# renjie-liang/HUAL

Hardware: AMD Instinct MI355X
Metric: train clips/sec (higher is better)
Workload: dtype f32 (fp16x3 / bf16x3 split-operand MFMA, fp32 accumulate); 1 GPU; Charades-STA SeqPAN train step (fwd+bwd+clip+AdamWD, dropout 0.2), batch 64/GPU, T=128, vdim=1024, L=20, C=8, dim=128, 8 heads, 2 attention layers, random init; ONE batch resident in HBM, batch assembly (hual_assemble_batch) outside the timed region; global_batch=64, T=128, vdim=1024, L=20, parallelism=dp1, launch=hipGraph, video_dtype=f32

## Files before the change

hual_amd/csrc/convblock.h:

```cpp
#pragma once
#include "common.h"
#include "rowops.h"

namespace hual {

struct CbLayerFwd {
  const float* ln_g; const float* ln_b;
  const float* dw;
  const float* wimg;
  const float* bias;
  float* c; float* xout;
  float* y;
  uint8_t* relu_bits; uint8_t* keep_bits;
  float* mean; float* rstd;
  int drop_site;
};
struct CbFwdArgs {
  const float* x0;
  const float* pos; float* x0_out;
  CbLayerFwd l[4];
  int MT;
  uint32_t drop_row0;
};
#define HUAL_CB_MAXMT 46
int conv_block_fused_rows(int R, int Nv = 0);
struct LnProjArgs;
int launch_conv_block_fwd(const CbFwdArgs& a, const RowSpace& rs, const DropCfg& drop, hipStream_t s, const LnProjArgs* tail = nullptr);

struct CbLayerBwd {
  const float* ln_g; const float* ln_b; const float* dw;
  const float* wimg_t;
  const float* x;
  const float* mean; const float* rstd;
  const uint8_t* relu_prev; const uint8_t* keep_prev;
  float* dz;
  float* dz_prev;
  float* part;
};
struct CbBwdArgs {
  const float* dx_in;
  const uint8_t* relu_bits3; const uint8_t* keep_bits3;
  float* dx_out;
  CbLayerBwd l[4];
  int MT;
  uint32_t drop_row0;
};
#define HUAL_CB_BWD_MAXMT 40
int conv_block_fused_rows_bwd(int R, int Nv = 0);
int conv_block_bwd_blocks(int R, int Nv = 0);
int launch_conv_block_bwd(const CbBwdArgs& a, const RowSpace& rs, const DropCfg& drop, hipStream_t s);

}
```

hual_amd/csrc/convblock.hip:

```cpp
#include "convblock.h"
#include "tilecore.h"
#include "prof.h"

using namespace hual;

#include "lnproj_body.h"

#define CB_XS 33
#define CB_NPAR 10
#define CB_TP_F4 (10 * 32)

template <bool TAIL>
__device__ __forceinline__ void conv_block_fwd_body(const CbFwdArgs& a, const RowSpace& rs, const DropCfg& drop, const LnProjArgs* lp, char* cb_lds) {
  const int MT = a.MT;
  const int XR = MT + 24;
  float4* X = reinterpret_cast<float4*>(cb_lds);
  float4* TP = X + XR * CB_XS;
  char* Ahi = reinterpret_cast<char*>(TP + (TAIL ? CB_TP_F4 : 0));
  char* Alo = Ahi + 64 * 256;
  float* ainv = reinterpret_cast<float*>(Alo + 64 * 256);
  float* smean = ainv + 64;
  float* srstd = smean + 72;
  float4* par = reinterpret_cast<float4*>(srstd + 72);
  const int lane = threadIdx.x & 63, wave = threadIdx.x >> 6;
  const int l32 = threadIdx.x & 31, grp = threadIdx.x >> 5;
  const int col = 4 * l32;
  const int R = rs.R;
  const int tile_ = xcd_tile_clip(blockIdx.x, rs.R, rs.Nq > 0 ? rs.Nv : 0, MT);
  if (tile_ < 0) return;
  const int r0 = tile_ * MT;
  if (r0 >= rs.R) return;
  const int xbase = r0 - 12;

  const DropRegs dr = drop_load(drop);
  HUAL_STAMP_K(2, 0);
  TfW wc, wn;
  tf_load_w(wc, a.l[0].wimg, wave, lane);
  {
    float4 xv[5], pv[5], qv[4];
    const float* posp = a.pos ? a.pos : a.x0;
#pragma unroll
    for (int u = 0; u < 5; ++u) {
      const int i = grp + 16 * u, row = min(max(xbase + i, 0), R - 1);
      int lo, hi;
      cb_segment(row, rs, lo, hi);
      xv[u] = ld4(a.x0 + (size_t)row * HUAL_D + col);
      pv[u] = ld4(posp + (size_t)(a.pos ? row - lo : row) * HUAL_D + col);
    }
#pragma unroll
    for (int l = 0; l < 4; ++l) {
      const CbLayerFwd& L = a.l[l];
      const float* src = grp < 7 ? L.dw + grp * HUAL_D : (grp == 7 ? L.ln_g : (grp == 8 ? L.ln_b : L.bias));
      qv[l] = ld4(src + col);
    }
    float4 tq = f4zero();
    if (TAIL) {
      const float* src = lp->g1;
      if (grp == 1) src = lp->b1;
      if (grp == 2 && lp->g2) src = lp->g2;
      if (grp == 3 && lp->g2) src = lp->b2;
#pragma unroll
      for (int k = 0; k < HUAL_LNPROJ_MAX; ++k)
        if (grp == 4 + k && k < lp->nproj && lp->bias[k]) src = lp->bias[k];
      tq = ld4(src + col);
    }
#pragma unroll
    for (int u = 0; u < 5; ++u) {
      const int i = grp + 16 * u, row = xbase + i;
      if (i >= XR) continue;
      const bool ok = row >= 0 && row < R;
      float4 v = ok ? xv[u] : f4zero();
      if (a.pos) {
        v = ok ? cb_add(v, pv[u]) : v;
        if (row >= r0 && row < r0 + MT && row < R) st4(a.x0_out + (size_t)row * HUAL_D + col, v);
      }
      X[__mul24(i, CB_XS) + l32] = v;
    }
#pragma unroll
    for (int l = 0; l < 4; ++l)
      if (grp < CB_NPAR) par[(l * CB_NPAR + grp) * 32 + l32] = qv[l];
    if (TAIL && grp < LNP_TP_VECS) TP[grp * 32 + l32] = tq;
  }
  cb_barrier();
  HUAL_STAMP_K(2, 1);

#pragma unroll 1
  for (int l = 0; l < 4; ++l) {
    const CbLayerFwd& L = a.l[l];
    const int H = 9 - 3 * l;
    const int nout = MT + 2 * H;
    const int ntile = (nout + 15) >> 4;
    const int obase = r0 - H;
    const int j = lane & 15, g = lane >> 4, ecol = 16 * wave + 4 * g;
    const float4* lp = par + l * CB_NPAR * 32;
    {
      const int ri = threadIdx.x >> 2, q = threadIdx.x & 3;
      const int xi = ri + 9 - H;
      const int t = xbase + xi;
      const bool ok = ri < nout + 6 && t >= 0 && t < R;
      float4 v[8];
#pragma unroll
      for (int k = 0; k < 8; ++k) v[k] = ok ? X[__mul24(xi, CB_XS) + 8 * q + k] : f4zero();
      float p[8];
#pragma unroll
      for (int k = 0; k < 8; ++k) p[k] = cb_hsum(v[k]);
      float s = ((p[0] + p[1]) + (p[2] + p[3])) + ((p[4] + p[5]) + (p[6] + p[7]));
      s += dpp_xor_partner(s, 1);
      s += dpp_xor_partner(s, 2);
      const float mean = s * (1.0f / HUAL_D);
#pragma unroll
      for (int k = 0; k < 8; ++k) {
        const float4 d = make_float4(v[k].x - mean, v[k].y - mean, v[k].z - mean, v[k].w - mean);
        p[k] = cb_hsum(cb_mul(d, d));
      }
      s = ((p[0] + p[1]) + (p[2] + p[3])) + ((p[4] + p[5]) + (p[6] + p[7]));
      s += dpp_xor_partner(s, 1);
      s += dpp_xor_partner(s, 2);
      const float rstd = rsqrtf(s * (1.0f / HUAL_D) + LN_EPS);
      if (ok && q == 0) {
        smean[xi] = mean;
        srstd[xi] = rstd;
        if (t >= r0 && t < r0 + MT) { L.mean[t] = mean; L.rstd[t] = rstd; }
      }
    }
    cb_barrier();
    HUAL_STAMP_K(2, 2 + 6 * l);
    if (l + 1 < 4) tf_load_w(wn, a.l[l + 1].wimg, wave, lane);
    {
      const float4 gam = lp[7 * 32 + l32], bet = lp[8 * 32 + l32];
      float4 w[7];
#pragma unroll
      for (int k = 0; k < 7; ++k) w[k] = lp[k * 32 + l32];
      const int la = grp * ntile, lb = la + ntile;
      float4 hv[10];
      {
        float4 xr[10];
        float mr[10], sr[10];
#pragma unroll
        for (int s = 0; s < 10; ++s) {
          const int t = obase + la - 3 + s;
          const int xi = min(max(t - xbase, 0), XR - 1);
          xr[s] = X[__mul24(xi, CB_XS) + l32];
          mr[s] = smean[xi];
          sr[s] = srstd[xi];
        }
#pragma unroll
        for (int s = 0; s < 10; ++s) {
          const int li = la - 3 + s, t = obase + li;
          const bool in = s < ntile + 6 && li < nout + 3 && t >= 0 && t < R;
          const float4 v = xr[s];
          const float mean = mr[s], rstd = sr[s];
          const float4 hn = cb_fma(make_float4((v.x - mean) * rstd, (v.y - mean) * rstd, (v.z - mean) * rstd, (v.w - mean) * rstd), gam, bet);
          hv[s] = in ? hn : f4zero();
        }
      }
      int slo, shi;
      cb_segment(min(max(obase + la, 0), R - 1), rs, slo, shi);
#pragma unroll
      for (int u = 0; u < 4; ++u) {
        const int lo_ = la + u;
        if (lo_ >= lb) continue;
        const int o = obase + lo_;
        float4 c = f4zero();
        const bool live = lo_ < nout && o >= 0 && o < R;
        if (live) {
          if (o >= shi) { slo = shi; shi = slo + (slo < rs.Nv ? rs.T : rs.L); }
          c = cb_fma((o - 3 >= slo) ? hv[u] : f4zero(), w[0], c);
          c = cb_fma((o - 2 >= slo) ? hv[u + 1] : f4zero(), w[1], c);
          c = cb_fma((o - 1 >= slo) ? hv[u + 2] : f4zero(), w[2], c);
          c = cb_fma(hv[u + 3], w[3], c);
          c = cb_fma((o + 1 < shi) ? hv[u + 4] : f4zero(), w[4], c);
          c = cb_fma((o + 2 < shi) ? hv[u + 5] : f4zero(), w[5], c);
          c = cb_fma((o + 3 < shi) ? hv[u + 6] : f4zero(), w[6], c);
          if (o >= r0 && o < r0 + MT) st4_nt(L.c + (size_t)o * HUAL_D + col, c);
        }
        const float inv = cb_store_operand_fx(Ahi, Alo, lo_, l32, c);
        if (l32 == 0) ainv[lo_] = live ? inv : 0.f;
      }
    }
    HUAL_STAMP_K(2, 3 + 6 * l);
    cb_barrier();
    HUAL_STAMP_K(2, 4 + 6 * l);
    f32x4 acc[4];
    if (ntile > 3) tf_mma_lean<4, 64 * 256>(Ahi, wc, lane, acc);
    else tf_mma_lean<3, 64 * 256>(Ahi, wc, lane, reinterpret_cast<f32x4(&)[3]>(acc));
    HUAL_STAMP_K(2, 5 + 6 * l);
    {
      const float4 bias = lp[9 * 32 + (ecol >> 2)];
      const bool dropping = L.drop_site >= 0 && dr.enabled;
      int orow[4];
      bool own[4], live[4];
#pragma unroll
      for (int rt = 0; rt < 4; ++rt) {
        const int lr = 16 * rt + j;
        orow[rt] = obase + lr;
        live[rt] = rt < ntile && lr < nout && orow[rt] >= 0 && orow[rt] < R;
        own[rt] = live[rt] && orow[rt] >= r0 && orow[rt] < r0 + MT;
      }
      uint32_t nib[4] = {15u, 15u, 15u, 15u};
      if (dropping) {
        drop_nib2_store_t(dr, (uint32_t)L.drop_site, a.drop_row0, orow[0], orow[1], own[0], own[1], (uint32_t)(ecol >> 2), L.keep_bits, nib[0], nib[1], lane);
        drop_nib2_store_t(dr, (uint32_t)L.drop_site, a.drop_row0, orow[2], orow[3], own[2], own[3], (uint32_t)(ecol >> 2), L.keep_bits, nib[2], nib[3], lane);
      }
      uint32_t rb[4] = {0u, 0u, 0u, 0u};
      float irv[4];
      float4 xres[4];
#pragma unroll
      for (int rt = 0; rt < 4; ++rt) {
        irv[rt] = ainv[16 * rt + j];
        xres[rt] = X[__mul24(min(max(orow[rt] - xbase, 0), XR - 1), CB_XS) + (ecol >> 2)];
      }
#pragma unroll
      for (int rt = 0; rt < 4; ++rt) {
        if (!live[rt]) continue;
        const int o = orow[rt];
        const float ir = irv[rt];
        float4 v = make_float4(fmaf(acc[rt][0], ir, 0.f) + bias.x, fmaf(acc[rt][1], ir, 0.f) + bias.y,
                               fmaf(acc[rt][2], ir, 0.f) + bias.z, fmaf(acc[rt][3], ir, 0.f) + bias.w);
        v = relu_nan4(v);
        if (own[rt] && L.y) st4(L.y + (size_t)o * HUAL_D + ecol, v);
        rb[rt] = f4_posbits(v);
        if (dropping) v = f4_select(nib[rt], make_float4(v.x * dr.scale, v.y * dr.scale, v.z * dr.scale, v.w * dr.scale));
        v = cb_add(v, xres[rt]);
        X[__mul24(o - xbase, CB_XS) + (ecol >> 2)] = v;
        if (own[rt]) st4(L.xout + (size_t)o * HUAL_D + ecol, v);
      }
      bits_store2_t(L.relu_bits, orow[0], orow[1], own[0], own[1], ecol >> 2, rb[0], rb[1], lane);
      bits_store2_t(L.relu_bits, orow[2], orow[3], own[2], own[3], ecol >> 2, rb[2], rb[3], lane);
    }
    if (l + 1 < 4) wc = wn;
    cb_barrier();
    HUAL_STAMP_K(2, 7 + 6 * l);
  }
  if (TAIL) {
    if (MT <= 32) ln_proj_body<2, true, true>(*lp, drop, Ahi, r0, X, xbase, CB_XS, XR, TP);
    else ln_proj_body<3, true, true>(*lp, drop, Ahi, r0, X, xbase, CB_XS, XR, TP);
  }
}

__global__ __launch_bounds__(CB_THREADS) void conv_block_fwd_kernel(CbFwdArgs a, RowSpace rs, DropCfg drop) {
  extern __shared__ __attribute__((aligned(16))) char cb_lds[];
  conv_block_fwd_body<false>(a, rs, drop, nullptr, cb_lds);
}
__global__ __launch_bounds__(CB_THREADS) void conv_block_fwd_lnproj_kernel(CbFwdArgs a, RowSpace rs, DropCfg drop, LnProjArgs lp) {
  extern __shared__ __attribute__((aligned(16))) char cb_lds[];
  conv_block_fwd_body<true>(a, rs, drop, &lp, cb_lds);
}

__global__ __launch_bounds__(CB_THREADS) void conv_block_bwd_kernel(CbBwdArgs a, RowSpace rs, DropCfg drop) {
  extern __shared__ __attribute__((aligned(16))) char cb_lds[];
  const int MT = a.MT;
  const int XR = MT + 24;
  float4* DX = reinterpret_cast<float4*>(cb_lds);
  char* Ahi = cb_lds + (size_t)XR * 512;
  char* Alo = Ahi + 64 * 256;
  float4* DC = reinterpret_cast<float4*>(Ahi);
  float* ainv = reinterpret_cast<float*>(Ahi + 64 * 512);
  float4* par = reinterpret_cast<float4*>(ainv + 64);
  float4* pbuf = par + 9 * 32;
  const int lane = threadIdx.x & 63, wave = threadIdx.x >> 6;
  const int l32 = threadIdx.x & 31, grp = threadIdx.x >> 5;
  const int col = 4 * l32;
  const int R = rs.R;
  const int tile_ = xcd_tile_clip(blockIdx.x, rs.R, rs.Nq > 0 ? rs.Nv : 0, MT);
  if (tile_ < 0) return;
  const int r0 = tile_ * MT;
  if (r0 >= rs.R) return;
  const int xbase = r0 - 12;

  const DropRegs dr = drop_load(drop);
  const float dscale3 = dr.enabled ? dr.scale : 1.0f;
  HUAL_STAMP_K(3, 0);
  TfW wc;
  tf_load_w(wc, a.l[3].wimg_t, wave, lane);
  {
    float4 dv[4];
    uint32_t zn[4];
#pragma unroll
    for (int u = 0; u < 4; ++u) {
      const int i = grp + 16 * u, row = min(max(xbase + i, 0), R - 1);
      dv[u] = ld4(a.dx_in + (size_t)row * HUAL_D + col);
      const uint32_t kn = bits_nibble(a.keep_bits3, row, l32);
      zn[u] = bits_nibble(a.relu_bits3, row, l32) & (dr.enabled ? kn : 15u);
    }
#pragma unroll
    for (int u = 0; u < 4; ++u) {
      const int i = grp + 16 * u, row = xbase + i;
      if (i >= 64) continue;
      const bool ok = i < XR && row >= 0 && row < R;
      float4 v = ok ? dv[u] : f4zero();
      if (i < XR) DX[i * 32 + l32] = v;
      v = f4_select(ok ? zn[u] : 0u, make_float4(v.x * dscale3, v.y * dscale3, v.z * dscale3, v.w * dscale3));
      if (ok && row >= r0 && row < r0 + MT) st4(a.l[3].dz + (size_t)row * HUAL_D + col, v);
      const float inv = cb_store_operand(Ahi, Alo, i, l32, v);
      if (l32 == 0) ainv[i] = ok ? inv : 0.f;
    }
  }

  HUAL_STAMP_K(3, 1);
#pragma unroll 1
  for (int i = 3; i >= 0; --i) {
    const CbLayerBwd& L = a.l[i];
    const int E1 = 3 * (i + 1), E0 = 3 * i;
    const int nG = MT + 2 * E1, ntile = (nG + 15) >> 4, gbase = r0 - E1;
    const int nR = MT + 2 * E0, rbase = r0 - E0;
    const int ra = (grp * nR) >> 4, rb = ((grp + 1) * nR) >> 4;
    const float4 pv = ld4((grp < 7 ? L.dw + grp * HUAL_D : (grp == 7 ? L.ln_g : L.ln_b)) + col);
    float4 xv[4];
    float mu[4], rsd[4];
    uint32_t zb[4], zk[4];
    const uint8_t* rprev = L.relu_prev ? L.relu_prev : a.relu_bits3;
    const uint8_t* kprev = L.keep_prev ? L.keep_prev : a.keep_bits3;
#pragma unroll
    for (int u = 0; u < 4; ++u) {
      const int tc = min(max(rbase + ra + u, 0), R - 1);
      xv[u] = ld4(L.x + (size_t)tc * HUAL_D + col);
      zk[u] = kprev[(size_t)tc * 16 + (l32 >> 1)];
      zb[u] = rprev[(size_t)tc * 16 + (l32 >> 1)];
      mu[u] = L.mean[tc];
      rsd[u] = L.rstd[tc];
    }
    if (grp < 9) par[grp * 32 + l32] = pv;
    HUAL_STAMP_K(3, 2 + 7 * (3 - i));
    cb_barrier();
    HUAL_STAMP_K(3, 3 + 7 * (3 - i));
    f32x4 acc[4];
    if (ntile > 3) tf_mma_lean<4, 64 * 256>(Ahi, wc, lane, acc);
    else tf_mma_lean<3, 64 * 256>(Ahi, wc, lane, reinterpret_cast<f32x4(&)[3]>(acc));
    if (i > 0) tf_load_w(wc, a.l[i - 1].wimg_t, wave, lane);
    float irv[4];
#pragma unroll
    for (int rt = 0; rt < 4; ++rt) irv[rt] = ainv[16 * rt + (lane & 15)];
    cb_barrier();
    HUAL_STAMP_K(3, 4 + 7 * (3 - i));
    {
      const int j = lane & 15, g = lane >> 4;
#pragma unroll
      for (int rt = 0; rt < 4; ++rt) {
        if (rt >= ntile) continue;
        const int lr = 16 * rt + j;
        const float ir = irv[rt];
        DC[lr * 32 + ((4 * wave + g) ^ (2 * j))] = make_float4(acc[rt][0] * ir, acc[rt][1] * ir, acc[rt][2] * ir, acc[rt][3] * ir);
      }
    }
    cb_barrier();
    uint32_t zbits = 0;
#pragma unroll
    for (int u = 0; u < 4; ++u) {
      const uint32_t sh = 4 * (l32 & 1);
      zbits |= (((zb[u] >> sh) & 15u) & (dr.enabled ? ((zk[u] >> sh) & 15u) : 15u)) << (4 * u);
    }
    HUAL_STAMP_K(3, 5 + 7 * (3 - i));
    float4 sw[7], sg = f4zero(), sb = f4zero();
#pragma unroll
    for (int k = 0; k < 7; ++k) sw[k] = f4zero();
    {
      float4 d0 = f4zero(), d1 = f4zero(), d2 = f4zero(), d3 = f4zero(), d4 = f4zero(), d5 = f4zero(), d6 = f4zero();
#pragma unroll
      for (int s = 0; s < 10; ++s) {
        const int tt = rbase + ra - 3 + s;
        const int di = tt - gbase;
        float4 dn = f4zero();
        if (s < (rb - ra) + 6 && di >= 0 && di < nG && tt >= 0 && tt < R) dn = DC[di * 32 + (l32 ^ (2 * (di & 15)))];
        d0 = d1; d1 = d2; d2 = d3; d3 = d4; d4 = d5; d5 = d6; d6 = dn;
        if (s < 6) continue;
        const int u = s - 6;
        const int lr = ra + u, t = rbase + lr;
        if (!(lr < rb && t >= 0 && t < R)) continue;
        int slo, shi;
        cb_segment(t, rs, slo, shi);
        const float4 e0 = (t + 3 < shi) ? d6 : f4zero(), e1 = (t + 2 < shi) ? d5 : f4zero(), e2 = (t + 1 < shi) ? d4 : f4zero();
        const float4 e4 = (t - 1 >= slo) ? d2 : f4zero(), e5 = (t - 2 >= slo) ? d1 : f4zero(), e6 = (t - 3 >= slo) ? d0 : f4zero();
        float4 dh = f4zero();
        dh = cb_fma(e0, par[0 * 32 + l32], dh); dh = cb_fma(e1, par[1 * 32 + l32], dh); dh = cb_fma(e2, par[2 * 32 + l32], dh);
        dh = cb_fma(d3, par[3 * 32 + l32], dh);
        dh = cb_fma(e4, par[4 * 32 + l32], dh); dh = cb_fma(e5, par[5 * 32 + l32], dh); dh = cb_fma(e6, par[6 * 32 + l32], dh);
        const float4 gam = par[7 * 32 + l32];
        const float4 v = xv[u];
        const float mean = mu[u], rstd = rsd[u];
        const float4 xh = make_float4((v.x - mean) * rstd, (v.y - mean) * rstd, (v.z - mean) * rstd, (v.w - mean) * rstd);
        if (t >= r0 && t < r0 + MT) {
          const float4 h = cb_fma(xh, gam, par[8 * 32 + l32]);
          sw[0] = cb_fma(h, e0, sw[0]); sw[1] = cb_fma(h, e1, sw[1]); sw[2] = cb_fma(h, e2, sw[2]); sw[3] = cb_fma(h, d3, sw[3]);
          sw[4] = cb_fma(h, e4, sw[4]); sw[5] = cb_fma(h, e5, sw[5]); sw[6] = cb_fma(h, e6, sw[6]);
          sb = cb_add(sb, dh);
          sg = cb_fma(dh, xh, sg);
        }
        const float4 gv = cb_mul(dh, gam);
        const float m1 = fast_sum32(cb_hsum(gv)) * (1.0f / HUAL_D);
        const float m2 = fast_sum32(cb_hsum(cb_mul(gv, xh))) * (1.0f / HUAL_D);
        float4 dx = make_float4(rstd * (gv.x - m1 - xh.x * m2), rstd * (gv.y - m1 - xh.y * m2),
                                rstd * (gv.z - m1 - xh.z * m2), rstd * (gv.w - m1 - xh.w * m2));
        float4* dxp = DX + (t - xbase) * 32 + l32;
        const float4 dres = *dxp;
        dx = make_float4(__fadd_rn(dx.x, dres.x), __fadd_rn(dx.y, dres.y), __fadd_rn(dx.z, dres.z), __fadd_rn(dx.w, dres.w));
        *dxp = dx;
        if (i == 0) st4(a.dx_out + (size_t)t * HUAL_D + col, dx);
      }
    }
    HUAL_STAMP_K(3, 6 + 7 * (3 - i));
    {
      auto xor32_sum = [&](float v) {
        const unsigned x = __builtin_bit_cast(unsigned, v);
        const auto r = __builtin_amdgcn_permlane32_swap(x, x, false, false);
        return v + __builtin_bit_cast(float, (lane & 32) ? r[0] : r[1]);
      };
      auto xor32_sum4 = [&](float4 v) { return make_float4(xor32_sum(v.x), xor32_sum(v.y), xor32_sum(v.z), xor32_sum(v.w)); };
#pragma unroll
      for (int k = 0; k < 7; ++k) sw[k] = xor32_sum4(sw[k]);
      sg = xor32_sum4(sg);
      sb = xor32_sum4(sb);
      float pacc[3] = {0.f, 0.f, 0.f};
#pragma unroll
      for (int batch = 0; batch < 2; ++batch) {
        if ((wave >> 2) == batch && lane < 32) {
          float4* dst = pbuf + (wave & 3) * 9 * 32 + l32;
#pragma unroll
          for (int k = 0; k < 7; ++k) dst[k * 32] = sw[k];
          dst[7 * 32] = sg;
          dst[8 * 32] = sb;
        }
        cb_barrier();
        const float* pf = reinterpret_cast<const float*>(pbuf);
#pragma unroll
        for (int q = 0; q < 3; ++q) {
          const int e = threadIdx.x + CB_THREADS * q;
          if (e < 9 * HUAL_D) pacc[q] += (pf[e] + pf[e + 9 * HUAL_D]) + (pf[e + 2 * 9 * HUAL_D] + pf[e + 3 * 9 * HUAL_D]);
        }
        cb_barrier();
      }
#pragma unroll
      for (int q = 0; q < 3; ++q) {
        const int e = threadIdx.x + CB_THREADS * q;
        if (e < 9 * HUAL_D) L.part[(size_t)tile_ * 9 * HUAL_D + e] = pacc[q];
      }
    }
    HUAL_STAMP_K(3, 7 + 7 * (3 - i));
    if (i > 0) {
#pragma unroll
      for (int u = 0; u < 4; ++u) {
        const int lr = ra + u, t = rbase + lr;
        if (lr >= rb) continue;
        const bool ok = lr < rb && t >= 0 && t < R;
        float4 v = f4zero();
        if (ok) {
          v = cb_mul(DX[(t - xbase) * 32 + l32], mask_from_bits4((zbits >> (4 * u)) & 0xfu, dscale3));
        }
        if (ok && t >= r0 && t < r0 + MT) st4(L.dz_prev + (size_t)t * HUAL_D + col, v);
        const float inv = cb_store_operand(Ahi, Alo, lr, l32, v);
        if (l32 == 0) ainv[lr] = ok ? inv : 0.f;
      }
    }
    HUAL_STAMP_K(3, 8 + 7 * (3 - i));
  }
}

#if defined(HUAL_STAMPS) && (HUAL_STAMPS == 2 || HUAL_STAMPS == 3 || HUAL_STAMPS == 7)
extern "C" int hual_debug_stamps(unsigned long long* out, int n) {
  return (int)hipMemcpyFromSymbol(out, HIP_SYMBOL(g_hual_stamps), sizeof(unsigned long long) * (size_t)n);
}
extern "C" int hual_debug_stamps_reset() {
  static unsigned long long zeros[512 * HUAL_STAMP_SLOTS];
  return (int)hipMemcpyToSymbol(HIP_SYMBOL(g_hual_stamps), zeros, sizeof(zeros));
}
#endif

namespace hual {

int conv_block_fused_rows(int R, int Nv) {
  return xcd_clip_rows(R, Nv, 16, HUAL_CB_MAXMT);
}

static size_t cb_fwd_lds(int MT) { return (size_t)(MT + 24) * CB_XS * 16 + 2 * 64 * 256 + (64 + 72 + 72) * sizeof(float) + 4 * CB_NPAR * 512; }

int launch_conv_block_fwd(const CbFwdArgs& a, const RowSpace& rs, const DropCfg& drop, hipStream_t s, const LnProjArgs* tail) {
  HUAL_REQUIRE(a.x0 && rs.R > 0 && a.MT >= 1 && a.MT <= HUAL_CB_MAXMT, "conv_block_fwd: bad arguments");
  HUAL_REQUIRE(!a.pos || a.x0_out, "conv_block_fwd: pos needs x0_out");
  for (int l = 0; l < 4; ++l) {
    const CbLayerFwd& L = a.l[l];
    HUAL_REQUIRE(L.ln_g && L.ln_b && L.dw && L.wimg && L.bias && L.c && L.xout && L.mean && L.rstd && L.relu_bits && L.keep_bits, "conv_block_fwd: null layer tensor");
  }
  const double rows = (double)rs.R;
  const dim3 grid(xcd_clip_grid(rs.R, rs.Nq > 0 ? rs.Nv : 0, a.MT));
  double flops = 4.0 * 2.0 * rows * HUAL_D * HUAL_D, bytes = 4.0 * (rows * HUAL_D * 13.0 + 4.0 * HUAL_D * HUAL_D);
  if (!tail) {
    HUAL_DYN_LDS(conv_block_fwd_kernel, 160 * 1024);
    HUAL_LAUNCH(flops, bytes, conv_block_fwd_kernel, grid, dim3(CB_THREADS), cb_fwd_lds(a.MT), s, a, rs, drop);
  } else {
    LnProjArgs lp = *tail;
    lp.MT = a.MT;
    int rc = check_ln_proj_args(lp);
    if (rc) return rc;
    HUAL_REQUIRE(lp.x == a.l[3].xout && lp.R == rs.R && ln_proj_plain(lp), "conv_block_fwd: the tail must read the block output and be of the plain shape");
    const size_t tail_from_planes = std::max((size_t)LN_PROJ_LDS, cb_fwd_lds(a.MT) - (size_t)(a.MT + 24) * CB_XS * 16);
    const size_t lds = (size_t)(a.MT + 24) * CB_XS * 16 + CB_TP_F4 * 16 + tail_from_planes;
    HUAL_REQUIRE(lds <= 160 * 1024, "conv_block_fwd: LDS of the tail");
    flops += 2.0 * rows * HUAL_D * HUAL_D * lp.nproj;
    bytes += 4.0 * rows * HUAL_D * (lp.nproj + 1.0 + (lp.g2 ? 1.0 : 0.0)) - 4.0 * rows * HUAL_D;
    HUAL_DYN_LDS(conv_block_fwd_lnproj_kernel, 160 * 1024);
    HUAL_LAUNCH(flops, bytes, conv_block_fwd_lnproj_kernel, grid, dim3(CB_THREADS), lds, s, a, rs, drop, lp);
  }
  HUAL_CHECK_HIP(hipGetLastError());
  return 0;
}

int conv_block_fused_rows_bwd(int R, int Nv) { return xcd_clip_rows(R, Nv, 16, HUAL_CB_BWD_MAXMT); }
int conv_block_bwd_blocks(int R, int Nv) { return cdiv(R, conv_block_fused_rows_bwd(R, Nv)); }

static size_t cb_bwd_lds(int MT) { return (size_t)(MT + 24) * 512 + 64 * 512 + 64 * sizeof(float) + (1 + 4) * 9 * HUAL_D * sizeof(float); }

int launch_conv_block_bwd(const CbBwdArgs& a, const RowSpace& rs, const DropCfg& drop, hipStream_t s) {
  HUAL_REQUIRE(a.dx_in && a.relu_bits3 && a.keep_bits3 && a.dx_out && rs.R > 0 && a.MT >= 1 && a.MT <= HUAL_CB_BWD_MAXMT, "conv_block_bwd: bad arguments");
  for (int l = 0; l < 4; ++l) {
    const CbLayerBwd& L = a.l[l];
    HUAL_REQUIRE(L.ln_g && L.ln_b && L.dw && L.wimg_t && L.x && L.mean && L.rstd && L.dz && L.part, "conv_block_bwd: null layer tensor");
    HUAL_REQUIRE(l == 0 || (L.relu_prev && L.keep_prev && L.dz_prev), "conv_block_bwd: layers 1-3 need the bit planes of the layer below / dz_prev");
  }
  HUAL_DYN_LDS(conv_block_bwd_kernel, 160 * 1024);
  const double rows = (double)rs.R;
  HUAL_LAUNCH(4.0 * 2.0 * rows * HUAL_D * HUAL_D, 4.0 * (rows * HUAL_D * 14.0 + 4.0 * HUAL_D * HUAL_D), conv_block_bwd_kernel,
              dim3(xcd_clip_grid(rs.R, rs.Nq > 0 ? rs.Nv : 0, a.MT)), dim3(CB_THREADS), cb_bwd_lds(a.MT), s, a, rs, drop);
  HUAL_CHECK_HIP(hipGetLastError());
  return 0;
}

}
```

hual_amd/csrc/dablock.h:

```cpp
#pragma once
#include "common.h"
#include "rowops.h"

namespace hual {

#define HUAL_LNPROJ_MAX 5
struct LnProjArgs {
  const float* x;
  const float* xa; int pre_site; float* x_out;
  uint8_t* pre_bits; uint8_t* y1_bits;
  const float* x2;
  const float* g1; const float* b1; float* y1;
  int drop_site1;
  const float* g2; const float* b2; float* y2;
  float* mean; float* rstd;
  int nproj;
  const float* wimg[HUAL_LNPROJ_MAX];
  const float* bias[HUAL_LNPROJ_MAX];
  float* out[HUAL_LNPROJ_MAX]; int ldo[HUAL_LNPROJ_MAX];
  int src[HUAL_LNPROJ_MAX];
  int accum[HUAL_LNPROJ_MAX];
  int act[HUAL_LNPROJ_MAX];
  int out_site[HUAL_LNPROJ_MAX];
  uint8_t* out_bits[HUAL_LNPROJ_MAX];
  int add_x[HUAL_LNPROJ_MAX];
  int R; int MT;
  int Nv;
  uint32_t drop_row0;
};
int ln_proj_rows(int R, int Nv = 0);
int launch_ln_proj(const LnProjArgs& a, const DropCfg& drop, hipStream_t s);
int check_ln_proj_args(const LnProjArgs& a);
bool ln_proj_plain(const LnProjArgs& a);
int launch_ln_proj_pair(const LnProjArgs& a0, const LnProjArgs& a1, const DropCfg& drop, hipStream_t s);
int ln_proj_pair_rows(int R);

struct DaPostArgs {
  const float* s_att; const float* x_att; const float* ln1; const float* x;
  const float* rowmask;
  const float* w[11];
  const float* b[9];
  const float* ln2_g; const float* ln2_b;
  float *sv, *xv, *sg, *xg, *o, *gd, *gate, *val, *mha, *res, *l2, *out;
  float *mean2, *rstd2;
  int site;
  uint8_t *bits2, *bits3, *bits4;
  int R; int MT;
  int Nv;
  uint32_t drop_row0;
};
int da_post_rows(int R, int Nv = 0);
int launch_da_post(const DaPostArgs& a, const DropCfg& drop, hipStream_t s, const LnProjArgs* tail = nullptr);

}

namespace hual {

#define HUAL_LNBWD_MAX 6
struct LnProjBwdArgs {
  int nsteps;
  const float* A[HUAL_LNBWD_MAX]; int lda[HUAL_LNBWD_MAX];
  const uint8_t* a_bits[HUAL_LNBWD_MAX];
  float* a_save[HUAL_LNBWD_MAX];
  const float* wimg_t[HUAL_LNBWD_MAX];
  int dst[HUAL_LNBWD_MAX];
  const float* add_dy1;
  const uint8_t* dy1_bits;
  const float* x; const float* mean; const float* rstd;
  const float* g1; const float* g2;
  const float* add1;
  float* dx;
  float* dz; const uint8_t* dz_bits;
  float* part;
  int R; int MT; uint32_t drop_row0;
  int Nv;
  const float* pre_x; const float* pre_mean; const float* pre_rstd; const float* pre_g; const float* pre_dy; const float* pre_add;
};
int ln_proj_bwd_rows(int R, int Nv = 0);
int ln_proj_bwd_blocks(int R, int Nv = 0);
int launch_ln_proj_bwd(const LnProjBwdArgs& a, const DropCfg& drop, hipStream_t s);

struct DaMidBwdArgs {
  const float* dz1;
  const float *gate, *val, *sg, *xg, *sv, *xv;
  const float* w[10];
  float *d_sc, *d_val, *d_ln1a, *d_g, *dz_sg, *dz_xg, *d_sv, *d_xv, *d_satt, *d_xatt;
  int R; int MT; int Nv;
};
int launch_da_mid_bwd(const DaMidBwdArgs& a, hipStream_t s);
bool ln2_mid_bwd_fits(const LnProjBwdArgs& a, const DaMidBwdArgs& m);
int launch_ln2_mid_bwd(const LnProjBwdArgs& a, const DaMidBwdArgs& m, const DropCfg& drop, hipStream_t s);

}
```

hual_amd/csrc/dablock.hip:

```cpp
#include "dablock.h"
#include "tilecore.h"
#include "prof.h"

using namespace hual;

__device__ __forceinline__ float row16_max(float v) {
  v = fmaxf(v, dpp_xor_partner(v, 1));
  v = fmaxf(v, dpp_xor_partner(v, 2));
  v = fmaxf(v, dpp_xor_partner(v, 4));
  v = fmaxf(v, dpp_xor_partner(v, 8));
  return v;
}
__device__ __forceinline__ float4 sig4(float4 v) { return make_float4(sigmoidf_(v.x), sigmoidf_(v.y), sigmoidf_(v.z), sigmoidf_(v.w)); }

#include "lnproj_body.h"

template <int NT, bool PLAIN>
__global__ __launch_bounds__(CB_THREADS) void ln_proj_kernel(LnProjArgs a, DropCfg drop) {
  extern __shared__ __attribute__((aligned(16))) char lp_lds[];
  ln_proj_body<NT, false, PLAIN>(a, drop, lp_lds);
}
template <int NT>
__global__ __launch_bounds__(CB_THREADS) void ln_proj_pair_kernel(LnProjArgs a0, LnProjArgs a1, DropCfg drop) {
  extern __shared__ __attribute__((aligned(16))) char lp_lds[];
// ... 131 lines not shown
  tf_mma_lean<NT, DP_PLANE>(P1, wb, lane, accp);
  tf_load_w(wb, a.w[3], wave, lane);
  fold(XV, ainv1, true);
#pragma unroll
  for (int rt = 0; rt < NT; ++rt) {
    SV[rt] = addb(SV[rt], 0);
    XV[rt] = addb(XV[rt], 1);
    save_nt(a.sv, rt, SV[rt]);
    save_nt(a.xv, rt, XV[rt]);
  }
  zero_invalid(SV);
  zero_invalid(XV);
  put(P2, ainv2, SV);
  put(P3, ainv3, XV);
  cb_barrier();
  tf_mma_lean<NT, DP_PLANE>(P2, wa, lane, accp);
  fold(T1, ainv2, true);
  tf_load_w(wa, a.w[4], wave, lane);
  tf_mma_lean<NT, DP_PLANE>(P3, wb, lane, accp);
  tf_load_w(wb, a.w[5], wave, lane);
  fold(T2, ainv3, true);
#pragma unroll
  for (int rt = 0; rt < NT; ++rt) {
    const float4 sg = sig4(addb(T1[rt], 2)), xg = sig4(addb(T2[rt], 3));
    save_nt(a.sg, rt, sg);
    save_nt(a.xg, rt, xg);
    T1[rt] = cb_add(cb_mul(sg, XV[rt]), cb_mul(xg, SV[rt]));
    save_nt(a.o, rt, T1[rt]);
  }
  zero_invalid(T1);
  put(P0, ainv0, T1);
  cb_barrier();
  tf_mma_lean<NT, DP_PLANE>(P0, wa, lane, accp);
  tf_load_w(wa, a.w[6], wave, lane);
  fold(T1, ainv0, true);
#pragma unroll
  for (int rt = 0; rt < NT; ++rt) { T1[rt] = addb(T1[rt], 4); save_nt(a.gd, rt, T1[rt]); }
  zero_invalid(T1);
  put(P2, ainv2, T1);
#pragma unroll
  for (int u = 0; u < 3; ++u) {
    const int lr = grp + 16 * u;
    if (lr >= MT) continue;
    const bool ok = r0 + lr < RE;
    const float i0 = cb_store_operand_fx(P1, P1 + DP_PLANE, lr, l32, ok ? l1[u] : f4zero());
    if (l32 == 0) ainv1[lr] = ok ? i0 : 0.f;
  }
  cb_barrier();
  tf_mma_lean<NT, DP_PLANE>(P1, wb, lane, accp);
  fold(T1, ainv1, true);
  tf_load_w(wb, a.w[7], wave, lane);
  tf_mma_lean<NT, DP_PLANE>(P2, wa, lane, accp);
  fold(T1, ainv2, false);
  tf_load_w(wa, a.w[8], wave, lane);
  tf_mma_lean<NT, DP_PLANE>(P1, wb, lane, accp);
  fold(T2, ainv1, true);
  tf_load_w(wb, a.w[9], wave, lane);
  tf_mma_lean<NT, DP_PLANE>(P2, wa, lane, accp);
  tf_load_w(wa, a.w[10], wave, lane);
  fold(T2, ainv2, false);
#pragma unroll
  for (int rt = 0; rt < NT; ++rt) {
    float4 gate = addb(T1[rt], 5);
    gate = rm[rt] != 0.f ? sig4(gate) : f4zero();
    const float4 val = addb(T2[rt], 6);
    save_nt(a.gate, rt, gate);
    save_nt(a.val, rt, val);
    T1[rt] = cb_mul(gate, val);
    save_nt(a.mha, rt, T1[rt]);
  }
  zero_invalid(T1);
  put(P3, ainv3, T1);
  cb_barrier();
  tf_mma_lean<NT, DP_PLANE>(P3, wb, lane, accp);
  fold(SV, ainv3, true);
  {
    uint32_t nbd[NT];
#pragma unroll
    for (int rt = 0; rt < NT; ++rt) nbd[rt] = 15u;
    if (dr.enabled) drop_rows((uint32_t)(a.site + 2), a.bits2, nbd);
#pragma unroll
    for (int rt = 0; rt < NT; ++rt) {
      const int lr = 16 * rt + j;
      float4 v = addb(SV[rt], 7);
      if (dr.enabled) v = f4_select(nbd[rt], make_float4(v.x * dr.scale, v.y * dr.scale, v.z * dr.scale, v.w * dr.scale));
      v = cb_add(v, xin[rt]);
      SV[rt] = v;
      save(a.res, rt, v);
      scratch[lr * 32 + (ecol >> 2)] = v;
    }
  }
  cb_barrier();
  {
    const float4 g2 = bl[9 * 32 + l32], b2 = bl[10 * 32 + l32];
    uint32_t nb3[4] = {15u, 15u, 15u, 15u};
    if (dr.enabled) {
      const int lrA = grp, lrB = grp + 16, lrC = grp + 32;
      drop_nib2_store_r(dr, (uint32_t)(a.site + 3), a.drop_row0, r0 + lrA, r0 + lrB, lrA < MT && r0 + lrA < RE, lrB < MT && r0 + lrB < RE,
                        (uint32_t)l32, a.bits3, nb3[0], nb3[1]);
      drop_nib2_store_r(dr, (uint32_t)(a.site + 3), a.drop_row0, r0 + lrC, r0 + lrC, lrC < MT && r0 + lrC < RE, lrC < MT && r0 + lrC < RE,
                        (uint32_t)l32, a.bits3, nb3[2], nb3[3]);
    }
#pragma unroll
    for (int u = 0; u < 3; ++u) {
      const int lr = grp + 16 * u, row = r0 + lr;
      if (lr >= MT) continue;
      const bool ok = row < RE;
      float mean, rstd;
      const float4 xh = ln_row(scratch[lr * 32 + l32], mean, rstd);
      float4 y = cb_fma(xh, g2, b2);
      if (dr.enabled) y = f4_select(nb3[u], make_float4(y.x * dr.scale, y.y * dr.scale, y.z * dr.scale, y.w * dr.scale));
      if (!ok) y = f4zero();
      if (ok) {
        st4_nt(a.l2 + (size_t)row * HUAL_D + col, y);
        if (l32 == 0) { a.mean2[row] = mean; a.rstd2[row] = rstd; }
      }
      const float i2 = cb_store_operand_fx(P2, P2 + DP_PLANE, lr, l32, y);
      if (l32 == 0) ainv2[lr] = ok ? i2 : 0.f;
    }
  }
  cb_barrier();
  tf_mma_lean<NT, DP_PLANE>(P2, wa, lane, accp);
  fold(T1, ainv2, true);
  {
    uint32_t nbe[NT];
#pragma unroll
    for (int rt = 0; rt < NT; ++rt) nbe[rt] = 15u;
    if (dr.enabled) drop_rows((uint32_t)(a.site + 4), a.bits4, nbe);
#pragma unroll
    for (int rt = 0; rt < NT; ++rt) {
      float4 v = addb(T1[rt], 8);
      if (dr.enabled) v = f4_select(nbe[rt], make_float4(v.x * dr.scale, v.y * dr.scale, v.z * dr.scale, v.w * dr.scale));
      v = cb_add(v, SV[rt]);
      save(a.out, rt, v);
      if (TAIL) scratch[(16 * rt + j) * 32 + (ecol >> 2)] = v;
    }
  }
  if (TAIL) {
    cb_barrier();
    ln_proj_body<NT, true, true>(*lp, drop, P1, r0, scratch, r0, 32, DP_ROWS, TP);
  }
}
template <int NT>
__global__ __launch_bounds__(CB_THREADS) void da_post_kernel(DaPostArgs a, DropCfg drop) {
  extern __shared__ __attribute__((aligned(16))) char dp_lds[];
  da_post_body<NT, false>(a, drop, nullptr, dp_lds);
}
template <int NT>
__global__ __launch_bounds__(CB_THREADS) void da_post_lnproj_kernel(DaPostArgs a, DropCfg drop, LnProjArgs lp) {
  extern __shared__ __attribute__((aligned(16))) char dp_lds[];
  da_post_body<NT, true>(a, drop, &lp, dp_lds);
}

#define LB_ROWS 48
#define LB_U (LB_ROWS / 16)
template <int NT> struct DaMidPre { TfW wa, wb; float4 gate[NT], val[NT]; };
#define LB_LDS ((size_t)4 * LB_ROWS * 256 + 8 * 4 * 32 * 16 + 2 * LB_ROWS * sizeof(float))
template <bool PRE, int NT, bool SIX, bool MID>
__device__ __forceinline__ bool ln_proj_bwd_body(const LnProjBwdArgs& a, const DropCfg& drop, char* lb_lds, const DaMidBwdArgs* m,
                                                 DaMidPre<NT>* mp, float4 (&zv)[LB_U]) {
  char* S0 = lb_lds;
  char* S1 = S0 + 2 * LB_ROWS * 256;
  char* Ps = S1 + 2 * LB_ROWS * 256;
  float* ainv0 = reinterpret_cast<float*>(Ps + 8 * 4 * 32 * 16);
  float* ainv1 = ainv0 + LB_ROWS;
  const int lane = threadIdx.x & 63, wave = threadIdx.x >> 6;
  const int l32 = threadIdx.x & 31, grp = threadIdx.x >> 5;
  const int col = 4 * l32;
  const int MT = a.MT, R = a.R;
  const int tile_ = xcd_tile_clip(blockIdx.x, R, a.Nv, MT);
  if (tile_ < 0) return false;
  const int r0 = tile_ * MT;
  const int RE = min(R, r0 + MT);
  const int j = lane & 15, g = lane >> 4, ecol = 16 * wave + 4 * g;
  const DropRegs dr = drop_load(drop);

  TfW w[2];
  tf_load_w(w[0], a.wimg_t[0], wave, lane);
  float4 nv[LB_U], xv[LB_U], a1v[LB_U];
  float mu[LB_U], rsd[LB_U];
  constexpr bool pre = PRE;
  const float* add1p = pre ? (a.pre_add ? a.pre_add : a.x) : (a.add1 ? a.add1 : a.x);
  const float* a0p = pre ? a.pre_dy : a.A[0];
  const int lda0 = pre ? HUAL_D : a.lda[0];
  uint32_t nkb[LB_U];
  const int nsteps = SIX ? 6 : (MID ? 1 : a.nsteps);
  auto has_bits = [&](int k) { return !SIX && a.a_bits[k] != nullptr; };
  auto to_second = [&](int k) { return SIX ? k >= 4 : a.dst[k] != 0; };
  const bool has_g2 = SIX || (!MID && a.g2 != nullptr), has_add_dy1 = SIX || (!MID && a.add_dy1 != nullptr), has_dy1_bits = !SIX && a.dy1_bits != nullptr;
  const uint8_t* kb0p = has_bits(0) ? a.a_bits[0] : reinterpret_cast<const uint8_t*>(a.x);
  float4 pxv[LB_U];
  float pmu[LB_U], prs[LB_U];
#pragma unroll
  for (int u = 0; u < LB_U; ++u) {
    const int row = min(r0 + grp + 16 * u, R - 1);
    nv[u] = ld4(a0p + (size_t)row * lda0 + col);
    nkb[u] = SIX ? 0u : kb0p[(size_t)row * 16 + (l32 >> 1)];
    xv[u] = ld4(a.x + (size_t)row * HUAL_D + col);
    a1v[u] = ld4(add1p + (size_t)row * HUAL_D + col);
    mu[u] = a.mean[row];
    rsd[u] = a.rstd[row];
    if (pre) { pxv[u] = ld4(a.pre_x + (size_t)row * HUAL_D + col); pmu[u] = a.pre_mean[row]; prs[u] = a.pre_rstd[row]; }
  }
  const float4 g1 = ld4(a.g1 + col);
  float4 sg2 = f4zero(), sb2 = f4zero();
  if (pre) {
    const float4 pg = ld4(a.pre_g + col);
#pragma unroll
    for (int u = 0; u < LB_U; ++u) {
      const int lr = grp + 16 * u;
      const bool ok = lr < MT && r0 + lr < RE;
      const float4 v = pxv[u], dy = nv[u];
      const float mean = pmu[u], rstd = prs[u];
      const float4 xh = make_float4((v.x - mean) * rstd, (v.y - mean) * rstd, (v.z - mean) * rstd, (v.w - mean) * rstd);
      if (ok) { sb2 = cb_add(sb2, dy); sg2 = cb_fma(dy, xh, sg2); }
      const float4 gv = cb_mul(dy, pg);
      const float m1 = fast_sum32(cb_hsum(gv)) * (1.0f / HUAL_D);
      const float m2 = fast_sum32(cb_hsum(cb_mul(gv, xh))) * (1.0f / HUAL_D);
      float4 dx = make_float4(rstd * (gv.x - m1 - xh.x * m2), rstd * (gv.y - m1 - xh.y * m2),
                              rstd * (gv.z - m1 - xh.z * m2), rstd * (gv.w - m1 - xh.w * m2));
      if (a.pre_add) dx = make_float4(__fadd_rn(dx.x, a1v[u].x), __fadd_rn(dx.y, a1v[u].y), __fadd_rn(dx.z, a1v[u].z), __fadd_rn(dx.w, a1v[u].w));
      nv[u] = dx;
      a1v[u] = dx;
    }
  }
  const float4 g2 = has_g2 ? ld4(a.g2 + col) : f4zero();
  float4 addt[NT];
  const float* addp = has_add_dy1 ? a.add_dy1 : a.x;
#pragma unroll
  for (int rt = 0; rt < NT; ++rt) addt[rt] = (SIX || MID) ? f4zero() : ld4(addp + (uint32_t)min(r0 + 16 * rt + j, R - 1) * (uint32_t)HUAL_D + (uint32_t)ecol);
  auto fill = [&](int k) {
    char* S = (k & 1) ? S1 : S0;
    float* ai = (k & 1) ? ainv1 : ainv0;
#pragma unroll
    for (int u = 0; u < LB_U; ++u) {
      const int lr = grp + 16 * u, row = r0 + lr;
      if (lr >= MT) continue;
      const bool ok = row < RE;
      float4 v = ok ? nv[u] : f4zero();
      if (has_bits(k)) {
        if (dr.enabled) v = f4_select((nkb[u] >> (4 * (l32 & 1))) & 15u, make_float4(v.x * dr.scale, v.y * dr.scale, v.z * dr.scale, v.w * dr.scale));
        if (ok && a.a_save[k]) st4_nt(a.a_save[k] + (size_t)row * HUAL_D + col, v);
      }
      const float inv = cb_store_operand(S, S + LB_ROWS * 256, lr, l32, v);
      if (l32 == 0) ai[lr] = ok ? inv : 0.f;
    }
  };
  HUAL_STAMP_K(4, 0);
  fill(0);
  HUAL_STAMP_K(4, 1);
  float4 acc0[NT], acc1[NT];
  bool first0 = true, first1 = true;
#pragma unroll
  for (int rt = 0; rt < NT; ++rt) { acc0[rt] = f4zero(); acc1[rt] = f4zero(); }
#pragma unroll
  for (int k = 0; k < HUAL_LNBWD_MAX; ++k) {
    if (k >= nsteps) break;
    const bool more = k + 1 < nsteps;
    if (SIX && k == 5) {
#pragma unroll
      for (int rt = 0; rt < NT; ++rt) addt[rt] = ld4(addp + (uint32_t)min(r0 + 16 * rt + j, R - 1) * (uint32_t)HUAL_D + (uint32_t)ecol);
    }
    if (more) {
      const uint8_t* nbp = has_bits(k + 1) ? a.a_bits[k + 1] : reinterpret_cast<const uint8_t*>(a.x);
      const float* nap = a.A[k + 1];
      const int nld = a.lda[k + 1];
#pragma unroll
      for (int u = 0; u < LB_U; ++u) {
        const size_t row = (size_t)min(r0 + grp + 16 * u, R - 1);
        nv[u] = ld4(nap + row * nld + col);
        nkb[u] = SIX ? 0u : nbp[row * 16 + (l32 >> 1)];
      }
      tf_load_w(w[(k + 1) & 1], a.wimg_t[k + 1], wave, lane);
    }
    cb_barrier();
    HUAL_STAMP_K(4, 2 + 3 * k);
    const char* S = (k & 1) ? S1 : S0;
    const float* ai = (k & 1) ? ainv1 : ainv0;
    f32x4 accp[NT];
    tf_mma_lean<NT, LB_ROWS * 256>(S, w[k & 1], lane, accp);
    HUAL_STAMP_K(4, 3 + 3 * k);
    {
      const bool to1 = to_second(k);
      const bool first = to1 ? first1 : first0;
#pragma unroll
      for (int rt = 0; rt < NT; ++rt) {
        const float ir = ai[16 * rt + j];
        const float4 o = to1 ? acc1[rt] : acc0[rt];
        const float4 n = first ? make_float4(fmaf(accp[rt][0], ir, 0.f), fmaf(accp[rt][1], ir, 0.f), fmaf(accp[rt][2], ir, 0.f), fmaf(accp[rt][3], ir, 0.f))
                               : make_float4(fmaf(accp[rt][0], ir, o.x), fmaf(accp[rt][1], ir, o.y), fmaf(accp[rt][2], ir, o.z), fmaf(accp[rt][3], ir, o.w));
        if (to1) acc1[rt] = n; else acc0[rt] = n;
      }
    }
    if (to_second(k)) first1 = false; else first0 = false;
    if (more) fill(k + 1);
    HUAL_STAMP_K(4, 4 + 3 * k);
  }
  cb_barrier();
  HUAL_STAMP_K(4, 20);
  float4* D0 = reinterpret_cast<float4*>(S0);
  float4* D1 = reinterpret_cast<float4*>(S1);
#pragma unroll
  for (int rt = 0; rt < NT; ++rt) {
    const int lr = 16 * rt + j;
    float4 v = acc0[rt];
    if (has_add_dy1) v = cb_add(v, addt[rt]);
    D0[lr * 32 + (ecol >> 2)] = v;
    if (has_g2) D1[lr * 32 + (ecol >> 2)] = acc1[rt];
  }
  uint32_t kb1[LB_U], kbz[LB_U];
  {
    const uint8_t* b1p = has_dy1_bits ? a.dy1_bits : reinterpret_cast<const uint8_t*>(a.x);
    const uint8_t* bzp = a.dz_bits ? a.dz_bits : reinterpret_cast<const uint8_t*>(a.x);
#pragma unroll
    for (int u = 0; u < LB_U; ++u) {
      const size_t row = (size_t)min(r0 + grp + 16 * u, R - 1);
      kb1[u] = SIX ? 0u : b1p[row * 16 + (l32 >> 1)];
      kbz[u] = bzp[row * 16 + (l32 >> 1)];
    }
  }
  if (MID) {
    tf_load_w(mp->wa, m->w[0], wave, lane);
    tf_load_w(mp->wb, m->w[1], wave, lane);
#pragma unroll
    for (int rt = 0; rt < NT; ++rt) {
      const uint32_t eo = (uint32_t)min(r0 + 16 * rt + j, R - 1) * (uint32_t)HUAL_D + (uint32_t)ecol;
      mp->gate[rt] = ld4(m->gate + eo);
      mp->val[rt] = ld4(m->val + eo);
    }
#pragma unroll
    for (int u = 0; u < LB_U; ++u) zv[u] = f4zero();
  }
  cb_barrier();
  HUAL_STAMP_K(4, 21);
  float4 sg1 = f4zero(), sb1 = f4zero();
#pragma unroll
  for (int u = 0; u < LB_U; ++u) {
    const int lr = grp + 16 * u, row = r0 + lr;
    if (lr >= MT || row >= R) continue;
    const size_t off = (size_t)row * HUAL_D + col;
    const float4 v = xv[u];
    const float mean = mu[u], rstd = rsd[u];
    const float4 xh = make_float4((v.x - mean) * rstd, (v.y - mean) * rstd, (v.z - mean) * rstd, (v.w - mean) * rstd);
    float4 dy = D0[lr * 32 + l32];
    if (has_dy1_bits && dr.enabled) dy = f4_select((kb1[u] >> (4 * (l32 & 1))) & 15u, make_float4(dy.x * dr.scale, dy.y * dr.scale, dy.z * dr.scale, dy.w * dr.scale));
    sb1 = cb_add(sb1, dy);
    sg1 = cb_fma(dy, xh, sg1);
    float4 gv = cb_mul(dy, g1);
    if (has_g2) {
      const float4 dy2 = D1[lr * 32 + l32];
      sb2 = cb_add(sb2, dy2);
      sg2 = cb_fma(dy2, xh, sg2);
      gv = cb_fma(dy2, g2, gv);
    }
    const float m1 = fast_sum32(cb_hsum(gv)) * (1.0f / HUAL_D);
    const float m2 = fast_sum32(cb_hsum(cb_mul(gv, xh))) * (1.0f / HUAL_D);
    float4 dx = make_float4(rstd * (gv.x - m1 - xh.x * m2), rstd * (gv.y - m1 - xh.y * m2),
                            rstd * (gv.z - m1 - xh.z * m2), rstd * (gv.w - m1 - xh.w * m2));
    if (SIX || a.add1 || pre) dx = make_float4(__fadd_rn(dx.x, a1v[u].x), __fadd_rn(dx.y, a1v[u].y), __fadd_rn(dx.z, a1v[u].z), __fadd_rn(dx.w, a1v[u].w));
    st4(a.dx + off, dx);
    if (a.dz) {
      if (a.dz_bits && dr.enabled) dx = f4_select((kbz[u] >> (4 * (l32 & 1))) & 15u, make_float4(dx.x * dr.scale, dx.y * dr.scale, dx.z * dr.scale, dx.w * dr.scale));
      st4(a.dz + off, dx);
      if (MID) zv[u] = dx;
    }
  }
  HUAL_STAMP_K(4, 22);
  {
    auto xor32_sum = [&](float v) {
      const unsigned x = __builtin_bit_cast(unsigned, v);
      const auto r = __builtin_amdgcn_permlane32_swap(x, x, false, false);
      return v + __builtin_bit_cast(float, (lane & 32) ? r[0] : r[1]);
    };
    auto xor32_sum4 = [&](float4 v) { return make_float4(xor32_sum(v.x), xor32_sum(v.y), xor32_sum(v.z), xor32_sum(v.w)); };
    sg1 = xor32_sum4(sg1); sb1 = xor32_sum4(sb1); sg2 = xor32_sum4(sg2); sb2 = xor32_sum4(sb2);
    float4* pb = reinterpret_cast<float4*>(Ps);
    if (lane < 32) {
      float4* dst = pb + wave * 4 * 32 + l32;
      dst[0] = sg1; dst[32] = sb1; dst[64] = sg2; dst[96] = sb2;
    }
    cb_barrier();
    const float* pf = reinterpret_cast<const float*>(pb);
    const int e = threadIdx.x;
    float s = 0.f;
#pragma unroll
    for (int w = 0; w < 8; ++w) s += pf[w * 4 * HUAL_D + e];
    a.part[(size_t)tile_ * 4 * HUAL_D + e] = s;
  }
  HUAL_STAMP_K(4, 23);
  return true;
}
template <bool PRE, int NT, bool SIX = false>
__global__ __launch_bounds__(CB_THREADS) void ln_proj_bwd_kernel(LnProjBwdArgs a, DropCfg drop) {
  extern __shared__ __attribute__((aligned(16))) char lb_lds[];
  float4 zv[LB_U];
  ln_proj_bwd_body<PRE, NT, SIX, false>(a, drop, lb_lds, nullptr, nullptr, zv);
}

#define DM_LDS ((size_t)3 * DP_SLOT + (3 * DP_ROWS + 16 * DP_ROWS) * sizeof(float))
template <int NT, bool FUSED>
__device__ __forceinline__ void da_mid_bwd_body(const DaMidBwdArgs& a, char* dm_lds, DaMidPre<NT>* mp, const float4 (&zin)[3]) {
  char* P0 = dm_lds;
  char* P1 = P0 + DP_SLOT;
  char* P2 = P1 + DP_SLOT;
  float* ainv0 = reinterpret_cast<float*>(P2 + DP_SLOT);
  float* ainv1 = ainv0 + DP_ROWS;
  float* ainv2 = ainv1 + DP_ROWS;
  float* smaxA = ainv2 + DP_ROWS;
  float* smaxB = smaxA + 8 * DP_ROWS;
  const int lane = threadIdx.x & 63, wave = threadIdx.x >> 6;
  const int l32 = threadIdx.x & 31, grp = threadIdx.x >> 5;
  const int col = 4 * l32;
  const int MT = a.MT, R = a.R;
  const int tile_ = xcd_tile_clip(blockIdx.x, R, a.Nv, MT);
  if (tile_ < 0) return;
  const int r0 = tile_ * MT;
  const int RE = min(R, r0 + MT);
  const int j = lane & 15, g = lane >> 4, ecol = 16 * wave + 4 * g;

  TfW wa, wb;
  if (FUSED) wa = mp->wa;
  else tf_load_w(wa, a.w[0], wave, lane);
  {
    float4 zv[3];
#pragma unroll
    for (int u = 0; u < 3; ++u) zv[u] = FUSED ? zin[u] : ld4(a.dz1 + (size_t)min(r0 + grp + 16 * u, R - 1) * HUAL_D + col);
#pragma unroll
    for (int u = 0; u < 3; ++u) {
      const int lr = grp + 16 * u;
      if (lr >= MT) continue;
      const bool ok = r0 + lr < RE;
      const float inv = cb_store_operand(P1, P1 + DP_PLANE, lr, l32, ok ? zv[u] : f4zero());
      if (l32 == 0) ainv1[lr] = ok ? inv : 0.f;
    }
  }
  f32x4 accp[NT];
  auto fold = [&](float4 (&acc)[NT], const float* ai, bool first) {
#pragma unroll
    for (int rt = 0; rt < NT; ++rt) {
      const float ir = ai[16 * rt + j];
      if (first) acc[rt] = make_float4(fmaf(accp[rt][0], ir, 0.f), fmaf(accp[rt][1], ir, 0.f), fmaf(accp[rt][2], ir, 0.f), fmaf(accp[rt][3], ir, 0.f));
      else acc[rt] = make_float4(fmaf(accp[rt][0], ir, acc[rt].x), fmaf(accp[rt][1], ir, acc[rt].y), fmaf(accp[rt][2], ir, acc[rt].z), fmaf(accp[rt][3], ir, acc[rt].w));
    }
  };
  uint32_t eoff[NT];
#pragma unroll
  for (int rt = 0; rt < NT; ++rt) eoff[rt] = (uint32_t)min(r0 + 16 * rt + j, R - 1) * (uint32_t)HUAL_D + (uint32_t)ecol;
  auto tile_ld = [&](const float* src, float4 (&t)[NT]) {
#pragma unroll
    for (int rt = 0; rt < NT; ++rt) t[rt] = ld4(src + eoff[rt]);
  };
  auto save = [&](float* dst, int rt, float4 v) {
    if (r0 + 16 * rt + j < RE) st4(dst + eoff[rt], v);
  };
  auto save_nt = [&](float* dst, int rt, float4 v) {
    if (r0 + 16 * rt + j < RE) DA_ST_NT(dst + eoff[rt], v);
  };
  auto put_max = [&](float* sm, const float4 (&v)[NT]) {
#pragma unroll
    for (int rt = 0; rt < NT; ++rt) {
      const float m = slice16_max(f4absmax(v[rt]), lane);
      if (g == 0) sm[(16 * rt + j) * 8 + wave] = m;
    }
  };
  auto put_planes = [&](char* P, float* ai, const float* sm, const float4 (&v)[NT]) {
#pragma unroll
    for (int rt = 0; rt < NT; ++rt) {
      const int lr = 16 * rt + j;
      const float4 ma = *reinterpret_cast<const float4*>(sm + lr * 8), mb = *reinterpret_cast<const float4*>(sm + lr * 8 + 4);
      float inv;
      const float sc = f16_row_scale(fmaxf(fmaxf(fmaxf(ma.x, ma.y), fmaxf(ma.z, ma.w)), fmaxf(fmaxf(mb.x, mb.y), fmaxf(mb.z, mb.w))), inv);
      uint2 h, l;
      f16_split4(f4scale1(v[rt], sc), h, l);
      const int off = tile256_off(lr, ecol >> 3) + 8 * (g & 1);
      *reinterpret_cast<uint2*>(P + off) = h;
      *reinterpret_cast<uint2*>(P + DP_PLANE + off) = l;
      if (wave == 0 && g == 0) ai[lr] = (r0 + lr < RE) ? inv : 0.f;
    }
  };
  auto zero_invalid = [&](float4 (&v)[NT]) {
#pragma unroll
    for (int rt = 0; rt < NT; ++rt) if (r0 + 16 * rt + j >= RE) v[rt] = f4zero();
  };

  float4 T1[NT], T2[NT], U1[NT], U2[NT], U3[NT], U4[NT];
  if (FUSED) {
    wb = mp->wb;
#pragma unroll
    for (int rt = 0; rt < NT; ++rt) { U1[rt] = mp->gate[rt]; U2[rt] = mp->val[rt]; }
  } else {
    tf_load_w(wb, a.w[1], wave, lane);
    tile_ld(a.gate, U1);
    tile_ld(a.val, U2);
  }
  cb_barrier();
  tf_mma_lean<NT, DP_PLANE>(P1, wa, lane, accp);
  tf_load_w(wa, a.w[2], wave, lane);
  fold(T1, ainv1, true);
#pragma unroll
  for (int rt = 0; rt < NT; ++rt) {
    const float4 d0 = T1[rt], gt = U1[rt], vl = U2[rt];
    T1[rt] = make_float4(d0.x * vl.x * gt.x * (1.f - gt.x), d0.y * vl.y * gt.y * (1.f - gt.y), d0.z * vl.z * gt.z * (1.f - gt.z),
                         d0.w * vl.w * gt.w * (1.f - gt.w));
    T2[rt] = cb_mul(d0, gt);
    save_nt(a.d_sc, rt, T1[rt]);
    save_nt(a.d_val, rt, T2[rt]);
  }
  zero_invalid(T1);
  zero_invalid(T2);
  put_max(smaxA, T1);
  put_max(smaxB, T2);
  cb_barrier();
  put_planes(P0, ainv0, smaxA, T1);
  put_planes(P2, ainv2, smaxB, T2);
  cb_barrier();
  tf_mma_lean<NT, DP_PLANE>(P0, wb, lane, accp);
  fold(T1, ainv0, true);
  tf_load_w(wb, a.w[3], wave, lane);
  tf_mma_lean<NT, DP_PLANE>(P2, wa, lane, accp);
  fold(T1, ainv2, false);
  tf_load_w(wa, a.w[4], wave, lane);
  tf_mma_lean<NT, DP_PLANE>(P0, wb, lane, accp);
  fold(T2, ainv0, true);
  tf_load_w(wb, a.w[5], wave, lane);
  tile_ld(a.sg, U1);
  tile_ld(a.xg, U2);
  tile_ld(a.sv, U3);
  tile_ld(a.xv, U4);
#pragma unroll
  for (int rt = 0; rt < NT; ++rt) save(a.d_ln1a, rt, T1[rt]);
  tf_mma_lean<NT, DP_PLANE>(P2, wa, lane, accp);
  fold(T2, ainv2, false);
  tf_load_w(wa, a.w[6], wave, lane);
#pragma unroll
  for (int rt = 0; rt < NT; ++rt) save_nt(a.d_g, rt, T2[rt]);
  zero_invalid(T2);
  put_max(smaxA, T2);
  cb_barrier();
  put_planes(P1, ainv1, smaxA, T2);
  cb_barrier();
  tf_mma_lean<NT, DP_PLANE>(P1, wb, lane, accp);
  tf_load_w(wb, a.w[7], wave, lane);
  fold(T1, ainv1, true);
#pragma unroll
// ... 64 lines not shown

#if defined(HUAL_STAMPS) && (HUAL_STAMPS == 1 || (HUAL_STAMPS >= 4 && HUAL_STAMPS <= 6))
extern "C" int hual_debug_stamps(unsigned long long* out, int n) {
  return (int)hipMemcpyFromSymbol(out, HIP_SYMBOL(g_hual_stamps), sizeof(unsigned long long) * (size_t)n);
}
extern "C" int hual_debug_stamps_reset() {
  static unsigned long long zeros[512 * HUAL_STAMP_SLOTS];
  return (int)hipMemcpyToSymbol(HIP_SYMBOL(g_hual_stamps), zeros, sizeof(zeros));
}
#endif

namespace hual {

static int tile_rows(int R, int Nv, int max_rows) { return xcd_clip_rows(R, Nv, 16, max_rows); }
int ln_proj_rows(int R, int Nv) { return tile_rows(R, Nv, LP_ROWS); }
int ln_proj_pair_rows(int R) {
  int mt = 16;
  while (mt < LP_ROWS && 2 * xcd_clip_grid(R, 0, mt) > 256) ++mt;
  return mt;
}
int da_post_rows(int R, int Nv) { return tile_rows(R, Nv, DP_ROWS); }

static int check_ln_proj(const LnProjArgs& a) {
  HUAL_REQUIRE(a.x && a.g1 && a.b1 && a.y1 && a.mean && a.rstd && a.R > 0, "ln_proj: null / empty");
  HUAL_REQUIRE(a.MT >= 1 && a.MT <= LP_ROWS, "ln_proj: MT must be 1..64");
  HUAL_REQUIRE(a.nproj >= 1 && a.nproj <= HUAL_LNPROJ_MAX, "ln_proj: projection count");
  HUAL_REQUIRE(!a.g2 || (a.b2 && a.y2), "ln_proj: second layer norm incomplete");
  HUAL_REQUIRE(!(a.g2 && a.x2), "ln_proj: second layer norm and raw second operand are exclusive");
  HUAL_REQUIRE(!a.xa || a.x_out, "ln_proj: xa needs x_out");
  for (int p = 0; p < a.nproj; ++p) {
    HUAL_REQUIRE(a.wimg[p] && (a.accum[p] || (a.out[p] && (a.ldo[p] % 4) == 0)), "ln_proj: projection operand");
    HUAL_REQUIRE(a.src[p] == 0 || a.g2 || a.x2, "ln_proj: projection reads an absent second operand");
    HUAL_REQUIRE(!a.add_x[p] || !(a.g2 || a.x2), "ln_proj: the residual rows share LDS with the second operand");
    HUAL_REQUIRE(!a.accum[p] || p + 1 < a.nproj, "ln_proj: the last projection cannot be marked accum");
  }
  return 0;
}
int check_ln_proj_args(const LnProjArgs& a) { return check_ln_proj(a); }
bool ln_proj_plain(const LnProjArgs& a) {
  if (a.xa || a.x2 || a.pre_site >= 0) return false;
  for (int p = 0; p < a.nproj; ++p)
    if (a.accum[p] || a.act[p] || a.out_site[p] >= 0 || a.add_x[p]) return false;
  return true;
}
static const size_t kLnProjLds = LN_PROJ_LDS;
static void ln_proj_work(const LnProjArgs& a, double& flops, double& bytes) {
  const double rows = (double)a.R;
  flops += 2.0 * rows * HUAL_D * HUAL_D * a.nproj;
  bytes += 4.0 * (rows * HUAL_D * (2.0 + (a.g2 ? 1.0 : 0.0) + a.nproj) + (double)a.nproj * HUAL_D * HUAL_D);
}

int launch_ln_proj(const LnProjArgs& a, const DropCfg& drop, hipStream_t s) {
  int rc = check_ln_proj(a);
  if (rc) return rc;
  double flops = 0.0, bytes = 0.0;
  ln_proj_work(a, flops, bytes);
  const dim3 grid(xcd_clip_grid(a.R, a.Nv, a.MT));
  const bool plain = ln_proj_plain(a);
#define LN_PROJ_NT(NT) { if (plain) { HUAL_DYN_LDS((ln_proj_kernel<NT, true>), 160 * 1024); HUAL_LAUNCH(flops, bytes, (ln_proj_kernel<NT, true>), grid, dim3(CB_THREADS), kLnProjLds, s, a, drop); } \
                         else { HUAL_DYN_LDS((ln_proj_kernel<NT, false>), 160 * 1024); HUAL_LAUNCH(flops, bytes, (ln_proj_kernel<NT, false>), grid, dim3(CB_THREADS), kLnProjLds, s, a, drop); } break; }
  switch (cdiv(a.MT, 16)) {
    case 1: LN_PROJ_NT(1)
    case 2: LN_PROJ_NT(2)
    case 3: LN_PROJ_NT(3)
    default: LN_PROJ_NT(4)
  }
#undef LN_PROJ_NT
  HUAL_CHECK_HIP(hipGetLastError());
  return 0;
}

int launch_ln_proj_pair(const LnProjArgs& a0, const LnProjArgs& a1, const DropCfg& drop, hipStream_t s) {
  int rc = check_ln_proj(a0);
  if (rc) return rc;
  if ((rc = check_ln_proj(a1))) return rc;
  HUAL_REQUIRE(a0.R == a1.R && a0.MT == a1.MT, "ln_proj_pair: the two problems must have the same rows / tile");
  double flops = 0.0, bytes = 0.0;
  ln_proj_work(a0, flops, bytes);
  ln_proj_work(a1, flops, bytes);
  const dim3 grid(xcd_clip_grid(a0.R, a0.Nv, a0.MT), 2);
#define LN_PROJ_NT(NT) { HUAL_DYN_LDS(ln_proj_pair_kernel<NT>, 160 * 1024); HUAL_LAUNCH(flops, bytes, ln_proj_pair_kernel<NT>, grid, dim3(CB_THREADS), kLnProjLds, s, a0, a1, drop); break; }
  switch (cdiv(a0.MT, 16)) {
    case 1: LN_PROJ_NT(1)
    case 2: LN_PROJ_NT(2)
    case 3: LN_PROJ_NT(3)
    default: LN_PROJ_NT(4)
  }
#undef LN_PROJ_NT
  HUAL_CHECK_HIP(hipGetLastError());
  return 0;
}

int launch_da_post(const DaPostArgs& a, const DropCfg& drop, hipStream_t s, const LnProjArgs* tail) {
  HUAL_REQUIRE(a.s_att && a.x_att && a.ln1 && a.x && a.rowmask && a.ln2_g && a.ln2_b && a.R > 0, "da_post: null / empty");
  HUAL_REQUIRE(a.MT >= 1 && a.MT <= DP_ROWS, "da_post: MT must be 1..48");
  for (int k = 0; k < 11; ++k) HUAL_REQUIRE(a.w[k] != nullptr, "da_post: null weight image");
  for (int k = 0; k < 9; ++k) HUAL_REQUIRE(a.b[k] != nullptr, "da_post: null bias");
  HUAL_REQUIRE(a.sv && a.xv && a.sg && a.xg && a.o && a.gd && a.gate && a.val && a.mha && a.res && a.l2 && a.out && a.mean2 && a.rstd2,
               "da_post: null output");
  const size_t lds = (size_t)4 * DP_SLOT + DP_NB * 512 + 4 * DP_ROWS * sizeof(float) + (tail ? 10 * 512 : 0);
  const double rows = (double)a.R;
  double flops = 11.0 * 2.0 * rows * HUAL_D * HUAL_D, bytes = 4.0 * (rows * HUAL_D * 16.0 + 11.0 * HUAL_D * HUAL_D);
  const dim3 grid(xcd_clip_grid(a.R, a.Nv, a.MT));
  if (tail) {
    LnProjArgs lp = *tail;
    lp.MT = a.MT;
    int rc = check_ln_proj(lp);
    if (rc) return rc;
    HUAL_REQUIRE(lp.x == a.out && lp.R == a.R && ln_proj_plain(lp), "da_post: the tail must read the block output and be of the plain shape");
    static_assert(DP_SLOT + LN_PROJ_LDS <= 4 * DP_SLOT, "the tail's operand slots must fit slots 1 .. 3");
    flops += 2.0 * rows * HUAL_D * HUAL_D * lp.nproj;
    bytes += 4.0 * rows * HUAL_D * (lp.nproj + (lp.g2 ? 1.0 : 0.0));
    switch (cdiv(a.MT, 16)) {
      case 1: { HUAL_DYN_LDS(da_post_lnproj_kernel<1>, 160 * 1024); HUAL_LAUNCH(flops, bytes, da_post_lnproj_kernel<1>, grid, dim3(CB_THREADS), lds, s, a, drop, lp); break; }
      case 2: { HUAL_DYN_LDS(da_post_lnproj_kernel<2>, 160 * 1024); HUAL_LAUNCH(flops, bytes, da_post_lnproj_kernel<2>, grid, dim3(CB_THREADS), lds, s, a, drop, lp); break; }
      default: { HUAL_DYN_LDS(da_post_lnproj_kernel<3>, 160 * 1024); HUAL_LAUNCH(flops, bytes, da_post_lnproj_kernel<3>, grid, dim3(CB_THREADS), lds, s, a, drop, lp); break; }
    }
    HUAL_CHECK_HIP(hipGetLastError());
    return 0;
  }
  switch (cdiv(a.MT, 16)) {
    case 1: { HUAL_DYN_LDS(da_post_kernel<1>, 160 * 1024); HUAL_LAUNCH(flops, bytes, da_post_kernel<1>, grid, dim3(CB_THREADS), lds, s, a, drop); break; }
    case 2: { HUAL_DYN_LDS(da_post_kernel<2>, 160 * 1024); HUAL_LAUNCH(flops, bytes, da_post_kernel<2>, grid, dim3(CB_THREADS), lds, s, a, drop); break; }
    default: { HUAL_DYN_LDS(da_post_kernel<3>, 160 * 1024); HUAL_LAUNCH(flops, bytes, da_post_kernel<3>, grid, dim3(CB_THREADS), lds, s, a, drop); break; }
  }
  HUAL_CHECK_HIP(hipGetLastError());
  return 0;
}

int ln_proj_bwd_rows(int R, int Nv) { return tile_rows(R, Nv, LB_ROWS); }
int ln_proj_bwd_blocks(int R, int Nv) { return cdiv(R, ln_proj_bwd_rows(R, Nv)); }

static bool ln_proj_bwd_six(const LnProjBwdArgs& a) {
  if (a.pre_x || a.nsteps != 6 || !a.g2 || !a.add_dy1 || a.dy1_bits || !a.add1) return false;
  for (int k = 0; k < 6; ++k)
    if (a.a_bits[k] || a.a_save[k] || (a.dst[k] != 0) != (k >= 4)) return false;
  return true;
}

static int check_ln_proj_bwd(const LnProjBwdArgs& a) {
  HUAL_REQUIRE(a.nsteps >= 1 && a.nsteps <= HUAL_LNBWD_MAX && a.R > 0, "ln_proj_bwd: step count / rows");
  HUAL_REQUIRE(a.MT >= 1 && a.MT <= LB_ROWS, "ln_proj_bwd: MT must be 1..48");
  HUAL_REQUIRE(a.x && a.mean && a.rstd && a.g1 && a.dx && a.part, "ln_proj_bwd: null tensor");
  bool any1 = false;
  for (int k = 0; k < a.nsteps; ++k) {
    HUAL_REQUIRE((a.A[k] || (k == 0 && a.pre_x)) && a.wimg_t[k] && (a.lda[k] % 4) == 0, "ln_proj_bwd: product operand");
    HUAL_REQUIRE(a.dst[k] == 0 || a.g2, "ln_proj_bwd: product for the absent second layer norm");
    any1 = any1 || a.dst[k] != 0;
  }
  HUAL_REQUIRE(!a.g2 || any1, "ln_proj_bwd: second layer norm without a product");
  HUAL_REQUIRE(!a.pre_x || (!a.g2 && !a.add1 && a.pre_mean && a.pre_rstd && a.pre_g && a.pre_dy), "ln_proj_bwd: layer-norm prologue");
  return 0;
}
static void ln_proj_bwd_work(const LnProjBwdArgs& a, double& flops, double& bytes) {
  const double rows = (double)a.R;
  flops += 2.0 * rows * HUAL_D * HUAL_D * a.nsteps;
  bytes += 4.0 * (rows * HUAL_D * ((a.pre_x ? 7.0 : 4.0) + a.nsteps) + (double)a.nsteps * HUAL_D * HUAL_D);
}

int launch_ln_proj_bwd(const LnProjBwdArgs& a, const DropCfg& drop, hipStream_t s) {
  int rc = check_ln_proj_bwd(a);
  if (rc) return rc;
  const size_t lds = LB_LDS;
  double flops = 0.0, bytes = 0.0;
  ln_proj_bwd_work(a, flops, bytes);
  const dim3 grid(xcd_clip_grid(a.R, a.Nv, a.MT));
  const bool six = ln_proj_bwd_six(a);
#define LN_BWD_NT(NT)                                                                                                   \
  {                                                                                                                     \
    if (a.pre_x) { HUAL_DYN_LDS((ln_proj_bwd_kernel<true, NT>), 160 * 1024); HUAL_LAUNCH(flops, bytes, (ln_proj_bwd_kernel<true, NT>), grid, dim3(CB_THREADS), lds, s, a, drop); } \
    else if (six) { HUAL_DYN_LDS((ln_proj_bwd_kernel<false, NT, true>), 160 * 1024); HUAL_LAUNCH(flops, bytes, (ln_proj_bwd_kernel<false, NT, true>), grid, dim3(CB_THREADS), lds, s, a, drop); } \
    else { HUAL_DYN_LDS((ln_proj_bwd_kernel<false, NT>), 160 * 1024); HUAL_LAUNCH(flops, bytes, (ln_proj_bwd_kernel<false, NT>), grid, dim3(CB_THREADS), lds, s, a, drop); }      \
    break;                                                                                                              \
  }
  switch (cdiv(a.MT, 16)) {
    case 1: LN_BWD_NT(1)
    case 2: LN_BWD_NT(2)
    default: LN_BWD_NT(3)
  }
#undef LN_BWD_NT
  HUAL_CHECK_HIP(hipGetLastError());
  return 0;
}

static int check_da_mid_bwd(const DaMidBwdArgs& a) {
  HUAL_REQUIRE(a.dz1 && a.gate && a.val && a.sg && a.xg && a.sv && a.xv && a.R > 0, "da_mid_bwd: null / empty");
  HUAL_REQUIRE(a.MT >= 1 && a.MT <= DP_ROWS, "da_mid_bwd: MT must be 1..48");
  for (int k = 0; k < 10; ++k) HUAL_REQUIRE(a.w[k] != nullptr, "da_mid_bwd: null weight image");
  HUAL_REQUIRE(a.d_sc && a.d_val && a.d_ln1a && a.d_g && a.dz_sg && a.dz_xg && a.d_sv && a.d_xv && a.d_satt && a.d_xatt, "da_mid_bwd: null output");
  return 0;
}
static void da_mid_bwd_work(const DaMidBwdArgs& a, double& flops, double& bytes) {
  const double rows = (double)a.R;
  flops += 10.0 * 2.0 * rows * HUAL_D * HUAL_D;
  bytes += 4.0 * (rows * HUAL_D * 17.0 + 10.0 * HUAL_D * HUAL_D);
}

int launch_da_mid_bwd(const DaMidBwdArgs& a, hipStream_t s) {
  int rc = check_da_mid_bwd(a);
  if (rc) return rc;
  const size_t lds = DM_LDS;
  double flops = 0.0, bytes = 0.0;
  da_mid_bwd_work(a, flops, bytes);
  const dim3 grid(xcd_clip_grid(a.R, a.Nv, a.MT));
  switch (cdiv(a.MT, 16)) {
    case 1: { HUAL_DYN_LDS(da_mid_bwd_kernel<1>, 160 * 1024); HUAL_LAUNCH(flops, bytes, da_mid_bwd_kernel<1>, grid, dim3(CB_THREADS), lds, s, a); break; }
    case 2: { HUAL_DYN_LDS(da_mid_bwd_kernel<2>, 160 * 1024); HUAL_LAUNCH(flops, bytes, da_mid_bwd_kernel<2>, grid, dim3(CB_THREADS), lds, s, a); break; }
    default: { HUAL_DYN_LDS(da_mid_bwd_kernel<3>, 160 * 1024); HUAL_LAUNCH(flops, bytes, da_mid_bwd_kernel<3>, grid, dim3(CB_THREADS), lds, s, a); break; }
  }
  HUAL_CHECK_HIP(hipGetLastError());
  return 0;
}

bool ln2_mid_bwd_fits(const LnProjBwdArgs& a, const DaMidBwdArgs& m) {
  return a.nsteps == 1 && !a.pre_x && !a.g2 && !a.add_dy1 && a.dst[0] == 0 && a.dz && a.dz == m.dz1 && a.R == m.R && a.Nv == m.Nv && a.MT == m.MT;
}

int launch_ln2_mid_bwd(const LnProjBwdArgs& a, const DaMidBwdArgs& m, const DropCfg& drop, hipStream_t s) {
  int rc = check_ln_proj_bwd(a);
  if (rc) return rc;
  if ((rc = check_da_mid_bwd(m))) return rc;
  HUAL_REQUIRE(ln2_mid_bwd_fits(a, m), "ln2_mid_bwd: one product into one layer norm whose dz is the middle's dz1, on the same row tiles");
  static_assert(LB_ROWS == DP_ROWS, "the two bodies share their row tiles");
  const size_t lds = LB_LDS > DM_LDS ? LB_LDS : DM_LDS;
  double flops = 0.0, bytes = 0.0;
  ln_proj_bwd_work(a, flops, bytes);
  da_mid_bwd_work(m, flops, bytes);
  bytes -= 4.0 * (double)a.R * HUAL_D;
  const dim3 grid(xcd_clip_grid(a.R, a.Nv, a.MT));
  switch (cdiv(a.MT, 16)) {
    case 1: { HUAL_DYN_LDS(ln2_mid_bwd_kernel<1>, 160 * 1024); HUAL_LAUNCH(flops, bytes, ln2_mid_bwd_kernel<1>, grid, dim3(CB_THREADS), lds, s, a, m, drop); break; }
    case 2: { HUAL_DYN_LDS(ln2_mid_bwd_kernel<2>, 160 * 1024); HUAL_LAUNCH(flops, bytes, ln2_mid_bwd_kernel<2>, grid, dim3(CB_THREADS), lds, s, a, m, drop); break; }
    default: { HUAL_DYN_LDS(ln2_mid_bwd_kernel<3>, 160 * 1024); HUAL_LAUNCH(flops, bytes, ln2_mid_bwd_kernel<3>, grid, dim3(CB_THREADS), lds, s, a, m, drop); break; }
  }
  HUAL_CHECK_HIP(hipGetLastError());
  return 0;
}

}
```

hual_amd/csrc/seqpan.hip:

```cpp
#include "attn.h"
#include "prof.h"
#include "cq.h"
#include "convblock.h"
#include "dablock.h"
#include "embed.h"
#include "gemm.h"
#include "heads.h"
#include "mproj.h"
#include "optim.h"
#include "params.h"
#include "rowops.h"
#include <stdlib.h>
#include <string.h>
#include <algorithm>
#include <unordered_map>
#include <vector>

namespace hual {
const char* last_error_cstr();
}
using namespace hual;

namespace {

enum { ST_ALWAYS = 0, ST_INPUT = 1, ST_CONV = 2, ST_DA = 3, ST_CQ = 4, ST_FUSE = 5, ST_PRED = 6 };

struct WsEntry { std::string name; size_t off, rows, cols; };

struct Ctx {
  const hual_cfg* cfg = nullptr;
  ParamMap pm;
  int B = 0, T = 0, L = 0, C = 0;
  RowSpace rs;
  RowSpace rsv;
  char* base = nullptr;
  size_t cap = 0, used = 0;
  bool dry = true;
  hipStream_t stream = nullptr;
  DropCfg drop;
  const float* P = nullptr;
  float* G = nullptr;
  const float* word_table = nullptr;
  std::vector<WsEntry> entries;
  std::unordered_map<std::string, size_t> index;
  std::vector<DwJob> dwjobs;
  std::vector<ColsumJob> colsum;
  int rc = 0;
  bool static_tables = false;
  void* ext_table = nullptr; size_t ext_table_bytes = 0;
  int wall_K = 0; uint32_t wall_off = 0, wall_boff = 0;
  struct DenseW { size_t off; int K; size_t boff; uint8_t need; };
  bool ksplit = false;
  std::vector<DenseW> dense;
  char* PKF = nullptr;
  char* PKT = nullptr;
  char* PKN = nullptr;
  const float* timg(size_t off, int blk = 0) const { return reinterpret_cast<const float*>(PKT + boff_of(off) + (size_t)blk * 65536); }
  const float* nimg(size_t off, int blk = 0) const { return reinterpret_cast<const float*>(PKN + boff_of(off) + (size_t)blk * 65536); }
  size_t boff_of(size_t off) const {
    for (const auto& d : dense) if (d.off == off) return d.boff;
    return off * 4;
  }
  size_t pk_bytes = 0;

  float* find(const std::string& name) {
    auto it = index.find(name);
    if (it != index.end()) return reinterpret_cast<float*>(base + entries[it->second].off);
    if (rc == 0) rc = fail(HUAL_ERR_WORKSPACE, "internal: unknown workspace buffer '" + name + "'");
    return reinterpret_cast<float*>(base);
  }
  float* buf(const std::string& name, size_t rows, size_t cols) {
    if (!dry || index.count(name)) return find(name);
    WsEntry e{name, used, rows, cols};
    size_t bytes = (rows * cols * sizeof(float) + 255) & ~(size_t)255;
    used += bytes + 256;
    index[name] = entries.size();
    entries.push_back(e);
    return reinterpret_cast<float*>(base + e.off);
  }
  float* act(const std::string& name) { return buf(name, (size_t)rs.R, HUAL_D); }
  int novf = 0;
  bool debug_taps = false;
  float* actv(const std::string& name) { return buf(name, (size_t)rs.Nv, HUAL_D); }
  float* vec(const std::string& name) { return buf(name, (size_t)rs.R, 1); }
  const float* p(size_t off) const { return P + off; }
  float* g(size_t off) const { return G + off; }
  int catw() const { return cfg->word_dim + 100; }
  bool ok() const { return rc == 0; }
  void chk(int r) { if (rc == 0 && r != 0) rc = r; }
  int sel_stage = -1, sel_sub = 0;
  bool active = true;
  bool want_bwd = false;
  int part_seq = 0;
  void stage(int st, int sub = 0) { active = sel_stage < 0 || st == ST_ALWAYS || (st == sel_stage && (st != ST_DA || sub == sel_sub)); }
  bool stage_on(int st, int sub = 0) const { return sel_stage < 0 || (st == sel_stage && (st != ST_DA || sub == sel_sub)); }
  bool live() const { return !dry && active && rc == 0; }
  void push_dw(const DwJob& j) { if (active) dwjobs.push_back(j); }

  void ln_bwd(const LnBwd& a0) {
    LnBwd a = a0;
    const int nblk = ln_bwd_blocks(a.R);
    a.part = buf("part." + std::to_string(part_seq++), (size_t)nblk * 4, HUAL_D);
    ColsumJob cj{};
    cj.src = a.part; cj.nblk = nblk; cj.nvec = 4;
    cj.dst[0] = a.dg1; cj.dst[1] = a.db1; cj.dst[2] = a.dg2; cj.dst[3] = a.db2;
    if (active) colsum.push_back(cj);
    if (live()) chk(launch_ln_bwd(a, drop, stream));
  }
  void ln_bwd_split(const LnBwd& a0, float* dg_lo, float* db_lo, float* dg_hi, float* db_hi, const PosBwdJob* pos = nullptr, int npos = 0) {
    LnBwd a = a0;
    const int nlo = ln_bwd_blocks(a.split), nhi = ln_bwd_blocks(a.R - a.split);
    a.part = buf("part." + std::to_string(part_seq++), (size_t)(nlo + nhi) * 4, HUAL_D);
    ColsumJob cj{};
    cj.src = a.part; cj.nblk = nlo; cj.nvec = 4;
    cj.dst[0] = dg_lo; cj.dst[1] = db_lo;
    if (active) colsum.push_back(cj);
    cj.src = a.part + (size_t)nlo * 4 * HUAL_D; cj.nblk = nhi;
    cj.dst[0] = dg_hi; cj.dst[1] = db_hi;
    if (active) colsum.push_back(cj);
    if (live()) chk(launch_ln_bwd(a, drop, stream, pos, npos, &rs));
  }
  void ln_proj_bwd(const LnProjBwdArgs& a0, float* dg1, float* db1, float* dg2, float* db2) {
    LnProjBwdArgs a = a0;
    a.MT = ln_proj_bwd_rows(a.R, a.Nv);
    const int nblk = ln_proj_bwd_blocks(a.R, a.Nv);
    a.part = buf("part." + std::to_string(part_seq++), (size_t)nblk * 4, HUAL_D);
    ColsumJob cj{};
    cj.src = a.part; cj.nblk = nblk; cj.nvec = 4;
    cj.dst[0] = dg1; cj.dst[1] = db1; cj.dst[2] = dg2; cj.dst[3] = db2;
    if (active) colsum.push_back(cj);
    if (live()) chk(launch_ln_proj_bwd(a, drop, stream));
  }
  void ln2_mid_bwd(const LnProjBwdArgs& a0, const DaMidBwdArgs& m0, float* dg1, float* db1) {
    LnProjBwdArgs a = a0;
    DaMidBwdArgs m = m0;
    a.MT = ln_proj_bwd_rows(a.R, a.Nv);
    m.MT = da_post_rows(m.R, m.Nv);
    const int nblk = ln_proj_bwd_blocks(a.R, a.Nv);
    a.part = buf("part." + std::to_string(part_seq++), (size_t)nblk * 4, HUAL_D);
    ColsumJob cj{};
    cj.src = a.part; cj.nblk = nblk; cj.nvec = 4;
    cj.dst[0] = dg1; cj.dst[1] = db1;
    if (active) colsum.push_back(cj);
    if (!live()) return;
#ifndef HUAL_NO_DA_BWD_FUSE
    if (sel_stage < 0 && ln2_mid_bwd_fits(a, m)) { chk(launch_ln2_mid_bwd(a, m, drop, stream)); return; }
#endif
    chk(launch_ln_proj_bwd(a, drop, stream));
    if (ok()) chk(launch_da_mid_bwd(m, stream));
  }
  void flush_colsum(const EmbedUnpack* unpack = nullptr) {
    for (size_t i = 0; i < colsum.size() && !dry && ok(); i += HUAL_COLSUM_MAX_JOBS) {
      const bool last = i + HUAL_COLSUM_MAX_JOBS >= colsum.size();
      chk(launch_colsum(colsum.data() + i, (int)std::min<size_t>(HUAL_COLSUM_MAX_JOBS, colsum.size() - i), stream, last ? unpack : nullptr));
    }
    if (colsum.empty() && unpack && !dry && ok()) chk(launch_colsum(nullptr, 0, stream, unpack));
    colsum.clear();
  }
  void attn_fwd(const AttnJob* j, int n) { if (live()) chk(launch_attn_fwd(j, n, drop, stream)); }
  void attn_bwd(const AttnJob* j, int n) {
    if (live()) chk(launch_attn_bwd(j, n, drop, stream));
  }
};

void set_embed_scratch(EmbedArgs& ea, float* base, int Nq, int C, int char_dim) {
  const EmbedLayout el = embed_layout(Nq, C, char_dim);
  ea.cemb = base + el.cemb; ea.ball = base + el.ball;
  ea.yall = base + el.yall; ea.dxall = base + el.dxall; ea.dfall = base + el.dfall;
}
void fill_embed_args(Ctx& c, EmbedArgs& ea, const hual_batch* bt, float* cat, int catw, int32_t* char_arg, float* scratch) {
  const ParamMap& pm = c.pm;
  ea.word_ids = bt->word_ids; ea.char_ids = bt->char_ids; ea.word_table = c.word_table; ea.unk = c.p(pm.unk);
  ea.char_table = c.p(pm.char_table);
  for (int i = 0; i < 4; ++i) { ea.filt[i] = c.p(pm.filt[i]); ea.fbias[i] = c.p(pm.fbias[i]); }
  ea.cat = cat; ea.ldcat = catw; ea.char_arg = char_arg;
  set_embed_scratch(ea, scratch, c.rs.Nq, c.C, c.cfg->char_dim);
  ea.word_dim = c.cfg->word_dim; ea.char_dim = c.cfg->char_dim; ea.C = c.C; ea.num_chars = c.cfg->num_chars;
  ea.wall_img = reinterpret_cast<const float*>(c.PKT + c.wall_boff);
  ea.wall_img_t = reinterpret_cast<const float*>(c.PKN + c.wall_boff);
}
DwJob mkdw(const float* A, int lda, int K, const float* dY, int ldy, int M, float* dW, float* db, int N = HUAL_D) {
  DwJob j;
  dw_job_init(j);
  j.npieces = 1;
  j.A[0] = A; j.lda[0] = lda; j.kw[0] = K; j.dW[0] = dW; j.ldw = N;
  j.dY = dY; j.ldy = ldy; j.M = M; j.N = N; j.db = db;
  return j;
}

MProjStep mstep(const float* A, int lda, int kw, const float* img, int wrows, bool first, bool last) {
  MProjStep s{};
  s.A = A; s.lda = lda; s.kw = kw; s.wimg = img; s.wrows = wrows; s.first = first ? 1 : 0; s.last = last ? 1 : 0;
  s.drop_site = -1; s.rep = 1; s.add_div = 1; s.ncol = HUAL_D;
  return s;
}
MProjStep mstep_reuse(const float* img, int wrows, bool first, bool last) {
  MProjStep s = mstep(nullptr, 0, 0, img, wrows, first, last);
  s.reuse = 1;
  return s;
}
void mstep_out(MProjStep& s, float* out, int ldo, const float* bias = nullptr, int ncol = HUAL_D) { s.out = out; s.ldo = ldo; s.bias = bias; s.ncol = ncol; }
MProjArgs margs(int R, int R_other = 0) {
  MProjArgs a{};
  a.R = R; a.MT = mproj_rows(R, R_other); a.drop_row0 = 0;
  return a;
}

void flush_dw(Ctx& c) {
  const size_t n = c.dwjobs.size();
  if (n == 0) return;
  std::stable_sort(c.dwjobs.begin(), c.dwjobs.end(), [](const DwJob& a, const DwJob& b) { return a.M > b.M; });
  DwJob* table = reinterpret_cast<DwJob*>(c.buf("dw.table.0", 1, dw_table_words(n)));
  if (!c.dry && c.ext_table) {
    if (4 * dw_table_words(n) > c.ext_table_bytes) { c.chk(fail(HUAL_ERR_INVALID, "hual_run_opts.dw_table too small: hual_seqpan_dw_table_bytes()")); return; }
    table = reinterpret_cast<DwJob*>(c.ext_table);
  }
  if (!c.dry && c.ok()) c.chk(launch_dw(c.dwjobs.data(), (int)n, c.drop, c.stream, table, !c.static_tables));
  c.dwjobs.clear();
}

int setup_ctx(Ctx& c, const hual_cfg* cfg, int B, int T, int L, int C) {
  HUAL_REQUIRE(cfg != nullptr, "null cfg");
  int rc = build_param_map(*cfg, c.pm);
  if (rc) return rc;
  HUAL_REQUIRE(B >= 1 && T >= 1 && L >= 1, "empty batch");
  HUAL_REQUIRE(T <= cfg->max_vlen && L <= cfg->max_vlen, "sequence longer than max_vlen (assert_less_equal, modules.py:44)");
  HUAL_REQUIRE(T <= 256 && L <= 256, "T, L <= 256");
  HUAL_REQUIRE(C >= 4, "char_ids need C >= 4 (conv width 4, VALID)");
  HUAL_REQUIRE((long long)B * (T + L) * 8 < (1ll << 28), "batch too large for 32-bit RNG row ids");
  HUAL_REQUIRE((long long)B * (T + L) < (1ll << 20), "batch too large: B (T + L) < 2^20 rows (row -> clip lookups, common.h small_div)");
  c.cfg = cfg; c.B = B; c.T = T; c.L = L; c.C = C;
  {
    const ParamMap& pm = c.pm;
    const int D = HUAL_D, catw = cfg->word_dim + 100;
    c.dense.clear();
    const uint8_t TN = HUAL_PACK_T | HUAL_PACK_N;
    auto add = [&](size_t off, int K, uint8_t need) { if (K % 8 == 0) c.dense.push_back({off, K, off * 4, need}); };
    const int qks = ((catw + 3) / 4 + 63) & ~63;
    c.ksplit = (cfg->vdim % 256) == 0 && cfg->vdim <= 1024 && (catw % 8) == 0 && qks <= 256;
    add(pm.vconv.k, cfg->vdim, c.ksplit ? HUAL_PACK_F : HUAL_PACK_T);
    add(pm.qconv.k, catw, (c.ksplit ? HUAL_PACK_F : HUAL_PACK_T) | HUAL_PACK_N);
    add(pm.shid.k, 2 * D, TN); add(pm.ehid.k, 2 * D, TN);
    add(pm.fe_dense.k, D, TN); add(pm.fe_q.k, D, TN); add(pm.fe_k.k, D, TN); add(pm.fe_v.k, D, TN);
    for (int i = 0; i < 4; ++i) { add(pm.fe_cb.pw[i], D, TN); add(pm.cb.pw[i], D, TN); }
    add(pm.cqcat.k, 2 * D, TN); add(pm.cq[0].dense, 4 * D, TN); add(pm.cq[1].dense, 4 * D, TN);
    for (int li = 0; li < cfg->attn_layer; ++li) {
      const DualAttnP& d = pm.da[li];
      const size_t w[] = {d.dense1.k, d.dense2.k, d.bl1_d1, d.bl1_d2, d.bl2_d1, d.bl2_d2, d.guided.k, d.s_gate.k, d.x_gate.k,
                          d.s_dense.k, d.x_dense.k, d.query.k, d.f_key.k, d.f_value.k, d.t_key.k, d.t_value.k};
      for (size_t o : w) add(o, D, TN);
    }
    std::sort(c.dense.begin(), c.dense.end(), [](const Ctx::DenseW& a, const Ctx::DenseW& b) { return a.off < b.off; });
    size_t extra = (pm.word_table != (size_t)-1 ? pm.word_table : pm.total) * 4;
    extra = (extra + 255) & ~(size_t)255;
    for (auto& d : c.dense)
      if (d.K % 128) { d.boff = extra; extra += (size_t)((d.K + 127) / 128) * HUAL_PACK_BLOCK_BYTES; }
    c.wall_K = 4 * embed_cpad(cfg->char_dim);
    c.wall_off = (uint32_t)(extra / 4);
    c.wall_boff = (uint32_t)extra;
    const size_t wf = (size_t)c.wall_K * 512, wb = (size_t)((c.wall_K + 127) / 128) * HUAL_PACK_BLOCK_BYTES;
    extra += wf > wb ? wf : wb;
    c.pk_bytes = extra;
  }
  c.rs.B = B; c.rs.T = T; c.rs.L = L; c.rs.Nv = B * T; c.rs.Nq = B * L; c.rs.R = B * (T + L); c.rs.rowmask = nullptr;
  c.rsv = c.rs; c.rsv.Nq = 0; c.rsv.L = 0; c.rsv.R = c.rs.Nv;
  return 0;
}

struct Res {
  Ctx& c;
  bool make;
  float* operator()(const std::string& name, size_t rows, size_t cols) const { return make ? c.buf(name, rows, cols) : c.find(name); }
  float* act(const std::string& name) const { return (*this)(name, (size_t)c.rs.R, HUAL_D); }
  float* actv(const std::string& name) const { return (*this)(name, (size_t)c.rs.Nv, HUAL_D); }
  float* vec(const std::string& name) const { return (*this)(name, (size_t)c.rs.R, 1); }
  uint8_t* bits(const std::string& name, size_t rows) const { return reinterpret_cast<uint8_t*>((*this)(name, rows, 4)); }
};

struct CoreBufs { float *rowmask, *loss_acc, *ortho_dE; uint32_t* ovf; };
CoreBufs core_bufs(const Res& r) {
  Ctx& c = r.c;
  CoreBufs k{};
  k.rowmask = r.vec("rowmask"); c.rs.rowmask = k.rowmask; c.rsv.rowmask = k.rowmask;
// ... 69 lines not shown
  b.n = da_ln_bufs(r, li);
  b.s_att = r.act(t + ".s_att"); b.x_att = r.act(t + ".x_att");
  for (int k = 0; k < 4; ++k) {
    const bool cross = k & 1, qside = k >= 2, klong = qside != cross;
    AttnJob& a = b.att[k];
    attn_job_init(a);
    a.Q = b.n.qkv; a.ldq = 3 * D; a.B = c.B; a.qmask = c.rs.rowmask; a.kmask = c.rs.rowmask; a.ldo = D;
    a.K = cross ? b.n.ktvt : b.n.qkv + D; a.V = cross ? b.n.ktvt + D : b.n.qkv + 2 * D; a.ldkv = cross ? 2 * D : 3 * D;
    a.Tq = qside ? L : T; a.Tk = klong ? L : T; a.qrow0 = qside ? Nv : 0; a.krow0 = klong ? Nv : 0;
    a.O = cross ? b.x_att : b.s_att; a.drop_site = HUAL_SITE_DA + 8 * li + (cross ? 1 : 0);
    set_dmask(r, a, t + ".dm" + std::to_string(k));
  }
  b.sv = r.act(t + ".s"); b.xv = r.act(t + ".x"); b.sg = r.act(t + ".sg"); b.xg = r.act(t + ".xg"); b.o = r.act(t + ".o");
  b.gd = r.act(t + ".g"); b.gate = r.act(t + ".gate"); b.val = r.act(t + ".val"); b.mha = r.act(t + ".mha"); b.res = r.act(t + ".res");
  b.l2 = r.act(t + ".l2"); b.mean2 = r.vec(t + ".mean2"); b.rstd2 = r.vec(t + ".rstd2"); b.out = r.act(t + ".out");
  b.kb2 = r.bits(t + ".kb2", R); b.kb3 = r.bits(t + ".kb3", R); b.kb4 = r.bits(t + ".kb4", R);
  return b;
}

struct CqStage { CqBufs b; float* feats; };
CqStage cq_bufs(const Res& r, float* x) {
  const Ctx& c = r.c;
  const size_t mat = cq_mat_elems_host(c.T, c.L);
  CqStage q{};
  CqBufs& cq = q.b;
  cq.X = x;
  cq.D1W = r.act("cq.d1w"); cq.D2 = r.act("cq.d2"); cq.S0 = r.vec("cq.s0"); cq.S1 = r.vec("cq.s1");
  cq.C2Q = r.act("cq.c2q"); cq.Q2C = r.act("cq.q2c");
  cq.SR = r("cq.sr", (size_t)2 * c.B, mat); cq.SC = r("cq.sc", (size_t)2 * c.B, mat);
  cq.M2 = r("cq.m2", (size_t)2 * c.B * cq_m2_rows_host(c.T, c.L), HUAL_D);
  cq.GS = cq_fwd_global(c.B, c.T, c.L) ? r("cq.gs", (size_t)2 * c.B, mat) : nullptr;
  q.feats = r.act("cq.feats");
  return q;
}

struct FuseBufs {
  PoolArgs pool;
  AlignPool align;
  float *fuse, *outputs;
  float *probs;
  float *match_part, *d_that, *d_vhat, *align_scratch;
  float *align_rows;
};
FuseBufs fuse_bufs(const Res& r, float* cqf, const hual_labels* lab) {
  const Ctx& c = r.c;
  const int D = HUAL_D, B = c.B;
  FuseBufs f{};
  f.pool.F2 = cqf; f.pool.wp = c.p(c.pm.pool_w); f.pool.Wbot = c.p(c.pm.cqcat.k) + (size_t)D * D;
  f.pool.alpha = r("pool.alpha", B, c.L); f.pool.pooled = r("pool.pooled", B, D); f.pool.PW = r("pool.pw", B, D);
  AlignPool& ap = f.align;
  ap.F2 = cqf; ap.F1 = cqf; ap.inner = (lab && !c.dry) ? lab->inner_labels : nullptr;
  ap.tpre = r("align.tpre", B, D); ap.vpre = r("align.vpre", B, D);
  ap.that = r("align.tv", B, 2 * D); ap.vhat = ap.that + D; ap.ld = 2 * D;
  f.fuse = r.actv("fuse"); f.outputs = r.actv("outputs");
  f.probs = r("match.probs", c.rs.Nv, 4); f.match_part = r("match.part", (size_t)match_fwd_blocks(c.rs.Nv), 2);
  f.d_that = r("d.align.that", B, D); f.d_vhat = r("d.align.vhat", B, D);
  f.align_scratch = r("align.scratch", (size_t)2 * B, B); f.align_rows = r("align.rowloss", B, 1);
  return f;
}
MatchArgs match_args(const Ctx& c, const CoreBufs& k, const FuseBufs& f, const hual_labels* lab, const hual_run_opts* opt) {
  MatchArgs ma{};
  ma.fuse = f.fuse; ma.Wm = c.p(c.pm.match.k); ma.bm = c.p(c.pm.match.b); ma.E = c.p(c.pm.label_emb);
  ma.labels = (lab && !c.dry) ? lab->match_labels : nullptr;
  ma.outputs = f.outputs; ma.loss_acc = k.loss_acc;
  if (!c.cfg->no_gumbel) { ma.rng = opt->rng_state; ma.inv_tau = 1.0f / c.cfg->tau; }
  return ma;
}

struct FeBufs {
  float *x0, *a, *mean, *rstd, *qkv; uint8_t* kb4;
  CbBufs cb;
  float* att; AttnJob job; float *res, *l2, *mean2, *rstd2, *out; uint8_t *kb6, *kb7, *kb8;
};
FeBufs fe_bufs(const Res& r, int ps) {
  const Ctx& c = r.c;
  const int D = HUAL_D, Nv = c.rs.Nv;
  const std::string t = "fe" + std::to_string(ps);
  FeBufs b{};
  b.x0 = r.actv(t + ".x0"); b.a = r.actv(t + ".a");
  b.mean = r(t + ".ln1.mean", Nv, 1); b.rstd = r(t + ".ln1.rstd", Nv, 1);
  b.qkv = r(t + ".qkv", Nv, 3 * D); b.kb4 = r.bits(t + ".kb4", Nv);
  b.cb = cb_bufs(r, t, b.x0, Nv);
  b.att = r.actv(t + ".att");
  AttnJob& a = b.job;
  attn_job_init(a);
  a.Q = b.qkv; a.ldq = 3 * D; a.K = b.qkv + D; a.V = b.qkv + 2 * D; a.ldkv = 3 * D; a.O = b.att; a.ldo = D;
  a.B = c.B; a.Tq = c.T; a.Tk = c.T; a.qrow0 = 0; a.krow0 = 0; a.qmask = c.rs.rowmask; a.kmask = c.rs.rowmask;
  a.drop_site = HUAL_SITE_FE + 16 * ps + 5;
  set_dmask(r, a, t + ".dm");
  b.res = r.actv(t + ".res"); b.l2 = r.actv(t + ".l2");
  b.mean2 = r(t + ".ln2.mean", Nv, 1); b.rstd2 = r(t + ".ln2.rstd", Nv, 1);
  b.out = r.actv(t + ".out");
  b.kb6 = r.bits(t + ".kb6", Nv); b.kb7 = r.bits(t + ".kb7", Nv); b.kb8 = r.bits(t + ".kb8", Nv);
  return b;
}

struct HeadBufs { float *fn[2], *mean, *rstd, *h[2], *d_logit[2], *dz[2], *part[2], *loc_part; };
HeadBufs head_bufs(const Res& r) {
  const Ctx& c = r.c;
  const int D = HUAL_D, Nv = c.rs.Nv, B = c.B;
  HeadBufs b{};
  b.fn[0] = r.actv("head.sfn"); b.fn[1] = r.actv("head.efn");
  b.mean = r("head.mean", (size_t)2 * Nv, 1); b.rstd = r("head.rstd", (size_t)2 * Nv, 1);
  b.h[0] = r.actv("head.hs"); b.h[1] = r.actv("head.he");
  b.d_logit[0] = r("d.s_logit", B, c.T); b.d_logit[1] = r("d.e_logit", B, c.T);
  b.dz[0] = r.actv("d.head.zs"); b.dz[1] = r.actv("d.head.ze");
  b.part[0] = r("head.part.s", (size_t)B * 2, D); b.part[1] = r("head.part.e", (size_t)B * 2, D);
  b.loc_part = r("loc.part", B, 1);
  return b;
}

void fill_da_ln_proj(Ctx& c, LnProjArgs& lp, int li) {
  const int D = HUAL_D;
  const DualAttnP& d = c.pm.da[li];
  const DaLnBufs n = da_ln_bufs(Res{c, true}, li);
  lp = LnProjArgs{};
  lp.g1 = c.p(d.ln1.g); lp.b1 = c.p(d.ln1.b); lp.y1 = n.ln1; lp.drop_site1 = -1; lp.pre_site = -1;
  lp.g2 = c.p(d.lnt.g); lp.b2 = c.p(d.lnt.b); lp.y2 = n.lnt; lp.mean = n.mean; lp.rstd = n.rstd;
  lp.nproj = 5; lp.R = c.rs.R; lp.Nv = c.rs.Nv; lp.MT = ln_proj_rows(c.rs.R, c.rs.Nv); lp.drop_row0 = 0;
  const DenseP* pr[5] = {&d.query, &d.f_key, &d.f_value, &d.t_key, &d.t_value};
  float* outs[5] = {n.qkv, n.qkv + D, n.qkv + 2 * D, n.ktvt, n.ktvt + D};
  for (int k = 0; k < 5; ++k) {
    lp.wimg[k] = c.timg(pr[k]->k); lp.bias[k] = c.p(pr[k]->b); lp.out[k] = outs[k]; lp.ldo[k] = k < 3 ? 3 * D : 2 * D; lp.src[k] = k < 3 ? 0 : 1;
    lp.out_site[k] = -1;
  }
}

bool cb_no_tail() {
  static const bool no_tail = getenv("HUAL_CB_NO_TAIL") != nullptr && atoi(getenv("HUAL_CB_NO_TAIL")) != 0;
  return no_tail;
}

float* conv_block_fwd(Ctx& c, const CbBufs& b, const ConvBlockP& cp, const RowSpace& rs, int site0,
                      const float* pos_src = nullptr, const float* pos = nullptr, LnProjArgs* tail = nullptr, bool* tail_done = nullptr) {
  CbFwdArgs a{};
  a.x0 = pos_src ? pos_src : b.x[0]; a.pos = pos; a.x0_out = pos_src ? b.x[0] : nullptr;
  a.MT = conv_block_fused_rows(rs.R, rs.Nq > 0 ? rs.Nv : 0); a.drop_row0 = 0;
  for (int i = 0; i < 4; ++i) {
    CbLayerFwd& L = a.l[i];
    L.c = b.c[i];
    L.y = c.debug_taps ? b.y[i] : nullptr;
    L.relu_bits = b.rb[i]; L.keep_bits = b.kb[i]; L.xout = b.x[i + 1]; L.mean = b.mean[i]; L.rstd = b.rstd[i];
    L.ln_g = c.p(cp.ln[i].g); L.ln_b = c.p(cp.ln[i].b); L.dw = c.p(cp.dw[i]);
    L.wimg = c.timg(cp.pw[i]); L.bias = c.p(cp.b[i]);
    L.drop_site = site0 + i;
  }
  const bool fuse = tail && c.sel_stage < 0 && !cb_no_tail();
  if (tail) tail->x = b.x[4];
  if (tail_done) *tail_done = fuse;
  if (c.live()) c.chk(launch_conv_block_fwd(a, rs, c.drop, c.stream, fuse ? tail : nullptr));
  return b.x[4];
}

float* conv_block_bwd(Ctx& c, const CbBufs& b, float* dx, const ConvBlockP& cp, const RowSpace& rs) {
  const int R = rs.R;
  const std::string dt = "d." + b.tag;
  CbBwdArgs a{};
  a.dx_in = dx; a.relu_bits3 = b.rb[3]; a.keep_bits3 = b.kb[3];
  a.dx_out = c.buf(dt + ".x0", R, HUAL_D);
  a.MT = conv_block_fused_rows_bwd(R, rs.Nq > 0 ? rs.Nv : 0); a.drop_row0 = 0;
  const int nblk = conv_block_bwd_blocks(R, rs.Nq > 0 ? rs.Nv : 0);
  for (int i = 3; i >= 0; --i) {
    CbLayerBwd& L = a.l[i];
    L.ln_g = c.p(cp.ln[i].g); L.ln_b = c.p(cp.ln[i].b); L.dw = c.p(cp.dw[i]);
    L.wimg_t = c.nimg(cp.pw[i]);
    L.x = b.x[i]; L.mean = b.mean[i]; L.rstd = b.rstd[i];
    L.relu_prev = i > 0 ? b.rb[i - 1] : nullptr; L.keep_prev = i > 0 ? b.kb[i - 1] : nullptr;
    L.dz = c.buf(dt + ".z" + std::to_string(i), R, HUAL_D);
    L.dz_prev = i > 0 ? c.buf(dt + ".z" + std::to_string(i - 1), R, HUAL_D) : nullptr;
    L.part = c.buf("part." + std::to_string(c.part_seq++), (size_t)nblk * 9, HUAL_D);
    ColsumJob cj{};
    cj.src = L.part; cj.nblk = nblk; cj.nvec = 9;
    for (int k = 0; k < 7; ++k) cj.dst[k] = c.g(cp.dw[i]) + k * HUAL_D;
    cj.dst[7] = c.g(cp.ln[i].g); cj.dst[8] = c.g(cp.ln[i].b);
    if (c.active) c.colsum.push_back(cj);
    c.push_dw(mkdw(b.c[i], HUAL_D, HUAL_D, L.dz, HUAL_D, R, c.g(cp.pw[i]), c.g(cp.b[i])));
  }
  if (c.live()) c.chk(launch_conv_block_bwd(a, rs, c.drop, c.stream));
  return a.dx_out;
}


void fwd_prologue(Ctx& c, const CoreBufs& k, const InputBufs& in, EmbedArgs& ea, const hual_batch* bt, const hual_labels* lab,
                  const hual_run_opts* opt) {
  if (c.dry || !c.ok()) return;
  const ParamMap& pm = c.pm;
  std::vector<uint32_t> offs, boffs; std::vector<int> Ks; std::vector<uint8_t> needs;
  for (const auto& d : c.dense) { offs.push_back((uint32_t)d.off); Ks.push_back(d.K); boffs.push_back((uint32_t)d.boff); needs.push_back(d.need); }
  offs.push_back(c.wall_off); Ks.push_back(c.wall_K); boffs.push_back(c.wall_boff);
  needs.push_back(HUAL_PACK_T | HUAL_PACK_N);
  fill_embed_args(c, ea, bt, in.cat, c.catw(), in.char_arg, in.embed_scratch);
  PackExtra ex{};
  ex.lens = bt->video_seq_len; ex.word_ids = bt->word_ids; ex.rowmask = k.rowmask; ex.loss_acc = k.loss_acc; ex.B = c.B; ex.T = c.T; ex.L = c.L;
  ex.zero_ptr = (lab && opt->grads_prezero && opt->prezero_token) ? opt->grads_prezero : nullptr;
  ex.zero_n = (size_t)((pm.total + 3) & ~(size_t)3);
  ex.E = lab ? c.p(pm.label_emb) : nullptr; ex.lambda = c.cfg->match_lambda; ex.dE_ortho = k.ortho_dE;
  ex.gather_tasks = (c.stage_on(ST_INPUT) && c.word_table) ? embed_gather_tasks(ea, c.rs.Nq) : 0;
  ex.gather_rows = c.rs.Nq; ex.emb = ea; ex.drop = c.drop;
  ex.wall_K = c.wall_K; ex.wall_off = c.wall_off; ex.wall_boff = c.wall_boff;
  if (c.novf) { ex.ovf = k.ovf; ex.novf = c.novf; }
  c.chk(launch_pack_weights(offs.data(), Ks.data(), boffs.data(), (int)offs.size(), c.P, c.PKF, c.stream, &ex,
                            c.PKT, c.want_bwd ? c.PKN : nullptr, needs.data()));
  if (opt->prezero_token) *opt->prezero_token = (ex.zero_ptr && c.ok()) ? (uint64_t)(uintptr_t)ex.zero_ptr : 0;
}

void fwd_input(Ctx& c, const InputBufs& in, const EmbedArgs& ea, const hual_batch* bt) {
  const ParamMap& pm = c.pm;
  const int Nv = c.rs.Nv, Nq = c.rs.Nq, R = c.rs.R, D = HUAL_D, catw = c.catw();
  c.stage(ST_INPUT);
  if (!c.live()) return;
  c.chk(launch_embed_fwd(ea, Nq, c.drop, c.stream));
  if (!c.ok()) return;
  float* x = in.x0;
  if (c.ksplit) {
    const int qks = ((catw + 3) / 4 + 63) & ~63;
    float* vpart = in.lin_part;
    FkJob fj[2];
    fj[0] = FkJob{reinterpret_cast<const float*>(bt->video), c.cfg->vdim, Nv, c.cfg->vdim, c.cfg->vdim / 4,
                  reinterpret_cast<const float*>(c.PKF + pm.vconv.k * 4), vpart, (size_t)R * D, HUAL_SITE_VIDEO, 0,
                  bt->video_dtype == HUAL_DTYPE_BF16 ? 1 : 0, c.want_bwd ? in.vkeep : nullptr, (c.cfg->vdim + 7) / 8};
    fj[1] = FkJob{in.cat, catw, Nq, catw, qks, reinterpret_cast<const float*>(c.PKF + pm.qconv.k * 4),
                  vpart + (size_t)Nv * D, (size_t)R * D, -1, 0, 0, nullptr, 0};
    c.chk(launch_feature_ksplit(fj, 2, c.drop, c.stream));
    LnFwd a{};
    a.R = R; a.g1 = c.p(pm.vln.g); a.b1 = c.p(pm.vln.b); a.y1 = x; a.mean = in.lin_mean; a.rstd = in.lin_rstd;
    a.pos = c.p(pm.pos); a.row0 = 0;
    a.split = Nv; a.g1_hi = c.p(pm.qln.g); a.b1_hi = c.p(pm.qln.b);
    a.x = nullptr; a.part = vpart; a.nparts = 4; a.part_stride = (size_t)R * D; a.part_bias = c.p(pm.vconv.b);
    a.part_bias_hi = c.p(pm.qconv.b); a.x_out = in.lin;
    if (c.ok()) c.chk(launch_ln_fwd(a, c.rs, c.drop, c.stream));
    return;
  }
  const int V = c.cfg->vdim;
  MProjArgs pr[2];
  pr[0] = margs(Nv, Nq); pr[0].nsteps = 1;
  pr[0].s[0] = mstep(reinterpret_cast<const float*>(bt->video), V, std::min(V, 128), c.timg(pm.vconv.k), V, true, true);
  pr[0].s[0].a_bf16 = bt->video_dtype == HUAL_DTYPE_BF16 ? 1 : 0;
  pr[0].s[0].rep = cdiv(V, 128); pr[0].s[0].ktot = V;
  pr[0].s[0].drop_site = HUAL_SITE_VIDEO; pr[0].s[0].col0 = 0;
  pr[0].s[0].keep_out = c.want_bwd ? in.vkeep : nullptr; pr[0].s[0].ld_keep = (V + 7) / 8; pr[0].s[0].bias = c.p(pm.vconv.b);
  pr[0].ln_g = c.p(pm.vln.g); pr[0].ln_b = c.p(pm.vln.b); pr[0].pos = c.p(pm.pos); pr[0].row_in_clip0 = 0; pr[0].Tc = c.T;
  pr[0].x_out = in.lin; pr[0].y_out = x; pr[0].mean = in.lin_mean; pr[0].rstd = in.lin_rstd;
  pr[1] = margs(Nq, Nv); pr[1].nsteps = 1;
  pr[1].s[0] = mstep(in.cat, catw, std::min(catw, 128), c.timg(pm.qconv.k), catw, true, true);
  pr[1].s[0].rep = cdiv(catw, 128); pr[1].s[0].ktot = catw; pr[1].s[0].bias = c.p(pm.qconv.b);
  pr[1].ln_g = c.p(pm.qln.g); pr[1].ln_b = c.p(pm.qln.b); pr[1].pos = c.p(pm.pos); pr[1].row_in_clip0 = 0; pr[1].Tc = c.L;
  pr[1].x_out = in.lin + (size_t)Nv * D; pr[1].y_out = x + (size_t)Nv * D; pr[1].mean = in.lin_mean + Nv; pr[1].rstd = in.lin_rstd + Nv;
  c.chk(launch_mproj(pr, 2, c.drop, c.stream));
}

float* fwd_conv(Ctx& c, float* x0, bool& da_lp_done) {
  c.stage(ST_CONV);
  LnProjArgs da0_lp{};
  fill_da_ln_proj(c, da0_lp, 0);
  const CbBufs cb = cb_bufs(Res{c, true}, "cb", x0, c.rs.R);
  return conv_block_fwd(c, cb, c.pm.cb, c.rs, HUAL_SITE_CONV, nullptr, nullptr, &da0_lp, &da_lp_done);
}

float* fwd_da(Ctx& c, int li, float* x, bool& da_lp_done) {
  const DualAttnP& d = c.pm.da[li];
  const int R = c.rs.R, Nv = c.rs.Nv;
  c.stage(ST_DA, li);
  const DaBufs b = da_bufs(Res{c, true}, li);
  if (!da_lp_done) {
    LnProjArgs lp{};
    fill_da_ln_proj(c, lp, li);
    lp.x = x;
    if (c.live()) c.chk(launch_ln_proj(lp, c.drop, c.stream));
  }
  c.attn_fwd(b.att, 4);
  DaPostArgs pa{};
  pa.s_att = b.s_att; pa.x_att = b.x_att; pa.ln1 = b.n.ln1; pa.x = x; pa.rowmask = c.rs.rowmask;
  const size_t wo[11] = {d.s_dense.k, d.x_dense.k, d.s_gate.k, d.x_gate.k, d.guided.k, d.bl1_d1, d.bl1_d2, d.bl2_d1, d.bl2_d2,
                         d.dense1.k, d.dense2.k};
  const size_t bo[9] = {d.s_dense.b, d.x_dense.b, d.s_gate.b, d.x_gate.b, d.guided.b, d.bl1_b, d.bl2_b, d.dense1.b, d.dense2.b};
  for (int k = 0; k < 11; ++k) pa.w[k] = c.timg(wo[k]);
  for (int k = 0; k < 9; ++k) pa.b[k] = c.p(bo[k]);
  pa.ln2_g = c.p(d.ln2.g); pa.ln2_b = c.p(d.ln2.b);
  pa.sv = b.sv; pa.xv = b.xv; pa.sg = b.sg; pa.xg = b.xg; pa.o = b.o; pa.gd = b.gd; pa.gate = b.gate; pa.val = b.val; pa.mha = b.mha;
  pa.res = b.res; pa.l2 = b.l2; pa.out = b.out; pa.mean2 = b.mean2; pa.rstd2 = b.rstd2;
  pa.site = HUAL_SITE_DA + 8 * li; pa.R = R; pa.Nv = Nv; pa.MT = da_post_rows(R, Nv); pa.drop_row0 = 0;
  pa.bits2 = b.kb2; pa.bits3 = b.kb3; pa.bits4 = b.kb4;
  LnProjArgs nlp{};
  const bool fuse = li + 1 < c.cfg->attn_layer && c.sel_stage < 0 && !cb_no_tail();
  if (fuse) { fill_da_ln_proj(c, nlp, li + 1); nlp.x = b.out; }
  if (c.live()) c.chk(launch_da_post(pa, c.drop, c.stream, fuse ? &nlp : nullptr));
  da_lp_done = fuse;
  return b.out;
}

CqStage fwd_cq(Ctx& c, float* x) {
  const ParamMap& pm = c.pm;
  const int Nv = c.rs.Nv, Nq = c.rs.Nq, D = HUAL_D;
  c.stage(ST_CQ);
  const CqStage q = cq_bufs(Res{c, true}, x);
  CqParams cqp{};
  for (int i = 0; i < 2; ++i) { cqp.w0[i] = c.p(pm.cq[i].w0); cqp.w1[i] = c.p(pm.cq[i].w1); cqp.wm[i] = c.p(pm.cq[i].wm); }
  if (c.live()) c.chk(launch_cq_fwd(q.b, cqp, c.rs, c.drop, c.stream));
  if (c.live()) {
    MProjArgs pr[2];
    for (int sd = 0; sd < 2; ++sd) {
      const size_t ro = sd == 0 ? 0 : (size_t)Nv * D;
      pr[sd] = margs(sd == 0 ? Nv : Nq, sd == 0 ? Nq : Nv);
      pr[sd].nsteps = 4;
      const float* a1[4] = {x + ro, q.b.C2Q + ro, x + ro, x + ro};
      const float* a2[4] = {nullptr, nullptr, q.b.C2Q + ro, q.b.Q2C + ro};
      for (int p = 0; p < 4; ++p) {
        pr[sd].s[p] = mstep(a1[p], D, D, c.timg(pm.cq[sd].dense, p), D, p == 0, p == 3);
        pr[sd].s[p].A2 = a2[p]; pr[sd].s[p].lda2 = D;
      }
      mstep_out(pr[sd].s[3], q.feats + ro, D);
    }
    c.chk(launch_mproj(pr, 2, c.drop, c.stream));
  }
  return q;
}

FuseBufs fwd_fuse(Ctx& c, const CoreBufs& k, float* cqf, const hual_labels* lab, const hual_outputs* out, const hual_run_opts* opt) {
  const ParamMap& pm = c.pm;
  const int D = HUAL_D, B = c.B;
  c.stage(ST_FUSE);
  const FuseBufs f = fuse_bufs(Res{c, true}, cqf, lab);
  if (c.live()) c.chk(launch_pool_align_fwd(f.pool, lab ? &f.align : nullptr, c.rs, c.stream));
  if (c.live()) {
    MProjArgs pr = margs(c.rs.Nv); pr.nsteps = 1;
    pr.s[0] = mstep(cqf, D, D, c.timg(pm.cqcat.k), D, true, true);
    mstep_out(pr.s[0], f.fuse, D, c.p(pm.cqcat.b));
    pr.s[0].add = f.pool.PW; pr.s[0].ldadd = D; pr.s[0].add_div = c.T;
    c.chk(launch_mproj(&pr, 1, c.drop, c.stream));
  }
  if (c.live()) {
    MatchArgs ma = match_args(c, k, f, lab, opt);
    ma.probs = out->match_scores;
    ma.probs2 = lab ? f.probs : nullptr;
    ma.part = f.match_part;
    AlignSim as{f.align.that, f.align.vhat, B, f.align_scratch, f.align_scratch + (size_t)B * B, f.align_rows, f.d_that, f.d_vhat,
                k.loss_acc, 1.0f, f.align.ld, 0, B};
    c.chk(launch_match_fwd(ma, c.rs, (lab && !opt->align_external) ? &as : nullptr, c.stream));
  }
  return f;
}

void fill_fe_ln_proj(const Ctx& c, LnProjArgs& lp, const FeBufs& b, int site) {
  const ParamMap& pm = c.pm;
  const int D = HUAL_D;
  lp = LnProjArgs{};
  lp.g1 = c.p(pm.fe_ln1.g); lp.b1 = c.p(pm.fe_ln1.b); lp.y1 = b.a; lp.drop_site1 = site + 4; lp.pre_site = -1; lp.y1_bits = b.kb4;
  lp.mean = b.mean; lp.rstd = b.rstd; lp.nproj = 3; lp.R = c.rs.Nv; lp.MT = ln_proj_rows(c.rs.Nv); lp.drop_row0 = 0;
  const DenseP* pr[3] = {&pm.fe_q, &pm.fe_k, &pm.fe_v};
  for (int k = 0; k < 3; ++k) {
    lp.wimg[k] = c.timg(pr[k]->k); lp.bias[k] = c.p(pr[k]->b); lp.out[k] = b.qkv + k * D; lp.ldo[k] = 3 * D; lp.out_site[k] = -1;
  }
}

float* fwd_fe(Ctx& c, int ps, float* fin) {
  const ParamMap& pm = c.pm;
  const int D = HUAL_D, Nv = c.rs.Nv;
  const int site = HUAL_SITE_FE + 16 * ps;
  const FeBufs b = fe_bufs(Res{c, true}, ps);
  LnProjArgs lp1{};
  fill_fe_ln_proj(c, lp1, b, site);
  bool lp_done = false;
  float* f = conv_block_fwd(c, b.cb, pm.fe_cb, c.rsv, site, fin, c.p(pm.fe_pos), &lp1, &lp_done);
  if (!lp_done && c.live()) c.chk(launch_ln_proj(lp1, c.drop, c.stream));
  c.attn_fwd(&b.job, 1);
  LnProjArgs lp{};
  lp.x = f; lp.xa = b.att; lp.pre_site = site + 6; lp.x_out = b.res;
  lp.pre_bits = b.kb6; lp.y1_bits = b.kb7; lp.out_bits[0] = b.kb8;
  lp.g1 = c.p(pm.fe_ln2.g); lp.b1 = c.p(pm.fe_ln2.b); lp.y1 = b.l2; lp.drop_site1 = site + 7; lp.mean = b.mean2; lp.rstd = b.rstd2;
  lp.nproj = 1; lp.R = Nv; lp.MT = ln_proj_rows(Nv); lp.drop_row0 = 0;
  lp.wimg[0] = c.timg(pm.fe_dense.k); lp.bias[0] = c.p(pm.fe_dense.b); lp.out[0] = b.out; lp.ldo[0] = D; lp.out_site[0] = site + 8; lp.add_x[0] = 1;
  if (c.live()) c.chk(launch_ln_proj(lp, c.drop, c.stream));
  return b.out;
}

void fwd_heads(Ctx& c, const CoreBufs& k, const FuseBufs& fu, float* const feo[2], const hual_labels* lab, const hual_outputs* out,
               const hual_run_opts* opt) {
  const ParamMap& pm = c.pm;
  const int D = HUAL_D, Nv = c.rs.Nv, B = c.B;
  const HeadBufs b = head_bufs(Res{c, true});
  if (!c.live()) return;
  LnProjArgs lp2[2];
  for (int h = 0; h < 2; ++h) {
    const DenseP& hp = h == 0 ? pm.shid : pm.ehid;
    const LnP& lnp = h == 0 ? pm.sln : pm.eln;
    LnProjArgs lp{};
    lp.x = feo[h]; lp.g1 = c.p(lnp.g); lp.b1 = c.p(lnp.b); lp.y1 = b.fn[h]; lp.drop_site1 = -1; lp.pre_site = -1;
    lp.mean = b.mean + (size_t)h * Nv; lp.rstd = b.rstd + (size_t)h * Nv; lp.x2 = fu.outputs;
    lp.nproj = 2; lp.R = Nv; lp.MT = ln_proj_pair_rows(Nv); lp.drop_row0 = 0;
    lp.wimg[0] = c.timg(hp.k, 0); lp.src[0] = 0; lp.accum[0] = 1; lp.out_site[0] = -1;
    lp.wimg[1] = c.timg(hp.k, 1); lp.src[1] = 1; lp.bias[1] = c.p(hp.b);
    lp.act[1] = 1; lp.out[1] = b.h[h]; lp.ldo[1] = D; lp.out_site[1] = -1;
    lp2[h] = lp;
  }
  c.chk(launch_ln_proj_pair(lp2[0], lp2[1], c.drop, c.stream));
  if (!c.ok()) return;
  HeadsArgs ha{};
  ha.h[0] = b.h[0]; ha.h[1] = b.h[1]; ha.w[0] = c.p(pm.sdense.k); ha.w[1] = c.p(pm.edense.k); ha.b[0] = c.p(pm.sdense.b); ha.b[1] = c.p(pm.edense.b);
  ha.logit[0] = out->start_logits; ha.logit[1] = out->end_logits; ha.vmask = k.rowmask;
  ha.y1 = lab ? lab->y1 : nullptr; ha.y2 = lab ? lab->y2 : nullptr;
  ha.start_index = out->start_index; ha.end_index = out->end_index;
  ha.ds = lab ? b.d_logit[0] : nullptr; ha.de = lab ? b.d_logit[1] : nullptr;
  if (lab) { ha.dZ[0] = b.dz[0]; ha.dZ[1] = b.dz[1]; ha.part[0] = b.part[0]; ha.part[1] = b.part[1]; }
  ha.loc_part = b.loc_part; ha.inv_batch = 1.0f / (float)B;
  if (!lab && c.novf) { ha.ovf = k.ovf; ha.novf = c.novf; }
  c.chk(launch_heads(ha, B, c.T, c.stream));
  if (lab && c.ok() && !opt->deferred_loss_terms) {
    LossTailArgs lt{k.loss_acc, fu.match_part, match_fwd_blocks(Nv), b.loc_part, B, c.cfg->match_lambda, opt->match_denom_override,
                    opt->match_denom_dev, out->loss_terms, k.ovf, c.novf, opt->align_external ? nullptr : fu.align_rows, B};
    c.chk(launch_loss_tail(lt, c.stream));
  }
}

int forward_graph(Ctx& c, const hual_batch* bt, const hual_labels* lab, const hual_outputs* out, const hual_run_opts* opt) {
  c.stage(ST_ALWAYS);
  const CoreBufs core = core_bufs(Res{c, true});
  const InputBufs in = input_bufs(Res{c, true});
  EmbedArgs ea{};
  fwd_prologue(c, core, in, ea, bt, lab, opt);
  fwd_input(c, in, ea, bt);
  bool da_lp_done = false;
  float* x = fwd_conv(c, in.x0, da_lp_done);
  for (int li = 0; li < c.cfg->attn_layer; ++li) x = fwd_da(c, li, x, da_lp_done);
  const CqStage cq = fwd_cq(c, x);
  const FuseBufs fu = fwd_fuse(c, core, cq.feats, lab, out, opt);
  c.stage(ST_PRED);
  float* feo[2];
  feo[0] = fwd_fe(c, 0, fu.outputs); feo[1] = fwd_fe(c, 1, feo[0]);
  fwd_heads(c, core, fu, feo, lab, out, opt);
  return c.rc;
}


struct HeadGrads { float *d_fn[2], *d_out; };
HeadGrads bwd_heads(Ctx& c, const HeadBufs& b, float* outputs) {
  const ParamMap& pm = c.pm;
  const int D = HUAL_D, Nv = c.rs.Nv, B = c.B;
  if (c.live() && c.sel_stage >= 0) {
    HeadsArgs ha{};
    ha.grad_only = 1; ha.h[0] = b.h[0]; ha.h[1] = b.h[1]; ha.w[0] = c.p(pm.sdense.k); ha.w[1] = c.p(pm.edense.k); ha.b[0] = c.p(pm.sdense.b); ha.b[1] = c.p(pm.edense.b);
    ha.ds = b.d_logit[0]; ha.de = b.d_logit[1]; ha.dZ[0] = b.dz[0]; ha.dZ[1] = b.dz[1]; ha.part[0] = b.part[0]; ha.part[1] = b.part[1];
    c.chk(launch_heads(ha, B, c.T, c.stream));
  }
  for (int h = 0; h < 2; ++h) {
    ColsumJob cj{};
    cj.src = b.part[h]; cj.nblk = B; cj.nvec = 2; cj.last_ncols = 1;
    cj.dst[0] = c.g(h == 0 ? pm.sdense.k : pm.edense.k); cj.dst[1] = c.g(h == 0 ? pm.sdense.b : pm.edense.b);
    if (c.active) c.colsum.push_back(cj);
    const DenseP& hp = h == 0 ? pm.shid : pm.ehid;
    DwJob j = mkdw(b.fn[h], D, D, b.dz[h], D, Nv, c.g(hp.k), c.g(hp.b));
    j.npieces = 2; j.A[1] = outputs; j.lda[1] = D; j.kw[1] = D; j.dW[1] = c.g(hp.k) + (size_t)D * D;
    c.push_dw(j);
  }
  HeadGrads g{};
  g.d_fn[0] = c.actv("d.head.sfn"); g.d_fn[1] = c.actv("d.head.efn"); g.d_out = c.actv("d.outputs.heads");
  if (c.live()) {
    MProjArgs pr = margs(Nv);
    pr.nsteps = 4;
    pr.s[0] = mstep(b.dz[0], D, D, c.nimg(pm.shid.k, 0), D, true, true);     mstep_out(pr.s[0], g.d_fn[0], D);
    pr.s[1] = mstep_reuse(c.nimg(pm.shid.k, 1), D, true, false);
    pr.s[2] = mstep(b.dz[1], D, D, c.nimg(pm.ehid.k, 1), D, false, true);    mstep_out(pr.s[2], g.d_out, D);
    pr.s[3] = mstep_reuse(c.nimg(pm.ehid.k, 0), D, true, true);             mstep_out(pr.s[3], g.d_fn[1], D);
    c.chk(launch_mproj(&pr, 1, c.drop, c.stream));
  }
  return g;
}

float* bwd_fe(Ctx& c, int ps, const HeadBufs& hd, float* d_fn, float* d_in) {
  const ParamMap& pm = c.pm;
  const int D = HUAL_D, Nv = c.rs.Nv;
  const std::string dt = "d.fe" + std::to_string(ps);
  const FeBufs b = fe_bufs(Res{c, false}, ps);
  float* f = b.cb.x[4];
  float* dzd = c.actv(dt + ".zd");
  c.push_dw(mkdw(b.l2, D, D, dzd, D, Nv, c.g(pm.fe_dense.k), c.g(pm.fe_dense.b)));
  float* d_res = c.actv(dt + ".res");
  float* d_att = c.actv(dt + ".att");
  {
    LnProjBwdArgs lb{};
    const LnP& hl = ps == 1 ? pm.eln : pm.sln;
    lb.pre_x = b.out; lb.pre_mean = hd.mean + (ps == 1 ? Nv : 0); lb.pre_rstd = hd.rstd + (ps == 1 ? Nv : 0);
    lb.pre_g = c.p(hl.g); lb.pre_dy = d_fn; lb.pre_add = ps == 1 ? nullptr : d_in;
    lb.a_bits[0] = b.kb8; lb.a_save[0] = dzd;
    lb.nsteps = 1; lb.A[0] = nullptr; lb.lda[0] = D; lb.wimg_t[0] = c.nimg(pm.fe_dense.k); lb.dst[0] = 0;
    lb.dy1_bits = b.kb7; lb.x = b.res; lb.mean = b.mean2; lb.rstd = b.rstd2; lb.g1 = c.p(pm.fe_ln2.g);
    lb.dx = d_res; lb.dz = d_att; lb.dz_bits = b.kb6; lb.R = Nv; lb.drop_row0 = 0;
    c.ln_proj_bwd(lb, c.g(pm.fe_ln2.g), c.g(pm.fe_ln2.b), c.g(hl.g), c.g(hl.b));
  }
  float* d_qkv = c.buf(dt + ".qkv", Nv, 3 * D);
  AttnJob a = b.job;
  a.dO = d_att; a.lddo = D; a.dQ = d_qkv; a.lddq = 3 * D; a.dK = d_qkv + D; a.dV = d_qkv + 2 * D; a.lddkv = 3 * D;
  c.attn_bwd(&a, 1);
  const DenseP* pr[3] = {&pm.fe_q, &pm.fe_k, &pm.fe_v};
  for (int k = 0; k < 3; ++k) c.push_dw(mkdw(b.a, D, D, d_qkv + k * D, 3 * D, Nv, c.g(pr[k]->k), c.g(pr[k]->b)));
  float* d_f = c.actv(dt + ".x4");
  {
    LnProjBwdArgs lb{};
    lb.nsteps = 3;
    for (int k = 0; k < 3; ++k) { lb.A[k] = d_qkv + k * D; lb.lda[k] = 3 * D; lb.wimg_t[k] = c.nimg(pr[k]->k); lb.dst[k] = 0; }
    lb.dy1_bits = b.kb4; lb.x = f; lb.mean = b.mean; lb.rstd = b.rstd; lb.g1 = c.p(pm.fe_ln1.g); lb.add1 = d_res;
    lb.dx = d_f; lb.R = Nv; lb.drop_row0 = 0;
    c.ln_proj_bwd(lb, c.g(pm.fe_ln1.g), c.g(pm.fe_ln1.b), nullptr, nullptr);
  }
  return conv_block_bwd(c, b.cb, d_f, pm.fe_cb, c.rsv);
}

float* bwd_fuse(Ctx& c, const CoreBufs& k, const FuseBufs& f, const HeadBufs& hd, float* cqf, float* d_in, float* d_out_heads,
                const hual_labels* lab, const hual_run_opts* opt) {
  const ParamMap& pm = c.pm;
  const int D = HUAL_D, Nv = c.rs.Nv, B = c.B;
  c.stage(ST_FUSE);
  float* d_fuse = c.actv("d.fuse");
  float* match_part_b = c.buf("part." + std::to_string(c.part_seq++), (size_t)match_bwd_blocks(Nv) * 9, D);
  ColsumJob cj{};
  cj.src = match_part_b; cj.nblk = match_bwd_blocks(Nv); cj.nvec = 9; cj.last_ncols = 4;
  for (int i = 0; i < 4; ++i) { cj.dst[i] = c.g(pm.label_emb) + i * D; cj.dst[4 + i] = c.g(pm.match.k) + i * D; }
  cj.dst[8] = c.g(pm.match.b);
  if (c.active) c.colsum.push_back(cj);
  if (c.live()) {
    MatchArgs ma = match_args(c, k, f, lab, opt);
    ma.probs = f.probs;
    MatchBwd mb{};
    mb.dOut = d_in; mb.dOut2 = d_out_heads; mb.dFuse = d_fuse; mb.dWm = c.g(pm.match.k); mb.dbm = c.g(pm.match.b); mb.dE = c.g(pm.label_emb);
    mb.lambda = c.cfg->match_lambda;
    mb.dE_ortho = k.ortho_dE;
    mb.part = match_part_b;
    if (opt->deferred_loss_terms && c.sel_stage < 0) {
      mb.do_tail = 1;
      mb.tail = LossTailArgs{k.loss_acc, f.match_part, match_fwd_blocks(Nv), hd.loc_part, B, c.cfg->match_lambda,
                             opt->match_denom_override, opt->match_denom_dev, opt->deferred_loss_terms, k.ovf, c.novf,
                             opt->align_external ? nullptr : f.align_rows, B};
    }
    c.chk(launch_match_bwd(ma, mb, c.rs, c.stream));
  }
  float* d_cqf = c.act("d.cq.feats");
  c.push_dw(mkdw(cqf, D, D, d_fuse, D, Nv, c.g(pm.cqcat.k), c.g(pm.cqcat.b)));
  if (c.live()) {
    MProjArgs pr = margs(Nv); pr.nsteps = 1;
    pr.s[0] = mstep(d_fuse, D, D, c.nimg(pm.cqcat.k), D, true, true);
    mstep_out(pr.s[0], d_cqf, D);
    c.chk(launch_mproj(&pr, 1, c.drop, c.stream));
  }
  float* d_pw = c.buf("d.pool.pw", B, D);
  if (c.live()) {
    AlignPoolBwd ab{f.d_that, f.d_vhat, d_cqf, d_cqf, nullptr, nullptr, 0};
    if (!opt->align_external && c.sel_stage < 0) {
      ab.col_dq = f.align_scratch; ab.col_da = f.align_scratch + (size_t)B * B; ab.col_Bg = B;
    }
    PoolBwd pb{d_fuse, d_pw, d_cqf, c.g(pm.pool_w)};
    c.chk(launch_pool_align_bwd(f.pool, pb, f.align, ab, c.rs, c.stream));
  }
  c.push_dw(mkdw(f.pool.pooled, D, D, d_pw, D, B, c.g(pm.cqcat.k) + (size_t)D * D, nullptr));
  return d_cqf;
}

float* bwd_cq(Ctx& c, const CqStage& q, float* d_cqf) {
  const ParamMap& pm = c.pm;
  const int D = HUAL_D, Nv = c.rs.Nv, Nq = c.rs.Nq, B = c.B, T = c.T, L = c.L;
  const CqBufs& cq = q.b;
  const float* xf = cq.X;
  c.stage(ST_CQ);
  for (int s = 0; s < 2; ++s) {
    const size_t ro = s == 0 ? 0 : (size_t)Nv * D;
    DwJob j = mkdw(xf + ro, D, D, d_cqf + ro, D, s == 0 ? Nv : Nq, c.g(pm.cq[s].dense), nullptr);
    j.npieces = 4;
    const float* a1[4] = {xf + ro, cq.C2Q + ro, xf + ro, xf + ro};
    const float* a2[4] = {nullptr, nullptr, cq.C2Q + ro, cq.Q2C + ro};
    for (int p = 0; p < 4; ++p) {
      j.A[p] = a1[p]; j.A2[p] = a2[p]; j.lda[p] = D; j.lda2[p] = D; j.kw[p] = D;
      j.dW[p] = c.g(pm.cq[s].dense) + (size_t)p * D * D;
    }
    c.push_dw(j);
  }
  CqBwdBufs cg{};
  cg.dCat = nullptr; cg.ldcat = 4 * D; cg.dC2Q = c.act("d.cq.c2q"); cg.dQ2C = c.act("d.cq.q2c"); cg.dX = c.act("d.cq.x");
  if (c.live()) {
    MProjArgs pr[2];
    for (int sd = 0; sd < 2; ++sd) {
      const size_t ro = sd == 0 ? 0 : (size_t)Nv;
      pr[sd] = margs(sd == 0 ? Nv : Nq, sd == 0 ? Nq : Nv);
      pr[sd].nsteps = 4;
      for (int p = 0; p < 4; ++p) {
        const float* img = c.nimg(pm.cq[sd].dense, p);
        pr[sd].s[p] = p == 0 ? mstep(d_cqf + ro * D, D, D, img, D, true, true) : mstep_reuse(img, D, true, true);
      }
      pr[sd].quad_x = xf + ro * D; pr[sd].quad_c2q = cq.C2Q + ro * D; pr[sd].quad_q2c = cq.Q2C + ro * D;
      pr[sd].quad_dc2q = cg.dC2Q + ro * D; pr[sd].quad_dq2c = cg.dQ2C + ro * D; pr[sd].quad_dx = cg.dX + ro * D;
    }
    c.chk(launch_mproj(pr, 2, c.drop, c.stream));
  }
  cg.dD1W = c.act("d.cq.d1w"); cg.dD2 = c.act("d.cq.d2"); cg.dS0 = c.vec("d.cq.s0"); cg.dS1 = c.vec("d.cq.s1");
  cg.dM2 = c.buf("d.cq.m2", (size_t)2 * B * cq_m2_rows_host(T, L), D);
  cg.GD = cq_bwd_global(B, T, L) ? c.buf("d.cq.gd", (size_t)4 * B, cq_mat_elems_host(T, L)) : nullptr;
  float *dXa = c.act("d.cq.xa"), *dXb = c.act("d.cq.xb");
  CqParams cqp{};
  CqGrads cqg{};
  for (int i = 0; i < 2; ++i) {
    cqp.w0[i] = c.p(pm.cq[i].w0); cqp.w1[i] = c.p(pm.cq[i].w1); cqp.wm[i] = c.p(pm.cq[i].wm);
    cqg.w0[i] = c.g(pm.cq[i].w0); cqg.w1[i] = c.g(pm.cq[i].w1); cqg.wm[i] = c.g(pm.cq[i].wm);
  }
  const int tri_nv = tri_bwd_blocks_v(c.rs), tri_nq = tri_bwd_blocks_q(c.rs);
  float* tri_part = c.buf("part." + std::to_string(c.part_seq++), (size_t)(tri_nv + tri_nq) * 3, D);
  for (int side = 0; side < 2; ++side) {
    ColsumJob cj{};
    cj.src = tri_part + (side == 0 ? 0 : (size_t)tri_nv * 3 * D); cj.nblk = side == 0 ? tri_nv : tri_nq; cj.nvec = 3;
    cj.dst[0] = cqg.wm[side]; cj.dst[1] = cqg.w0[side]; cj.dst[2] = cqg.w1[1 - side];
    if (c.active) c.colsum.push_back(cj);
  }
  if (c.live()) {
    c.chk(launch_cq_bwd_impl(cq, cg, c.rs, dXa, dXb, c.stream));
    if (c.ok()) c.chk(launch_tri_bwd_impl(cq, cg, cqp, tri_part, c.rs, c.drop, dXa, dXb, c.stream));
  }
  return cg.dX;
}

float* bwd_da(Ctx& c, int li, float* dx) {
  const DualAttnP& d = c.pm.da[li];
  const int D = HUAL_D, R = c.rs.R, Nv = c.rs.Nv;
  const Res r{c, false};
  c.stage(ST_DA, li);
  const DaBufs b = da_bufs(r, li);
  float* xin = li == 0 ? r.act("cb.x4") : r.act("da" + std::to_string(li - 1) + ".out");
  const std::string dt = "d.da" + std::to_string(li);
  float* dz2 = c.act(dt + ".z2");
  c.push_dw(mkdw(b.l2, D, D, dz2, D, R, c.g(d.dense2.k), c.g(d.dense2.b)));
  float *d_res = c.act(dt + ".res"), *dz1 = c.act(dt + ".z1"), *d_sc = c.act(dt + ".sc"), *d_val = c.act(dt + ".val");
  float *d_ln1a = c.act(dt + ".ln1a"), *d_g = c.act(dt + ".g"), *dz_sg = c.act(dt + ".zsg"), *dz_xg = c.act(dt + ".zxg");
  float *d_sv = c.act(dt + ".s"), *d_xv = c.act(dt + ".x"), *d_satt = c.act(dt + ".s_att"), *d_xatt = c.act(dt + ".x_att");
  const bool dz2_ready = li < c.cfg->attn_layer - 1 && c.sel_stage < 0;
  c.push_dw(mkdw(b.mha, D, D, dz1, D, R, c.g(d.dense1.k), c.g(d.dense1.b)));
  for (int k = 0; k < 2; ++k) {
    DwJob j = mkdw(b.n.ln1, D, D, k == 0 ? d_sc : d_val, D, R, c.g(k == 0 ? d.bl1_d1 : d.bl2_d1), c.g(k == 0 ? d.bl1_b : d.bl2_b));
    j.npieces = 2; j.A[1] = b.gd; j.lda[1] = D; j.kw[1] = D; j.dW[1] = c.g(k == 0 ? d.bl1_d2 : d.bl2_d2);
    c.push_dw(j);
  }
  c.push_dw(mkdw(b.o, D, D, d_g, D, R, c.g(d.guided.k), c.g(d.guided.b)));
  c.push_dw(mkdw(b.sv, D, D, dz_sg, D, R, c.g(d.s_gate.k), c.g(d.s_gate.b)));
  c.push_dw(mkdw(b.xv, D, D, dz_xg, D, R, c.g(d.x_gate.k), c.g(d.x_gate.b)));
  c.push_dw(mkdw(b.s_att, D, D, d_sv, D, R, c.g(d.s_dense.k), c.g(d.s_dense.b)));
  c.push_dw(mkdw(b.x_att, D, D, d_xv, D, R, c.g(d.x_dense.k), c.g(d.x_dense.b)));
  {
    LnProjBwdArgs lb{};
    lb.nsteps = 1; lb.lda[0] = D; lb.wimg_t[0] = c.nimg(d.dense2.k); lb.dst[0] = 0;
    if (dz2_ready) { lb.A[0] = dz2; }
    else { lb.A[0] = dx; lb.a_bits[0] = b.kb4; lb.a_save[0] = dz2; }
    lb.dy1_bits = b.kb3; lb.x = b.res; lb.mean = b.mean2; lb.rstd = b.rstd2; lb.g1 = c.p(d.ln2.g); lb.add1 = dx;
    lb.dx = d_res; lb.dz = dz1; lb.dz_bits = b.kb2; lb.R = R; lb.Nv = Nv; lb.drop_row0 = 0;
    DaMidBwdArgs mb{};
    mb.dz1 = dz1; mb.gate = b.gate; mb.val = b.val; mb.sg = b.sg; mb.xg = b.xg; mb.sv = b.sv; mb.xv = b.xv;
    const size_t wo[10] = {d.dense1.k, d.bl1_d1, d.bl2_d1, d.bl1_d2, d.bl2_d2, d.guided.k, d.s_gate.k, d.x_gate.k, d.s_dense.k, d.x_dense.k};
    for (int k = 0; k < 10; ++k) mb.w[k] = c.nimg(wo[k]);
    mb.d_sc = d_sc; mb.d_val = d_val; mb.d_ln1a = d_ln1a; mb.d_g = d_g; mb.dz_sg = dz_sg; mb.dz_xg = dz_xg; mb.d_sv = d_sv; mb.d_xv = d_xv;
    mb.d_satt = d_satt; mb.d_xatt = d_xatt; mb.R = R; mb.Nv = Nv;
    c.ln2_mid_bwd(lb, mb, c.g(d.ln2.g), c.g(d.ln2.b));
  }
  float *dq_self = c.act(dt + ".q_self"), *dq_cross = c.act(dt + ".q_cross");
  float *d_qkv = c.buf(dt + ".qkv", R, 3 * D), *d_ktvt = c.buf(dt + ".ktvt", R, 2 * D);
  AttnJob a[4];
  for (int k = 0; k < 4; ++k) {
    const bool cross = k & 1;
    a[k] = b.att[k];
    a[k].lddo = D; a[k].lddq = D; a[k].dO = cross ? d_xatt : d_satt; a[k].dQ = cross ? dq_cross : dq_self;
    a[k].dK = cross ? d_ktvt : d_qkv + D; a[k].dV = cross ? d_ktvt + D : d_qkv + 2 * D; a[k].lddkv = cross ? 2 * D : 3 * D;
  }
  c.attn_bwd(a, 4);
  const float* As[6] = {dq_self, dq_cross, d_qkv + D, d_qkv + 2 * D, d_ktvt, d_ktvt + D};
  const int lds_[6] = {D, D, 3 * D, 3 * D, 2 * D, 2 * D};
  const DenseP* pr[6] = {&d.query, &d.query, &d.f_key, &d.f_value, &d.t_key, &d.t_value};
  for (int k = 0; k < 6; ++k) c.push_dw(mkdw(k < 4 ? b.n.ln1 : b.n.lnt, D, D, As[k], lds_[k], R, c.g(pr[k]->k), c.g(pr[k]->b)));
  float* d_xin = c.act(dt + ".in");
  float* nz = nullptr; const uint8_t* nz_bits = nullptr;
  if (li > 0) { nz = c.act("d.da" + std::to_string(li - 1) + ".z2"); nz_bits = r.bits("da" + std::to_string(li - 1) + ".kb4", R); }
  {
    LnProjBwdArgs lb{};
    lb.nsteps = 6;
    for (int k = 0; k < 6; ++k) { lb.A[k] = As[k]; lb.lda[k] = lds_[k]; lb.wimg_t[k] = c.nimg(pr[k]->k); lb.dst[k] = k < 4 ? 0 : 1; }
    lb.add_dy1 = d_ln1a; lb.x = xin; lb.mean = b.n.mean; lb.rstd = b.n.rstd; lb.g1 = c.p(d.ln1.g); lb.g2 = c.p(d.lnt.g);
    lb.add1 = d_res; lb.dx = d_xin; lb.dz = nz; lb.dz_bits = nz_bits; lb.R = R; lb.Nv = Nv; lb.drop_row0 = 0;
    c.ln_proj_bwd(lb, c.g(d.ln1.g), c.g(d.ln1.b), c.g(d.lnt.g), c.g(d.lnt.b));
  }
  return d_xin;
}

bool bwd_input(Ctx& c, const InputBufs& in, float* d_x0, float* const fe_dx0[2], const hual_batch* bt, EmbedArgs& ea, EmbedGrads& eg) {
  const ParamMap& pm = c.pm;
  const int D = HUAL_D, Nv = c.rs.Nv, Nq = c.rs.Nq, catw = c.catw();
  c.stage(ST_ALWAYS);
  PosBwdJob pj[2];
  int npj = 0;
  if (!c.dry && c.stage_on(ST_INPUT)) pj[npj++] = PosBwdJob{{d_x0, nullptr}, c.g(pm.pos), 1, 1};
  if (!c.dry && c.stage_on(ST_PRED)) pj[npj++] = PosBwdJob{{fe_dx0[1], fe_dx0[0]}, c.g(pm.fe_pos), 1, 0};
  const bool pos_rides = c.sel_stage < 0;
  if (c.live() && npj && !pos_rides) c.chk(launch_pos_bwd(pj, npj, c.rs, c.stream));
  c.stage(ST_INPUT);
  float* d_lin = c.act("d.lin");
  LnBwd a{};
  a.x = in.lin; a.mean = in.lin_mean; a.rstd = in.lin_rstd; a.R = c.rs.R; a.dy1 = d_x0; a.g1 = c.p(pm.vln.g);
  a.dx = d_lin; a.split = Nv; a.g1_hi = c.p(pm.qln.g);
  c.ln_bwd_split(a, c.g(pm.vln.g), c.g(pm.vln.b), c.g(pm.qln.g), c.g(pm.qln.b), pj, pos_rides ? npj : 0);
  DwJob j = mkdw(c.dry ? nullptr : reinterpret_cast<const float*>(bt->video), c.cfg->vdim, c.cfg->vdim, d_lin, D, Nv, c.g(pm.vconv.k), c.g(pm.vconv.b));
  j.a_drop_site = HUAL_SITE_VIDEO; j.a_drop_row0 = 0;
  j.a_bf16 = (!c.dry && bt->video_dtype == HUAL_DTYPE_BF16) ? 1 : 0;
  j.a_keep = in.vkeep; j.ld_keep = (c.cfg->vdim + 7) / 8;
  c.push_dw(j);
  c.push_dw(mkdw(in.cat, catw, catw, d_lin + (size_t)Nv * D, D, Nq, c.g(pm.qconv.k), c.g(pm.qconv.b)));
  float* d_cat = c.buf("d.cat", Nq, catw);
  if (c.live()) {
    if (cdiv(catw, 128) > MP_MAX) { c.chk(fail(-1, "invalid argument: internal: query_conv1d image")); return c.active; }
    MProjArgs pr = margs(Nq);
    pr.nsteps = cdiv(catw, 128);
    for (int p = 0; p < pr.nsteps; ++p) {
      const float* img = c.nimg(pm.qconv.k, p);
      pr.s[p] = p == 0 ? mstep(d_lin + (size_t)Nv * D, D, D, img, D, true, true) : mstep_reuse(img, D, true, true);
      mstep_out(pr.s[p], d_cat + (size_t)p * D, catw, nullptr, std::min(D, catw - p * D));
    }
    c.chk(launch_mproj(&pr, 1, c.drop, c.stream));
  }
  set_embed_scratch(ea, in.embed_scratch, Nq, c.C, c.cfg->char_dim);
  ea.word_dim = c.cfg->word_dim; ea.char_dim = c.cfg->char_dim; ea.C = c.C; ea.num_chars = c.cfg->num_chars;
  DwJob embed_dw;
  embed_dw_job(ea, Nq, &embed_dw);
  if (c.live()) {
    fill_embed_args(c, ea, bt, in.cat, catw, in.char_arg, in.embed_scratch);
    eg.dcat = d_cat; eg.lddcat = catw; eg.dunk = c.g(pm.unk); eg.dchar_table = c.g(pm.char_table);
    if (pm.word_table != (size_t)-1) { eg.dword_table = c.g(pm.word_table); eg.dword_rows = c.cfg->num_words - 2; }
    for (int i = 0; i < 4; ++i) { eg.dfilt[i] = c.g(pm.filt[i]); eg.dfbias[i] = c.g(pm.fbias[i]); }
    c.chk(launch_embed_bwd(ea, eg, Nq, c.drop, c.stream, &embed_dw, false));
  }
  c.push_dw(embed_dw);
  return c.active;
}

void bwd_flush(Ctx& c, const EmbedArgs& ea, const EmbedGrads& eg, bool input_ran) {
  c.stage(ST_ALWAYS);
  flush_dw(c);
  EmbedUnpack eu{};
  const bool unpack = !c.dry && input_ran && c.active;
  if (unpack) {
    eu.a = ea; eu.g = eg; eu.CP = embed_unpack_cpad(ea); eu.ntasks = embed_unpack_tasks(ea);
    eu.finish_blocks = embed_finish_blocks(ea, c.rs.Nq); eu.finish_lds = embed_finish_lds(ea); eu.nrows = c.rs.Nq; eu.drop = c.drop;
  }
  c.flush_colsum(unpack ? &eu : nullptr);
}

int backward_graph(Ctx& c, const hual_batch* bt, const hual_labels* lab, const hual_run_opts* opt) {
  const Res r{c, false};
  c.dwjobs.clear(); c.colsum.clear(); c.part_seq = 0;
  c.stage(ST_ALWAYS);
  const CoreBufs core = core_bufs(r);
  const InputBufs in = input_bufs(r);
  const CqStage cq = cq_bufs(r, r.act("da" + std::to_string(c.cfg->attn_layer - 1) + ".out"));
  const FuseBufs fu = fuse_bufs(r, cq.feats, lab);
  const HeadBufs hd = head_bufs(r);
  {
    const bool prezeroed = !c.dry && opt->prezero_token && *opt->prezero_token == (uint64_t)(uintptr_t)c.G && c.sel_stage < 0;
    if (!c.dry && opt->prezero_token) *opt->prezero_token = 0;
    if (c.live() && !prezeroed) c.chk(launch_zero(c.G, c.pm.total, c.stream));
  }
  c.stage(ST_PRED);
  const HeadGrads hg = bwd_heads(c, hd, fu.outputs);
  float* fe_dx0[2] = {nullptr, nullptr};
  fe_dx0[1] = bwd_fe(c, 1, hd, hg.d_fn[1], nullptr);
  fe_dx0[0] = bwd_fe(c, 0, hd, hg.d_fn[0], fe_dx0[1]);
  float* d_cqf = bwd_fuse(c, core, fu, hd, cq.feats, fe_dx0[0], hg.d_out, lab, opt);
  float* dx = bwd_cq(c, cq, d_cqf);
  for (int li = c.cfg->attn_layer - 1; li >= 0; --li) dx = bwd_da(c, li, dx);
  c.stage(ST_CONV);
  float* d_x0 = conv_block_bwd(c, cb_bufs(r, "cb", in.x0, c.rs.R), dx, c.pm.cb, c.rs);
  EmbedArgs ea{}; EmbedGrads eg{};
  const bool input_ran = bwd_input(c, in, d_x0, fe_dx0, bt, ea, eg);
  bwd_flush(c, ea, eg, input_ran);
  return c.rc;
}

int plan(Ctx& c, const hual_cfg* cfg, int B, int T, int L, int C) {
  int rc = setup_ctx(c, cfg, B, T, L, C);
  if (rc) return rc;
  c.dry = true;
  c.base = nullptr;
  hual_run_opts o{};
  rc = forward_graph(c, nullptr, nullptr, nullptr, &o);
  if (rc) return rc;
  return backward_graph(c, nullptr, nullptr, &o);
}

}

extern "C" {

int hual_seqpan_validate(const hual_cfg* cfg) {
  HUAL_REQUIRE(cfg != nullptr, "null cfg");
  return validate_cfg(*cfg);
}

#define HUAL_DW_TABLE_JOBS 256
uint64_t hual_seqpan_dw_table_bytes(void) { return 4 * dw_table_words(HUAL_DW_TABLE_JOBS); }

int hual_seqpan_param_count(const hual_cfg* cfg, uint64_t* padded_floats, uint64_t* count) {
  HUAL_REQUIRE(cfg != nullptr, "null cfg");
  ParamMap pm;
  int rc = build_param_map(*cfg, pm);
  if (rc) return rc;
  if (padded_floats) *padded_floats = pm.total;
  if (count) *count = pm.count;
  return 0;
}

int hual_seqpan_param_table(const hual_cfg* cfg, hual_param_entry* out, int max_entries) {
  HUAL_REQUIRE(cfg != nullptr, "null cfg");
  ParamMap pm;
  int rc = build_param_map(*cfg, pm);
  if (rc) return rc;
  const int n = (int)pm.entries.size();
  for (int i = 0; i < n && i < max_entries && out; ++i) {
    const ParamEntry& e = pm.entries[i];
    memset(&out[i], 0, sizeof(out[i]));
    strncpy(out[i].name, e.name.c_str(), sizeof(out[i].name) - 1);
    out[i].offset = e.off; out[i].size = e.size; out[i].ndim = e.ndim; out[i].decay = e.decay;
    for (int k = 0; k < 4; ++k) out[i].shape[k] = e.shape[k];
  }
  return n;
}

int hual_seqpan_query_workspace(const hual_cfg* cfg, int B, int T, int L, int C, uint64_t* bytes) {
  HUAL_REQUIRE(bytes != nullptr, "null bytes");
  Ctx c;
  int rc = plan(c, cfg, B, T, L, C);
  if (rc) return rc;
  *bytes = c.used + 4096;
  return 0;
}

int hual_seqpan_ws_table(const hual_cfg* cfg, int B, int T, int L, int C, hual_ws_entry* out, int max_entries) {
  Ctx c;
  int rc = plan(c, cfg, B, T, L, C);
  if (rc) return rc;
  const int n = (int)c.entries.size();
  for (int i = 0; i < n && i < max_entries && out; ++i) {
    memset(&out[i], 0, sizeof(out[i]));
    strncpy(out[i].name, c.entries[i].name.c_str(), sizeof(out[i].name) - 1);
    out[i].offset = c.entries[i].off; out[i].rows = c.entries[i].rows; out[i].cols = c.entries[i].cols;
  }
  return n;
}

static int resolve_word_table(const Ctx& c, const float* params, const float* word_table, bool required, const float** out) {
  if (c.pm.word_table == (size_t)-1) {
    HUAL_REQUIRE(!required || word_table != nullptr, "null word_table");
    *out = word_table;
    return 0;
  }
  const float* own = params + c.pm.word_table;
  HUAL_REQUIRE(word_table == nullptr || word_table == own,
               "model.finetune_word_emb: word_table must be NULL or the address of the params entry word_embs/word_table");
  *out = own;
  return 0;
}

static int open_live(Ctx& c, const hual_cfg* cfg, const float* params, const float* word_table, bool need_table, const hual_batch* batch,
                     const hual_run_opts* opts, float* grads, void* workspace, uint64_t ws_bytes, void* stream) {
  int rc = plan(c, cfg, batch->B, batch->T, batch->L, batch->C);
  if (rc) return rc;
  if (c.used + 4096 > ws_bytes) return fail(HUAL_ERR_WORKSPACE, "workspace too small: call hual_seqpan_query_workspace");
  c.dry = false;
  c.base = (char*)workspace;
  c.stream = (hipStream_t)stream;
  c.P = params;
  c.G = grads;
  c.drop = make_dropcfg(opts->rng_state, opts->drop_rate);
  c.debug_taps = opts->debug_taps != 0;
  return resolve_word_table(c, params, word_table, need_table, &c.word_table);
}

static int check_common(const hual_cfg* cfg, const float* params, const hual_batch* batch, const hual_run_opts* opts,
                        void* workspace) {
  HUAL_REQUIRE(cfg && params && batch && opts && workspace, "null argument");
  HUAL_REQUIRE(batch->video && batch->video_seq_len && batch->word_ids && batch->char_ids, "null batch tensor");
  HUAL_REQUIRE(batch->video_dtype == HUAL_DTYPE_F32 || batch->video_dtype == HUAL_DTYPE_BF16, "video_dtype: HUAL_DTYPE_F32 or HUAL_DTYPE_BF16");
  HUAL_REQUIRE(((uintptr_t)batch->video & 15) == 0, "video features must be 16-byte aligned");
  HUAL_REQUIRE(opts->drop_rate >= 0.f && opts->drop_rate < 1.f, "drop_rate in [0,1)");
  HUAL_REQUIRE(opts->drop_rate == 0.f || opts->rng_state != nullptr, "rng_state required when drop_rate > 0");
  HUAL_REQUIRE(cfg->no_gumbel || opts->rng_state != nullptr, "rng_state required when loss.no_gumbel is false");
  HUAL_REQUIRE(((uintptr_t)workspace & 255) == 0 && ((uintptr_t)params & 15) == 0, "workspace/params alignment");
  return 0;
}

int hual_seqpan_forward(const hual_cfg* cfg, const float* params, const float* word_table, const hual_batch* batch,
                        const hual_labels* labels, const hual_outputs* out, const hual_run_opts* opts, void* workspace,
                        uint64_t ws_bytes, void* stream) {
  int rc = check_common(cfg, params, batch, opts, workspace);
  if (rc) return rc;
  HUAL_REQUIRE(out && out->start_logits && out->end_logits && out->match_scores && out->start_index && out->end_index,
               "null output tensor");
  if (labels) HUAL_REQUIRE(labels->y1 && labels->y2 && labels->match_labels && labels->inner_labels, "null label tensor");
  Ctx c;
  if ((rc = open_live(c, cfg, params, word_table, true, batch, opts, nullptr, workspace, ws_bytes, stream))) return rc;
  c.want_bwd = labels != nullptr;
  return forward_graph(c, batch, labels, out, opts);
}

int hual_seqpan_backward(const hual_cfg* cfg, const float* params, const float* word_table, const hual_batch* batch,
                         const hual_labels* labels, const hual_run_opts* opts, float* grads, void* workspace,
                         uint64_t ws_bytes, void* stream) {
  int rc = check_common(cfg, params, batch, opts, workspace);
  if (rc) return rc;
  HUAL_REQUIRE(grads != nullptr && ((uintptr_t)grads & 15) == 0, "null/unaligned grads");
  HUAL_REQUIRE(labels && labels->y1 && labels->y2 && labels->match_labels && labels->inner_labels, "null label tensor");
  Ctx c;
  if ((rc = open_live(c, cfg, params, word_table, false, batch, opts, grads, workspace, ws_bytes, stream))) return rc;
  c.static_tables = opts->static_tables != 0;
  HUAL_REQUIRE(!opts->dw_table || ((uintptr_t)opts->dw_table & 15) == 0, "unaligned hual_run_opts.dw_table");
  c.ext_table = opts->dw_table;
  c.ext_table_bytes = (size_t)opts->dw_table_bytes;
  return backward_graph(c, batch, labels, opts);
}

// ... 165 lines not shown
```

Measured before the change: 53960 clips/s.

## Fuse feature-encoder conv-block backward with the next LN-proj backward as a tail

```diff
diff --git a/hual_amd/csrc/convblock.h b/hual_amd/csrc/convblock.h
--- a/hual_amd/csrc/convblock.h
+++ b/hual_amd/csrc/convblock.h
@@ -48,6 +48,8 @@
 #define HUAL_CB_BWD_MAXMT 40
 int conv_block_fused_rows_bwd(int R, int Nv = 0);
 int conv_block_bwd_blocks(int R, int Nv = 0);
-int launch_conv_block_bwd(const CbBwdArgs& a, const RowSpace& rs, const DropCfg& drop, hipStream_t s);
+struct LnProjBwdArgs;
+bool conv_block_bwd_tail_fits(const CbBwdArgs& a, const RowSpace& rs, const LnProjBwdArgs& tail);
+int launch_conv_block_bwd(const CbBwdArgs& a, const RowSpace& rs, const DropCfg& drop, hipStream_t s, const LnProjBwdArgs* tail = nullptr);
 
 }
diff --git a/hual_amd/csrc/convblock.hip b/hual_amd/csrc/convblock.hip
--- a/hual_amd/csrc/convblock.hip
+++ b/hual_amd/csrc/convblock.hip
@@ -5,6 +5,7 @@
 using namespace hual;
 
 #include "lnproj_body.h"
+#include "lnproj_bwd_body.h"
 
 #define CB_XS 33
 #define CB_NPAR 10
@@ -247,8 +248,8 @@
   conv_block_fwd_body<true>(a, rs, drop, &lp, cb_lds);
 }
 
-__global__ __launch_bounds__(CB_THREADS) void conv_block_bwd_kernel(CbBwdArgs a, RowSpace rs, DropCfg drop) {
-  extern __shared__ __attribute__((aligned(16))) char cb_lds[];
+template <int TAIL_NT>
+__device__ __forceinline__ void conv_block_bwd_body(const CbBwdArgs& a, const RowSpace& rs, const DropCfg& drop, const LnProjBwdArgs* lb, char* cb_lds) {
   const int MT = a.MT;
   const int XR = MT + 24;
   float4* DX = reinterpret_cast<float4*>(cb_lds);
@@ -453,6 +454,19 @@
     }
     HUAL_STAMP_K(3, 8 + 7 * (3 - i));
   }
+  if constexpr (TAIL_NT > 0) {
+    float4 zv[LB_U];
+    ln_proj_bwd_body<true, TAIL_NT, false, false, true>(*lb, drop, cb_lds, nullptr, nullptr, zv, tile_, r0, DX + 12 * 32);
+  }
+}
+__global__ __launch_bounds__(CB_THREADS) void conv_block_bwd_kernel(CbBwdArgs a, RowSpace rs, DropCfg drop) {
+  extern __shared__ __attribute__((aligned(16))) char cb_lds[];
+  conv_block_bwd_body<0>(a, rs, drop, nullptr, cb_lds);
+}
+template <int NT>
+__global__ __launch_bounds__(CB_THREADS) void conv_block_bwd_lnbwd_kernel(CbBwdArgs a, RowSpace rs, DropCfg drop, LnProjBwdArgs lb) {
+  extern __shared__ __attribute__((aligned(16))) char cb_lds[];
+  conv_block_bwd_body<NT>(a, rs, drop, &lb, cb_lds);
 }
 
 #if defined(HUAL_STAMPS) && (HUAL_STAMPS == 2 || HUAL_STAMPS == 3 || HUAL_STAMPS == 7)
@@ -509,17 +523,40 @@
 
 static size_t cb_bwd_lds(int MT) { return (size_t)(MT + 24) * 512 + 64 * 512 + 64 * sizeof(float) + (1 + 4) * 9 * HUAL_D * sizeof(float); }
 
-int launch_conv_block_bwd(const CbBwdArgs& a, const RowSpace& rs, const DropCfg& drop, hipStream_t s) {
+bool conv_block_bwd_tail_fits(const CbBwdArgs& a, const RowSpace& rs, const LnProjBwdArgs& t) {
+  return t.pre_x && !t.g2 && !t.add_dy1 && t.pre_add && t.pre_add == a.dx_out && t.R == rs.R && t.Nv == (rs.Nq > 0 ? rs.Nv : 0) && t.MT == a.MT;
+}
+
+int launch_conv_block_bwd(const CbBwdArgs& a, const RowSpace& rs, const DropCfg& drop, hipStream_t s, const LnProjBwdArgs* tail) {
   HUAL_REQUIRE(a.dx_in && a.relu_bits3 && a.keep_bits3 && a.dx_out && rs.R > 0 && a.MT >= 1 && a.MT <= HUAL_CB_BWD_MAXMT, "conv_block_bwd: bad arguments");
   for (int l = 0; l < 4; ++l) {
     const CbLayerBwd& L = a.l[l];
     HUAL_REQUIRE(L.ln_g && L.ln_b && L.dw && L.wimg_t && L.x && L.mean && L.rstd && L.dz && L.part, "conv_block_bwd: null layer tensor");
     HUAL_REQUIRE(l == 0 || (L.relu_prev && L.keep_prev && L.dz_prev), "conv_block_bwd: layers 1-3 need the bit planes of the layer below / dz_prev");
   }
-  HUAL_DYN_LDS(conv_block_bwd_kernel, 160 * 1024);
   const double rows = (double)rs.R;
-  HUAL_LAUNCH(4.0 * 2.0 * rows * HUAL_D * HUAL_D, 4.0 * (rows * HUAL_D * 14.0 + 4.0 * HUAL_D * HUAL_D), conv_block_bwd_kernel,
-              dim3(xcd_clip_grid(rs.R, rs.Nq > 0 ? rs.Nv : 0, a.MT)), dim3(CB_THREADS), cb_bwd_lds(a.MT), s, a, rs, drop);
+  double flops = 4.0 * 2.0 * rows * HUAL_D * HUAL_D, bytes = 4.0 * (rows * HUAL_D * 14.0 + 4.0 * HUAL_D * HUAL_D);
+  const dim3 grid(xcd_clip_grid(rs.R, rs.Nq > 0 ? rs.Nv : 0, a.MT));
+  if (!tail) {
+    HUAL_DYN_LDS(conv_block_bwd_kernel, 160 * 1024);
+    HUAL_LAUNCH(flops, bytes, conv_block_bwd_kernel, grid, dim3(CB_THREADS), cb_bwd_lds(a.MT), s, a, rs, drop);
+    HUAL_CHECK_HIP(hipGetLastError());
+    return 0;
+  }
+  int rc = check_ln_proj_bwd_args(*tail);
+  if (rc) return rc;
+  HUAL_REQUIRE(conv_block_bwd_tail_fits(a, rs, *tail), "conv_block_bwd: the tail must take dx_out as its prologue's addend, on the same rows and row tiles");
+  static_assert(HUAL_CB_BWD_MAXMT <= LB_ROWS, "the tail's row layout must hold the block's tile");
+  const size_t lds = std::max(cb_bwd_lds(a.MT), (size_t)LB_LDS);
+  flops += 2.0 * rows * HUAL_D * HUAL_D * tail->nsteps;
+  bytes += 4.0 * (rows * HUAL_D * (7.0 + tail->nsteps) + (double)tail->nsteps * HUAL_D * HUAL_D) - 4.0 * rows * HUAL_D;
+#define CB_BWD_TAIL(NT) { HUAL_DYN_LDS(conv_block_bwd_lnbwd_kernel<NT>, 160 * 1024); HUAL_LAUNCH(flops, bytes, conv_block_bwd_lnbwd_kernel<NT>, grid, dim3(CB_THREADS), lds, s, a, rs, drop, *tail); break; }
+  switch (cdiv(a.MT, 16)) {
+    case 1: CB_BWD_TAIL(1)
+    case 2: CB_BWD_TAIL(2)
+    default: CB_BWD_TAIL(3)
+  }
+#undef CB_BWD_TAIL
   HUAL_CHECK_HIP(hipGetLastError());
   return 0;
 }
diff --git a/hual_amd/csrc/dablock.h b/hual_amd/csrc/dablock.h
--- a/hual_amd/csrc/dablock.h
+++ b/hual_amd/csrc/dablock.h
@@ -79,6 +79,7 @@
 int ln_proj_bwd_rows(int R, int Nv = 0);
 int ln_proj_bwd_blocks(int R, int Nv = 0);
 int launch_ln_proj_bwd(const LnProjBwdArgs& a, const DropCfg& drop, hipStream_t s);
+int check_ln_proj_bwd_args(const LnProjBwdArgs& a);
 
 struct DaMidBwdArgs {
   const float* dz1;
diff --git a/hual_amd/csrc/dablock.hip b/hual_amd/csrc/dablock.hip
--- a/hual_amd/csrc/dablock.hip
+++ b/hual_amd/csrc/dablock.hip
@@ -307,244 +307,7 @@
   da_post_body<NT, true>(a, drop, &lp, dp_lds);
 }
 
-#define LB_ROWS 48
-#define LB_U (LB_ROWS / 16)
-template <int NT> struct DaMidPre { TfW wa, wb; float4 gate[NT], val[NT]; };
-#define LB_LDS ((size_t)4 * LB_ROWS * 256 + 8 * 4 * 32 * 16 + 2 * LB_ROWS * sizeof(float))
-template <bool PRE, int NT, bool SIX, bool MID>
-__device__ __forceinline__ bool ln_proj_bwd_body(const LnProjBwdArgs& a, const DropCfg& drop, char* lb_lds, const DaMidBwdArgs* m,
-                                                 DaMidPre<NT>* mp, float4 (&zv)[LB_U]) {
-  char* S0 = lb_lds;
-  char* S1 = S0 + 2 * LB_ROWS * 256;
-  char* Ps = S1 + 2 * LB_ROWS * 256;
-  float* ainv0 = reinterpret_cast<float*>(Ps + 8 * 4 * 32 * 16);
-  float* ainv1 = ainv0 + LB_ROWS;
-  const int lane = threadIdx.x & 63, wave = threadIdx.x >> 6;
-  const int l32 = threadIdx.x & 31, grp = threadIdx.x >> 5;
-  const int col = 4 * l32;
-  const int MT = a.MT, R = a.R;
-  const int tile_ = xcd_tile_clip(blockIdx.x, R, a.Nv, MT);
-  if (tile_ < 0) return false;
-  const int r0 = tile_ * MT;
-  const int RE = min(R, r0 + MT);
-  const int j = lane & 15, g = lane >> 4, ecol = 16 * wave + 4 * g;
-  const DropRegs dr = drop_load(drop);
-
-  TfW w[2];
-  tf_load_w(w[0], a.wimg_t[0], wave, lane);
-  float4 nv[LB_U], xv[LB_U], a1v[LB_U];
-  float mu[LB_U], rsd[LB_U];
-  constexpr bool pre = PRE;
-  const float* add1p = pre ? (a.pre_add ? a.pre_add : a.x) : (a.add1 ? a.add1 : a.x);
-  const float* a0p = pre ? a.pre_dy : a.A[0];
-  const int lda0 = pre ? HUAL_D : a.lda[0];
-  uint32_t nkb[LB_U];
-  const int nsteps = SIX ? 6 : (MID ? 1 : a.nsteps);
-  auto has_bits = [&](int k) { return !SIX && a.a_bits[k] != nullptr; };
-  auto to_second = [&](int k) { return SIX ? k >= 4 : a.dst[k] != 0; };
-  const bool has_g2 = SIX || (!MID && a.g2 != nullptr), has_add_dy1 = SIX || (!MID && a.add_dy1 != nullptr), has_dy1_bits = !SIX && a.dy1_bits != nullptr;
-  const uint8_t* kb0p = has_bits(0) ? a.a_bits[0] : reinterpret_cast<const uint8_t*>(a.x);
-  float4 pxv[LB_U];
-  float pmu[LB_U], prs[LB_U];
-#pragma unroll
-  for (int u = 0; u < LB_U; ++u) {
-    const int row = min(r0 + grp + 16 * u, R - 1);
-    nv[u] = ld4(a0p + (size_t)row * lda0 + col);
-    nkb[u] = SIX ? 0u : kb0p[(size_t)row * 16 + (l32 >> 1)];
-    xv[u] = ld4(a.x + (size_t)row * HUAL_D + col);
-    a1v[u] = ld4(add1p + (size_t)row * HUAL_D + col);
-    mu[u] = a.mean[row];
-    rsd[u] = a.rstd[row];
-    if (pre) { pxv[u] = ld4(a.pre_x + (size_t)row * HUAL_D + col); pmu[u] = a.pre_mean[row]; prs[u] = a.pre_rstd[row]; }
-  }
-  const float4 g1 = ld4(a.g1 + col);
-  float4 sg2 = f4zero(), sb2 = f4zero();
-  if (pre) {
-    const float4 pg = ld4(a.pre_g + col);
-#pragma unroll
-    for (int u = 0; u < LB_U; ++u) {
-      const int lr = grp + 16 * u;
-      const bool ok = lr < MT && r0 + lr < RE;
-      const float4 v = pxv[u], dy = nv[u];
-      const float mean = pmu[u], rstd = prs[u];
-      const float4 xh = make_float4((v.x - mean) * rstd, (v.y - mean) * rstd, (v.z - mean) * rstd, (v.w - mean) * rstd);
-      if (ok) { sb2 = cb_add(sb2, dy); sg2 = cb_fma(dy, xh, sg2); }
-      const float4 gv = cb_mul(dy, pg);
-      const float m1 = fast_sum32(cb_hsum(gv)) * (1.0f / HUAL_D);
-      const float m2 = fast_sum32(cb_hsum(cb_mul(gv, xh))) * (1.0f / HUAL_D);
-      float4 dx = make_float4(rstd * (gv.x - m1 - xh.x * m2), rstd * (gv.y - m1 - xh.y * m2),
-                              rstd * (gv.z - m1 - xh.z * m2), rstd * (gv.w - m1 - xh.w * m2));
-      if (a.pre_add) dx = make_float4(__fadd_rn(dx.x, a1v[u].x), __fadd_rn(dx.y, a1v[u].y), __fadd_rn(dx.z, a1v[u].z), __fadd_rn(dx.w, a1v[u].w));
-      nv[u] = dx;
-      a1v[u] = dx;
-    }
-  }
-  const float4 g2 = has_g2 ? ld4(a.g2 + col) : f4zero();
-  float4 addt[NT];
-  const float* addp = has_add_dy1 ? a.add_dy1 : a.x;
-#pragma unroll
-  for (int rt = 0; rt < NT; ++rt) addt[rt] = (SIX || MID) ? f4zero() : ld4(addp + (uint32_t)min(r0 + 16 * rt + j, R - 1) * (uint32_t)HUAL_D + (uint32_t)ecol);
-  auto fill = [&](int k) {
-    char* S = (k & 1) ? S1 : S0;
-    float* ai = (k & 1) ? ainv1 : ainv0;
-#pragma unroll
-    for (int u = 0; u < LB_U; ++u) {
-      const int lr = grp + 16 * u, row = r0 + lr;
-      if (lr >= MT) continue;
-      const bool ok = row < RE;
-      float4 v = ok ? nv[u] : f4zero();
-      if (has_bits(k)) {
-        if (dr.enabled) v = f4_select((nkb[u] >> (4 * (l32 & 1))) & 15u, make_float4(v.x * dr.scale, v.y * dr.scale, v.z * dr.scale, v.w * dr.scale));
-        if (ok && a.a_save[k]) st4_nt(a.a_save[k] + (size_t)row * HUAL_D + col, v);
-      }
-      const float inv = cb_store_operand(S, S + LB_ROWS * 256, lr, l32, v);
-      if (l32 == 0) ai[lr] = ok ? inv : 0.f;
-    }
-  };
-  HUAL_STAMP_K(4, 0);
-  fill(0);
-  HUAL_STAMP_K(4, 1);
-  float4 acc0[NT], acc1[NT];
-  bool first0 = true, first1 = true;
-#pragma unroll
-  for (int rt = 0; rt < NT; ++rt) { acc0[rt] = f4zero(); acc1[rt] = f4zero(); }
-#pragma unroll
-  for (int k = 0; k < HUAL_LNBWD_MAX; ++k) {
-    if (k >= nsteps) break;
-    const bool more = k + 1 < nsteps;
-    if (SIX && k == 5) {
-#pragma unroll
-      for (int rt = 0; rt < NT; ++rt) addt[rt] = ld4(addp + (uint32_t)min(r0 + 16 * rt + j, R - 1) * (uint32_t)HUAL_D + (uint32_t)ecol);
-    }
-    if (more) {
-      const uint8_t* nbp = has_bits(k + 1) ? a.a_bits[k + 1] : reinterpret_cast<const uint8_t*>(a.x);
-      const float* nap = a.A[k + 1];
-      const int nld = a.lda[k + 1];
-#pragma unroll
-      for (int u = 0; u < LB_U; ++u) {
-        const size_t row = (size_t)min(r0 + grp + 16 * u, R - 1);
-        nv[u] = ld4(nap + row * nld + col);
-        nkb[u] = SIX ? 0u : nbp[row * 16 + (l32 >> 1)];
-      }
-      tf_load_w(w[(k + 1) & 1], a.wimg_t[k + 1], wave, lane);
-    }
-    cb_barrier();
-    HUAL_STAMP_K(4, 2 + 3 * k);
-    const char* S = (k & 1) ? S1 : S0;
-    const float* ai = (k & 1) ? ainv1 : ainv0;
-    f32x4 accp[NT];
-    tf_mma_lean<NT, LB_ROWS * 256>(S, w[k & 1], lane, accp);
-    HUAL_STAMP_K(4, 3 + 3 * k);
-    {
-      const bool to1 = to_second(k);
-      const bool first = to1 ? first1 : first0;
-#pragma unroll
-      for (int rt = 0; rt < NT; ++rt) {
-        const float ir = ai[16 * rt + j];
-        const float4 o = to1 ? acc1[rt] : acc0[rt];
-        const float4 n = first ? make_float4(fmaf(accp[rt][0], ir, 0.f), fmaf(accp[rt][1], ir, 0.f), fmaf(accp[rt][2], ir, 0.f), fmaf(accp[rt][3], ir, 0.f))
-                               : make_float4(fmaf(accp[rt][0], ir, o.x), fmaf(accp[rt][1], ir, o.y), fmaf(accp[rt][2], ir, o.z), fmaf(accp[rt][3], ir, o.w));
-        if (to1) acc1[rt] = n; else acc0[rt] = n;
-      }
-    }
-    if (to_second(k)) first1 = false; else first0 = false;
-    if (more) fill(k + 1);
-    HUAL_STAMP_K(4, 4 + 3 * k);
-  }
-  cb_barrier();
-  HUAL_STAMP_K(4, 20);
-  float4* D0 = reinterpret_cast<float4*>(S0);
-  float4* D1 = reinterpret_cast<float4*>(S1);
-#pragma unroll
-  for (int rt = 0; rt < NT; ++rt) {
-    const int lr = 16 * rt + j;
-    float4 v = acc0[rt];
-    if (has_add_dy1) v = cb_add(v, addt[rt]);
-    D0[lr * 32 + (ecol >> 2)] = v;
-    if (has_g2) D1[lr * 32 + (ecol >> 2)] = acc1[rt];
-  }
-  uint32_t kb1[LB_U], kbz[LB_U];
-  {
-    const uint8_t* b1p = has_dy1_bits ? a.dy1_bits : reinterpret_cast<const uint8_t*>(a.x);
-    const uint8_t* bzp = a.dz_bits ? a.dz_bits : reinterpret_cast<const uint8_t*>(a.x);
-#pragma unroll
-    for (int u = 0; u < LB_U; ++u) {
-      const size_t row = (size_t)min(r0 + grp + 16 * u, R - 1);
-      kb1[u] = SIX ? 0u : b1p[row * 16 + (l32 >> 1)];
-      kbz[u] = bzp[row * 16 + (l32 >> 1)];
-    }
-  }
-  if (MID) {
-    tf_load_w(mp->wa, m->w[0], wave, lane);
-    tf_load_w(mp->wb, m->w[1], wave, lane);
-#pragma unroll
-    for (int rt = 0; rt < NT; ++rt) {
-      const uint32_t eo = (uint32_t)min(r0 + 16 * rt + j, R - 1) * (uint32_t)HUAL_D + (uint32_t)ecol;
-      mp->gate[rt] = ld4(m->gate + eo);
-      mp->val[rt] = ld4(m->val + eo);
-    }
-#pragma unroll
-    for (int u = 0; u < LB_U; ++u) zv[u] = f4zero();
-  }
-  cb_barrier();
-  HUAL_STAMP_K(4, 21);
-  float4 sg1 = f4zero(), sb1 = f4zero();
-#pragma unroll
-  for (int u = 0; u < LB_U; ++u) {
-    const int lr = grp + 16 * u, row = r0 + lr;
-    if (lr >= MT || row >= R) continue;
-    const size_t off = (size_t)row * HUAL_D + col;
-    const float4 v = xv[u];
-    const float mean = mu[u], rstd = rsd[u];
-    const float4 xh = make_float4((v.x - mean) * rstd, (v.y - mean) * rstd, (v.z - mean) * rstd, (v.w - mean) * rstd);
-    float4 dy = D0[lr * 32 + l32];
-    if (has_dy1_bits && dr.enabled) dy = f4_select((kb1[u] >> (4 * (l32 & 1))) & 15u, make_float4(dy.x * dr.scale, dy.y * dr.scale, dy.z * dr.scale, dy.w * dr.scale));
-    sb1 = cb_add(sb1, dy);
-    sg1 = cb_fma(dy, xh, sg1);
-    float4 gv = cb_mul(dy, g1);
-    if (has_g2) {
-      const float4 dy2 = D1[lr * 32 + l32];
-      sb2 = cb_add(sb2, dy2);
-      sg2 = cb_fma(dy2, xh, sg2);
-      gv = cb_fma(dy2, g2, gv);
-    }
-    const float m1 = fast_sum32(cb_hsum(gv)) * (1.0f / HUAL_D);
-    const float m2 = fast_sum32(cb_hsum(cb_mul(gv, xh))) * (1.0f / HUAL_D);
-    float4 dx = make_float4(rstd * (gv.x - m1 - xh.x * m2), rstd * (gv.y - m1 - xh.y * m2),
-                            rstd * (gv.z - m1 - xh.z * m2), rstd * (gv.w - m1 - xh.w * m2));
-    if (SIX || a.add1 || pre) dx = make_float4(__fadd_rn(dx.x, a1v[u].x), __fadd_rn(dx.y, a1v[u].y), __fadd_rn(dx.z, a1v[u].z), __fadd_rn(dx.w, a1v[u].w));
-    st4(a.dx + off, dx);
-    if (a.dz) {
-      if (a.dz_bits && dr.enabled) dx = f4_select((kbz[u] >> (4 * (l32 & 1))) & 15u, make_float4(dx.x * dr.scale, dx.y * dr.scale, dx.z * dr.scale, dx.w * dr.scale));
-      st4(a.dz + off, dx);
-      if (MID) zv[u] = dx;
-    }
-  }
-  HUAL_STAMP_K(4, 22);
-  {
-    auto xor32_sum = [&](float v) {
-      const unsigned x = __builtin_bit_cast(unsigned, v);
-      const auto r = __builtin_amdgcn_permlane32_swap(x, x, false, false);
-      return v + __builtin_bit_cast(float, (lane & 32) ? r[0] : r[1]);
-    };
-    auto xor32_sum4 = [&](float4 v) { return make_float4(xor32_sum(v.x), xor32_sum(v.y), xor32_sum(v.z), xor32_sum(v.w)); };
-    sg1 = xor32_sum4(sg1); sb1 = xor32_sum4(sb1); sg2 = xor32_sum4(sg2); sb2 = xor32_sum4(sb2);
-    float4* pb = reinterpret_cast<float4*>(Ps);
-    if (lane < 32) {
-      float4* dst = pb + wave * 4 * 32 + l32;
-      dst[0] = sg1; dst[32] = sb1; dst[64] = sg2; dst[96] = sb2;
-    }
-    cb_barrier();
-    const float* pf = reinterpret_cast<const float*>(pb);
-    const int e = threadIdx.x;
-    float s = 0.f;
-#pragma unroll
-    for (int w = 0; w < 8; ++w) s += pf[w * 4 * HUAL_D + e];
-    a.part[(size_t)tile_ * 4 * HUAL_D + e] = s;
-  }
-  HUAL_STAMP_K(4, 23);
-  return true;
-}
+#include "lnproj_bwd_body.h"
 template <bool PRE, int NT, bool SIX = false>
 __global__ __launch_bounds__(CB_THREADS) void ln_proj_bwd_kernel(LnProjBwdArgs a, DropCfg drop) {
   extern __shared__ __attribute__((aligned(16))) char lb_lds[];
@@ -915,6 +678,7 @@
   HUAL_REQUIRE(!a.pre_x || (!a.g2 && !a.add1 && a.pre_mean && a.pre_rstd && a.pre_g && a.pre_dy), "ln_proj_bwd: layer-norm prologue");
   return 0;
 }
+int check_ln_proj_bwd_args(const LnProjBwdArgs& a) { return check_ln_proj_bwd(a); }
 static void ln_proj_bwd_work(const LnProjBwdArgs& a, double& flops, double& bytes) {
   const double rows = (double)a.R;
   flops += 2.0 * rows * HUAL_D * HUAL_D * a.nsteps;
diff --git a/hual_amd/csrc/lnproj_bwd_body.h b/hual_amd/csrc/lnproj_bwd_body.h
--- /dev/null
+++ b/hual_amd/csrc/lnproj_bwd_body.h
@@ -0,0 +1,245 @@
+#pragma once
+#include "dablock.h"
+#include "tilecore.h"
+
+#define LB_ROWS 48
+#define LB_U (LB_ROWS / 16)
+template <int NT> struct DaMidPre { TfW wa, wb; float4 gate[NT], val[NT]; };
+#define LB_LDS ((size_t)4 * LB_ROWS * 256 + 8 * 4 * 32 * 16 + 2 * LB_ROWS * sizeof(float))
+template <bool PRE, int NT, bool SIX, bool MID, bool TAILED = false>
+__device__ __forceinline__ bool ln_proj_bwd_body(const LnProjBwdArgs& a, const DropCfg& drop, char* lb_lds, const DaMidBwdArgs* m,
+                                                 DaMidPre<NT>* mp, float4 (&zv)[LB_U], const int tile_f = 0, const int r0f = 0,
+                                                 const float4* dxl = nullptr) {
+  static_assert(!TAILED || (PRE && !SIX && !MID), "the tail form is the prologue form");
+  char* S0 = lb_lds;
+  char* S1 = S0 + 2 * LB_ROWS * 256;
+  char* Ps = S1 + 2 * LB_ROWS * 256;
+  float* ainv0 = reinterpret_cast<float*>(Ps + 8 * 4 * 32 * 16);
+  float* ainv1 = ainv0 + LB_ROWS;
+  const int lane = threadIdx.x & 63, wave = threadIdx.x >> 6;
+  const int l32 = threadIdx.x & 31, grp = threadIdx.x >> 5;
+  const int col = 4 * l32;
+  const int MT = a.MT, R = a.R;
+  const int tile_ = TAILED ? tile_f : xcd_tile_clip(blockIdx.x, R, a.Nv, MT);
+  if (tile_ < 0) return false;
+  const int r0 = TAILED ? r0f : tile_ * MT;
+  const int RE = min(R, r0 + MT);
+  const int j = lane & 15, g = lane >> 4, ecol = 16 * wave + 4 * g;
+  const DropRegs dr = drop_load(drop);
+
+  TfW w[2];
+  tf_load_w(w[0], a.wimg_t[0], wave, lane);
+  float4 nv[LB_U], xv[LB_U], a1v[LB_U];
+  float mu[LB_U], rsd[LB_U];
+  constexpr bool pre = PRE;
+  const float* add1p = pre ? (a.pre_add ? a.pre_add : a.x) : (a.add1 ? a.add1 : a.x);
+  const float* a0p = pre ? a.pre_dy : a.A[0];
+  const int lda0 = pre ? HUAL_D : a.lda[0];
+  uint32_t nkb[LB_U];
+  const int nsteps = SIX ? 6 : (MID ? 1 : a.nsteps);
+  auto has_bits = [&](int k) { return !SIX && a.a_bits[k] != nullptr; };
+  auto to_second = [&](int k) { return SIX ? k >= 4 : a.dst[k] != 0; };
+  const bool has_g2 = SIX || (!MID && !TAILED && a.g2 != nullptr), has_add_dy1 = SIX || (!MID && !TAILED && a.add_dy1 != nullptr), has_dy1_bits = !SIX && a.dy1_bits != nullptr;
+  const uint8_t* kb0p = has_bits(0) ? a.a_bits[0] : reinterpret_cast<const uint8_t*>(a.x);
+  float4 pxv[LB_U];
+  float pmu[LB_U], prs[LB_U];
+#pragma unroll
+  for (int u = 0; u < LB_U; ++u) {
+    const int row = min(r0 + grp + 16 * u, R - 1);
+    nv[u] = ld4(a0p + (size_t)row * lda0 + col);
+    nkb[u] = SIX ? 0u : kb0p[(size_t)row * 16 + (l32 >> 1)];
+    xv[u] = ld4(a.x + (size_t)row * HUAL_D + col);
+    a1v[u] = TAILED ? dxl[min(grp + 16 * u, MT - 1) * 32 + l32] : ld4(add1p + (size_t)row * HUAL_D + col);
+    mu[u] = a.mean[row];
+    rsd[u] = a.rstd[row];
+    if (pre) { pxv[u] = ld4(a.pre_x + (size_t)row * HUAL_D + col); pmu[u] = a.pre_mean[row]; prs[u] = a.pre_rstd[row]; }
+  }
+  const float4 g1 = ld4(a.g1 + col);
+  float4 sg2 = f4zero(), sb2 = f4zero();
+  if (pre) {
+    const float4 pg = ld4(a.pre_g + col);
+#pragma unroll
+    for (int u = 0; u < LB_U; ++u) {
+      const int lr = grp + 16 * u;
+      const bool ok = lr < MT && r0 + lr < RE;
+      const float4 v = pxv[u], dy = nv[u];
+      const float mean = pmu[u], rstd = prs[u];
+      const float4 xh = make_float4((v.x - mean) * rstd, (v.y - mean) * rstd, (v.z - mean) * rstd, (v.w - mean) * rstd);
+      if (ok) { sb2 = cb_add(sb2, dy); sg2 = cb_fma(dy, xh, sg2); }
+      const float4 gv = cb_mul(dy, pg);
+      const float m1 = fast_sum32(cb_hsum(gv)) * (1.0f / HUAL_D);
+      const float m2 = fast_sum32(cb_hsum(cb_mul(gv, xh))) * (1.0f / HUAL_D);
+      float4 dx = make_float4(rstd * (gv.x - m1 - xh.x * m2), rstd * (gv.y - m1 - xh.y * m2),
+                              rstd * (gv.z - m1 - xh.z * m2), rstd * (gv.w - m1 - xh.w * m2));
+      if (TAILED || a.pre_add) dx = make_float4(__fadd_rn(dx.x, a1v[u].x), __fadd_rn(dx.y, a1v[u].y), __fadd_rn(dx.z, a1v[u].z), __fadd_rn(dx.w, a1v[u].w));
+      nv[u] = dx;
+      a1v[u] = dx;
+    }
+  }
+  const float4 g2 = has_g2 ? ld4(a.g2 + col) : f4zero();
+  float4 addt[NT];
+  const float* addp = has_add_dy1 ? a.add_dy1 : a.x;
+#pragma unroll
+  for (int rt = 0; rt < NT; ++rt) addt[rt] = (SIX || MID || TAILED) ? f4zero() : ld4(addp + (uint32_t)min(r0 + 16 * rt + j, R - 1) * (uint32_t)HUAL_D + (uint32_t)ecol);
+  auto fill = [&](int k) {
+    char* S = (k & 1) ? S1 : S0;
+    float* ai = (k & 1) ? ainv1 : ainv0;
+#pragma unroll
+    for (int u = 0; u < LB_U; ++u) {
+      const int lr = grp + 16 * u, row = r0 + lr;
+      if (lr >= MT) continue;
+      const bool ok = row < RE;
+      float4 v = ok ? nv[u] : f4zero();
+      if (has_bits(k)) {
+        if (dr.enabled) v = f4_select((nkb[u] >> (4 * (l32 & 1))) & 15u, make_float4(v.x * dr.scale, v.y * dr.scale, v.z * dr.scale, v.w * dr.scale));
+        if (ok && a.a_save[k]) st4_nt(a.a_save[k] + (size_t)row * HUAL_D + col, v);
+      }
+      const float inv = cb_store_operand(S, S + LB_ROWS * 256, lr, l32, v);
+      if (l32 == 0) ai[lr] = ok ? inv : 0.f;
+    }
+  };
+  HUAL_STAMP_K(4, 0);
+  if (TAILED) cb_barrier();
+  fill(0);
+  HUAL_STAMP_K(4, 1);
+  float4 acc0[NT], acc1[NT];
+  bool first0 = true, first1 = true;
+#pragma unroll
+  for (int rt = 0; rt < NT; ++rt) { acc0[rt] = f4zero(); acc1[rt] = f4zero(); }
+#pragma unroll
+  for (int k = 0; k < HUAL_LNBWD_MAX; ++k) {
+    if (k >= nsteps) break;
+    const bool more = k + 1 < nsteps;
+    if (SIX && k == 5) {
+#pragma unroll
+      for (int rt = 0; rt < NT; ++rt) addt[rt] = ld4(addp + (uint32_t)min(r0 + 16 * rt + j, R - 1) * (uint32_t)HUAL_D + (uint32_t)ecol);
+    }
+    if (more) {
+      const uint8_t* nbp = has_bits(k + 1) ? a.a_bits[k + 1] : reinterpret_cast<const uint8_t*>(a.x);
+      const float* nap = a.A[k + 1];
+      const int nld = a.lda[k + 1];
+#pragma unroll
+      for (int u = 0; u < LB_U; ++u) {
+        const size_t row = (size_t)min(r0 + grp + 16 * u, R - 1);
+        nv[u] = ld4(nap + row * nld + col);
+        nkb[u] = SIX ? 0u : nbp[row * 16 + (l32 >> 1)];
+      }
+      tf_load_w(w[(k + 1) & 1], a.wimg_t[k + 1], wave, lane);
+    }
+    cb_barrier();
+    HUAL_STAMP_K(4, 2 + 3 * k);
+    const char* S = (k & 1) ? S1 : S0;
+    const float* ai = (k & 1) ? ainv1 : ainv0;
+    f32x4 accp[NT];
+    tf_mma_lean<NT, LB_ROWS * 256>(S, w[k & 1], lane, accp);
+    HUAL_STAMP_K(4, 3 + 3 * k);
+    {
+      const bool to1 = to_second(k);
+      const bool first = to1 ? first1 : first0;
+#pragma unroll
+      for (int rt = 0; rt < NT; ++rt) {
+        const float ir = ai[16 * rt + j];
+        const float4 o = to1 ? acc1[rt] : acc0[rt];
+        const float4 n = first ? make_float4(fmaf(accp[rt][0], ir, 0.f), fmaf(accp[rt][1], ir, 0.f), fmaf(accp[rt][2], ir, 0.f), fmaf(accp[rt][3], ir, 0.f))
+                               : make_float4(fmaf(accp[rt][0], ir, o.x), fmaf(accp[rt][1], ir, o.y), fmaf(accp[rt][2], ir, o.z), fmaf(accp[rt][3], ir, o.w));
+        if (to1) acc1[rt] = n; else acc0[rt] = n;
+      }
+    }
+    if (to_second(k)) first1 = false; else first0 = false;
+    if (more) fill(k + 1);
+    HUAL_STAMP_K(4, 4 + 3 * k);
+  }
+  cb_barrier();
+  HUAL_STAMP_K(4, 20);
+  float4* D0 = reinterpret_cast<float4*>(S0);
+  float4* D1 = reinterpret_cast<float4*>(S1);
+#pragma unroll
+  for (int rt = 0; rt < NT; ++rt) {
+    const int lr = 16 * rt + j;
+    float4 v = acc0[rt];
+    if (has_add_dy1) v = cb_add(v, addt[rt]);
+    D0[lr * 32 + (ecol >> 2)] = v;
+    if (has_g2) D1[lr * 32 + (ecol >> 2)] = acc1[rt];
+  }
+  uint32_t kb1[LB_U], kbz[LB_U];
+  {
+    const uint8_t* b1p = has_dy1_bits ? a.dy1_bits : reinterpret_cast<const uint8_t*>(a.x);
+    const uint8_t* bzp = a.dz_bits ? a.dz_bits : reinterpret_cast<const uint8_t*>(a.x);
+#pragma unroll
+    for (int u = 0; u < LB_U; ++u) {
+      const size_t row = (size_t)min(r0 + grp + 16 * u, R - 1);
+      kb1[u] = SIX ? 0u : b1p[row * 16 + (l32 >> 1)];
+      kbz[u] = bzp[row * 16 + (l32 >> 1)];
+    }
+  }
+  if (MID) {
+    tf_load_w(mp->wa, m->w[0], wave, lane);
+    tf_load_w(mp->wb, m->w[1], wave, lane);
+#pragma unroll
+    for (int rt = 0; rt < NT; ++rt) {
+      const uint32_t eo = (uint32_t)min(r0 + 16 * rt + j, R - 1) * (uint32_t)HUAL_D + (uint32_t)ecol;
+      mp->gate[rt] = ld4(m->gate + eo);
+      mp->val[rt] = ld4(m->val + eo);
+    }
+#pragma unroll
+    for (int u = 0; u < LB_U; ++u) zv[u] = f4zero();
+  }
+  cb_barrier();
+  HUAL_STAMP_K(4, 21);
+  float4 sg1 = f4zero(), sb1 = f4zero();
+#pragma unroll
+  for (int u = 0; u < LB_U; ++u) {
+    const int lr = grp + 16 * u, row = r0 + lr;
+    if (lr >= MT || row >= R) continue;
+    const size_t off = (size_t)row * HUAL_D + col;
+    const float4 v = xv[u];
+    const float mean = mu[u], rstd = rsd[u];
+    const float4 xh = make_float4((v.x - mean) * rstd, (v.y - mean) * rstd, (v.z - mean) * rstd, (v.w - mean) * rstd);
+    float4 dy = D0[lr * 32 + l32];
+    if (has_dy1_bits && dr.enabled) dy = f4_select((kb1[u] >> (4 * (l32 & 1))) & 15u, make_float4(dy.x * dr.scale, dy.y * dr.scale, dy.z * dr.scale, dy.w * dr.scale));
+    sb1 = cb_add(sb1, dy);
+    sg1 = cb_fma(dy, xh, sg1);
+    float4 gv = cb_mul(dy, g1);
+    if (has_g2) {
+      const float4 dy2 = D1[lr * 32 + l32];
+      sb2 = cb_add(sb2, dy2);
+      sg2 = cb_fma(dy2, xh, sg2);
+      gv = cb_fma(dy2, g2, gv);
+    }
+    const float m1 = fast_sum32(cb_hsum(gv)) * (1.0f / HUAL_D);
+    const float m2 = fast_sum32(cb_hsum(cb_mul(gv, xh))) * (1.0f / HUAL_D);
+    float4 dx = make_float4(rstd * (gv.x - m1 - xh.x * m2), rstd * (gv.y - m1 - xh.y * m2),
+                            rstd * (gv.z - m1 - xh.z * m2), rstd * (gv.w - m1 - xh.w * m2));
+    if (SIX || a.add1 || pre) dx = make_float4(__fadd_rn(dx.x, a1v[u].x), __fadd_rn(dx.y, a1v[u].y), __fadd_rn(dx.z, a1v[u].z), __fadd_rn(dx.w, a1v[u].w));
+    st4(a.dx + off, dx);
+    if (a.dz) {
+      if (a.dz_bits && dr.enabled) dx = f4_select((kbz[u] >> (4 * (l32 & 1))) & 15u, make_float4(dx.x * dr.scale, dx.y * dr.scale, dx.z * dr.scale, dx.w * dr.scale));
+      st4(a.dz + off, dx);
+      if (MID) zv[u] = dx;
+    }
+  }
+  HUAL_STAMP_K(4, 22);
+  {
+    auto xor32_sum = [&](float v) {
+      const unsigned x = __builtin_bit_cast(unsigned, v);
+      const auto r = __builtin_amdgcn_permlane32_swap(x, x, false, false);
+      return v + __builtin_bit_cast(float, (lane & 32) ? r[0] : r[1]);
+    };
+    auto xor32_sum4 = [&](float4 v) { return make_float4(xor32_sum(v.x), xor32_sum(v.y), xor32_sum(v.z), xor32_sum(v.w)); };
+    sg1 = xor32_sum4(sg1); sb1 = xor32_sum4(sb1); sg2 = xor32_sum4(sg2); sb2 = xor32_sum4(sb2);
+    float4* pb = reinterpret_cast<float4*>(Ps);
+    if (lane < 32) {
+      float4* dst = pb + wave * 4 * 32 + l32;
+      dst[0] = sg1; dst[32] = sb1; dst[64] = sg2; dst[96] = sb2;
+    }
+    cb_barrier();
+    const float* pf = reinterpret_cast<const float*>(pb);
+    const int e = threadIdx.x;
+    float s = 0.f;
+#pragma unroll
+    for (int w = 0; w < 8; ++w) s += pf[w * 4 * HUAL_D + e];
+    a.part[(size_t)tile_ * 4 * HUAL_D + e] = s;
+  }
+  HUAL_STAMP_K(4, 23);
+  return true;
+}
diff --git a/hual_amd/csrc/seqpan.hip b/hual_amd/csrc/seqpan.hip
--- a/hual_amd/csrc/seqpan.hip
+++ b/hual_amd/csrc/seqpan.hip
@@ -26,6 +26,8 @@
 enum { ST_ALWAYS = 0, ST_INPUT = 1, ST_CONV = 2, ST_DA = 3, ST_CQ = 4, ST_FUSE = 5, ST_PRED = 6 };
 
 struct WsEntry { std::string name; size_t off, rows, cols; };
+
+struct CbBwdHeld { bool held = false; CbBwdArgs a; RowSpace rs; };
 
 struct Ctx {
   const hual_cfg* cfg = nullptr;
@@ -120,7 +122,7 @@
     if (active) colsum.push_back(cj);
     if (live()) chk(launch_ln_bwd(a, drop, stream, pos, npos, &rs));
   }
-  void ln_proj_bwd(const LnProjBwdArgs& a0, float* dg1, float* db1, float* dg2, float* db2) {
+  void ln_proj_bwd(const LnProjBwdArgs& a0, float* dg1, float* db1, float* dg2, float* db2, CbBwdHeld* front = nullptr) {
     LnProjBwdArgs a = a0;
     a.MT = ln_proj_bwd_rows(a.R, a.Nv);
     const int nblk = ln_proj_bwd_blocks(a.R, a.Nv);
@@ -129,6 +131,13 @@
     cj.src = a.part; cj.nblk = nblk; cj.nvec = 4;
     cj.dst[0] = dg1; cj.dst[1] = db1; cj.dst[2] = dg2; cj.dst[3] = db2;
     if (active) colsum.push_back(cj);
+    if (front && front->held) {
+      front->held = false;
+      if (live()) {
+        if (conv_block_bwd_tail_fits(front->a, front->rs, a)) { chk(launch_conv_block_bwd(front->a, front->rs, drop, stream, &a)); return; }
+        chk(launch_conv_block_bwd(front->a, front->rs, drop, stream));
+      }
+    }
     if (live()) chk(launch_ln_proj_bwd(a, drop, stream));
   }
   void ln2_mid_bwd(const LnProjBwdArgs& a0, const DaMidBwdArgs& m0, float* dg1, float* db1) {
@@ -504,7 +513,7 @@
   return b.x[4];
 }
 
-float* conv_block_bwd(Ctx& c, const CbBufs& b, float* dx, const ConvBlockP& cp, const RowSpace& rs) {
+float* conv_block_bwd(Ctx& c, const CbBufs& b, float* dx, const ConvBlockP& cp, const RowSpace& rs, CbBwdHeld* hold = nullptr) {
   const int R = rs.R;
   const std::string dt = "d." + b.tag;
   CbBwdArgs a{};
@@ -528,7 +537,8 @@
     if (c.active) c.colsum.push_back(cj);
     c.push_dw(mkdw(b.c[i], HUAL_D, HUAL_D, L.dz, HUAL_D, R, c.g(cp.pw[i]), c.g(cp.b[i])));
   }
-  if (c.live()) c.chk(launch_conv_block_bwd(a, rs, c.drop, c.stream));
+  if (hold && c.sel_stage < 0 && !cb_no_tail()) { hold->held = true; hold->a = a; hold->rs = rs; }
+  else if (c.live()) c.chk(launch_conv_block_bwd(a, rs, c.drop, c.stream));
   return a.dx_out;
 }
 
@@ -818,7 +828,7 @@
   return g;
 }
 
-float* bwd_fe(Ctx& c, int ps, const HeadBufs& hd, float* d_fn, float* d_in) {
+float* bwd_fe(Ctx& c, int ps, const HeadBufs& hd, float* d_fn, float* d_in, CbBwdHeld& held) {
   const ParamMap& pm = c.pm;
   const int D = HUAL_D, Nv = c.rs.Nv;
   const std::string dt = "d.fe" + std::to_string(ps);
@@ -837,7 +847,7 @@
     lb.nsteps = 1; lb.A[0] = nullptr; lb.lda[0] = D; lb.wimg_t[0] = c.nimg(pm.fe_dense.k); lb.dst[0] = 0;
     lb.dy1_bits = b.kb7; lb.x = b.res; lb.mean = b.mean2; lb.rstd = b.rstd2; lb.g1 = c.p(pm.fe_ln2.g);
     lb.dx = d_res; lb.dz = d_att; lb.dz_bits = b.kb6; lb.R = Nv; lb.drop_row0 = 0;
-    c.ln_proj_bwd(lb, c.g(pm.fe_ln2.g), c.g(pm.fe_ln2.b), c.g(hl.g), c.g(hl.b));
+    c.ln_proj_bwd(lb, c.g(pm.fe_ln2.g), c.g(pm.fe_ln2.b), c.g(hl.g), c.g(hl.b), ps == 0 ? &held : nullptr);
   }
   float* d_qkv = c.buf(dt + ".qkv", Nv, 3 * D);
   AttnJob a = b.job;
@@ -854,7 +864,7 @@
     lb.dx = d_f; lb.R = Nv; lb.drop_row0 = 0;
     c.ln_proj_bwd(lb, c.g(pm.fe_ln1.g), c.g(pm.fe_ln1.b), nullptr, nullptr);
   }
-  return conv_block_bwd(c, b.cb, d_f, pm.fe_cb, c.rsv);
+  return conv_block_bwd(c, b.cb, d_f, pm.fe_cb, c.rsv, ps == 1 ? &held : nullptr);
 }
 
 float* bwd_fuse(Ctx& c, const CoreBufs& k, const FuseBufs& f, const HeadBufs& hd, float* cqf, float* d_in, float* d_out_heads,
@@ -1112,8 +1122,9 @@
   c.stage(ST_PRED);
   const HeadGrads hg = bwd_heads(c, hd, fu.outputs);
   float* fe_dx0[2] = {nullptr, nullptr};
-  fe_dx0[1] = bwd_fe(c, 1, hd, hg.d_fn[1], nullptr);
-  fe_dx0[0] = bwd_fe(c, 0, hd, hg.d_fn[0], fe_dx0[1]);
+  CbBwdHeld held;
+  fe_dx0[1] = bwd_fe(c, 1, hd, hg.d_fn[1], nullptr, held);
+  fe_dx0[0] = bwd_fe(c, 0, hd, hg.d_fn[0], fe_dx0[1], held);
   float* d_cqf = bwd_fuse(c, core, fu, hd, cq.feats, fe_dx0[0], hg.d_out, lab, opt);
   float* dx = bwd_cq(c, cq, d_cqf);
   for (int li = c.cfg->attn_layer - 1; li >= 0; --li) dx = bwd_da(c, li, dx);
```

Result: no change. 53900 clips/s (-0.1%).
